# CIS565-Fall-2017/Project3-CUDA-Path-Tracer

Hardware: AMD Instinct MI355X
Metric: Mrays/sec (live paths x bounces) at 800x800 Cornell depth 8 (higher is better)
Workload: dtype f32

## Files before the change

project3-cuda-path-tracer_amd/csrc/pt_h_api.hpp:

```cpp
#pragma once

namespace one {

const char *pt_last_error(void) { return g_err; }
const char *pt_version(void) {
#ifdef PT_EXPERIMENTS
    return "ptmi355 0.1 (gfx950, fp32 no-contract, wave64) +experiments";
#else
    return "ptmi355 0.1 (gfx950, fp32 no-contract, wave64)";
#endif
}

void pt_free(void) {
    if (!R.live && !R.scratch) return;
    if (R.stream) (void)hipStreamSynchronize(R.stream);
    for (int k = 0; k < OV_MAX_LANES; ++k) {
        if (R.lane[k].stream) (void)hipStreamSynchronize(R.lane[k].stream);
        if (R.lane[k].la_stream) (void)hipStreamSynchronize(R.lane[k].la_stream);
    }
    if (R.la_gstream) (void)hipStreamSynchronize(R.la_gstream);
    for (int k = 0; k < 2; ++k) if (R.pool_mem[k]) (void)hipFree(R.pool_mem[k]);
    if (R.isect_mem) (void)hipFree(R.isect_mem);
    if (R.sort_table) (void)hipFree(R.sort_table);
    if (R.cache_mem) (void)hipFree(R.cache_mem);
    if (R.state_mem) (void)hipFree(R.state_mem);
    if (R.state_ended) (void)hipFree(R.state_ended);
    if (R.final_mem) (void)hipFree(R.final_mem);
    if (R.image && R.own_image) (void)hipFree(R.image);
    if (R.d_geoms) (void)hipFree(R.d_geoms);
    if (R.d_mats) (void)hipFree(R.d_mats);
    if (R.d_tris) (void)hipFree(R.d_tris);
    if (R.d_cull) (void)hipFree(R.d_cull);
    if (R.d_grec) (void)hipFree(R.d_grec);
    if (R.d_tri_bound) (void)hipFree(R.d_tri_bound);
    if (R.d_ginfo) (void)hipFree(R.d_ginfo);
    if (R.d_env) (void)hipFree(R.d_env);
    if (R.d_lights) (void)hipFree(R.d_lights);
    if (R.d_tex) (void)hipFree(R.d_tex);
    if (R.d_tex_tab) (void)hipFree(R.d_tex_tab);
    if (R.d_bump) (void)hipFree(R.d_bump);
    if (R.d_bump_tab) (void)hipFree(R.d_bump_tab);
    if (R.mesh_hit) (void)hipFree(R.mesh_hit);
    for (int k = 0; k < 2; ++k) if (R.mesh_flags[k]) (void)hipFree(R.mesh_flags[k]);
    if (R.d_bvh_nodes) (void)hipFree(R.d_bvh_nodes);
    if (R.d_bvh_meshes) (void)hipFree(R.d_bvh_meshes);
    if (R.d_bvh_tris) (void)hipFree(R.d_bvh_tris);
    if (R.d_bvh_top) (void)hipFree(R.d_bvh_top);
    if (R.d_cam_mask) (void)hipFree(R.d_cam_mask);
    R.d_cam_mask = nullptr; R.cam_mask_valid = false;
    if (R.d_cull0) (void)hipFree(R.d_cull0);
    R.d_cull0 = nullptr; R.cull0_tiles = 0;
    free_lanes();
    if (R.ctl) (void)hipFree(R.ctl);
    if (R.dir_mem) (void)hipFree(R.dir_mem);
    if (R.persist) (void)hipFree(R.persist);
    if (R.iter_counts) (void)hipFree(R.iter_counts);
    if (R.h_stats) (void)hipHostFree(R.h_stats);
    if (R.scratch) (void)hipFree(R.scratch);
    if (R.gb_mem) (void)hipFree(R.gb_mem);
    for (int k = 0; k < 2; ++k) if (R.dn_plane[k]) (void)hipFree(R.dn_plane[k]);
    if (R.dn_rgba) (void)hipFree(R.dn_rgba);
    if (R.gb_alt) (void)hipFree(R.gb_alt);
    if (R.alb_mem) (void)hipFree(R.alb_mem);
    for (int k = 0; k < 2; ++k) {
        if (R.tp_c[k]) (void)hipFree(R.tp_c[k]);
        if (R.tp_n[k]) (void)hipFree(R.tp_n[k]);
    }
    if (R.tp_hc) (void)hipFree(R.tp_hc);
    if (R.tp_hn) (void)hipFree(R.tp_hn);
    if (R.dbg_counts) (void)hipFree(R.dbg_counts);
    if (R.copy_stream) (void)hipStreamSynchronize(R.copy_stream);
    for (auto &h : R.host_regs) (void)hipHostUnregister(h.ptr);
    for (int j = 0; j < 2; ++j) {
        if (R.snap[j]) (void)hipFree(R.snap[j]);
        if (R.ev_snap[j]) (void)hipEventDestroy(R.ev_snap[j]);
        if (R.ev_copied[j]) (void)hipEventDestroy(R.ev_copied[j]);
    }
    if (R.copy_stream) (void)hipStreamDestroy(R.copy_stream);
    for (hipEvent_t e : R.ev) (void)hipEventDestroy(e);
    if (R.stream && R.own_stream) (void)hipStreamDestroy(R.stream);
    R = Renderer{};
}


static float glossy_alpha2(float exponent) {
    if (!(exponent > 0.0f)) return 0.0f;
    return (float)(2.0 / ((double)exponent + 2.0));
}

static void pack_materials(const pt_material *materials, int count, float *rec, bool glossy = false) {
    for (int i = 0; i < count; ++i) {
        const pt_material &m = materials[i];
        float *r = rec + (size_t)i * ptd::MAT_WORDS;
        r[0] = m.color.x; r[1] = m.color.y; r[2] = m.color.z;
        r[3] = m.specular.color.x; r[4] = m.specular.color.y; r[5] = m.specular.color.z;
        r[6] = m.hasReflective; r[7] = m.hasRefractive; r[8] = m.indexOfRefraction; r[9] = m.emittance;
        if (glossy) r[10] = glossy_alpha2(m.specular.exponent);
    }
}

static int init_impl(const pt_scene_desc *d);
int la_discard(int how);
enum { LA_STREAM = 0, LA_HOST = 1, LA_LATER = 2 };

}

#include "pt_h_scene.hpp"

namespace one {

int pt_init(const pt_scene_desc *d) {
    if (!d) return fail(PT_ERR_INVALID, "pt_init: null descriptor");
    if (R.live) pt_free();
    const int rc = init_impl(d);
    if (rc != PT_OK) {
        char keep[ERR_BYTES];
        memcpy(keep, t_err, sizeof keep);
        R.live = true;
        pt_free();
        memcpy(t_err, keep, sizeof keep);
    }
    return rc;
}

static int init_impl(const pt_scene_desc *d) {
    const int W = d->camera.resolution[0], H = d->camera.resolution[1];
    if (W <= 0 || H <= 0 || (int64_t)W * H > (1 << 28)) return fail(PT_ERR_INVALID, "pt_init: bad resolution %dx%d", W, H);
    if (d->num_geoms < 0 || d->num_materials <= 0 || (d->num_geoms > 0 && !d->geoms) || !d->materials)
        return fail(PT_ERR_INVALID, "pt_init: geoms/materials missing");
    if (d->trace_depth < 1 || d->trace_depth > MAX_DEPTH) return fail(PT_ERR_INVALID, "pt_init: trace_depth %d outside [1,%d]", d->trace_depth, MAX_DEPTH);
    const int tile_count = d->tile_count <= 0 ? 1 : d->tile_count;
    if (d->tile_index < 0 || d->tile_index >= tile_count) return fail(PT_ERR_INVALID, "pt_init: tile_index %d / tile_count %d", d->tile_index, tile_count);
    if (tile_count > 1 && d->strip_rows <= 0) return fail(PT_ERR_INVALID, "pt_init: strip_rows must be > 0 when tiling");
    for (int i = 0; i < d->num_geoms; ++i) {
        const pt_geom &g = d->geoms[i];
        if (g.type < PT_SPHERE || g.type > PT_TRIANGLE_MESH) return fail(PT_ERR_INVALID, "pt_init: geom %d has type %d", i, g.type);
        if (g.materialid < 0 || g.materialid >= d->num_materials) return fail(PT_ERR_INVALID, "pt_init: geom %d materialid %d out of range", i, g.materialid);
    }
    if (d->num_meshes < 0 || d->num_triangles < 0 || (d->num_meshes > 0 && !d->meshes) || (d->num_triangles > 0 && !d->triangles))
        return fail(PT_ERR_INVALID, "pt_init: meshes / triangles missing");
    for (int k = 0; k < d->num_meshes; ++k) {
        const pt_mesh &m = d->meshes[k];
        if (m.geom_index < 0 || m.geom_index >= d->num_geoms || d->geoms[m.geom_index].type != PT_TRIANGLE_MESH ||
            m.first_triangle < 0 || m.triangle_count < 0 ||
            (int64_t)m.first_triangle + (int64_t)m.triangle_count > (int64_t)d->num_triangles)
            return fail(PT_ERR_INVALID, "pt_init: mesh %d is inconsistent", k);
        for (int j = 0; j < k; ++j)
            if (d->meshes[j].geom_index == m.geom_index)
                return fail(PT_ERR_INVALID, "pt_init: geom %d owns more than one mesh", m.geom_index);
    }
    if ((d->flags & PT_CACHE_FIRST) && ((d->flags & PT_AA_JITTER) || d->lens_radius > 0.0f))
        return fail(PT_ERR_INVALID, "pt_init: PT_CACHE_FIRST needs identical camera rays every iteration; it cannot be "
                                    "combined with PT_AA_JITTER or a lens (INSTRUCTION.md:113)");
    if (d->lens_radius > 0.0f && !(d->focal_distance > 0.0f))
        return fail(PT_ERR_INVALID, "pt_init: a lens needs focal_distance > 0");
    std::vector<pt_light_element> light_el;
    if ((d->flags & PT_DIRECT_SKY) && !(d->flags & PT_DIRECT_LIGHT) && !(d->flags & PT_FAKE_SHADER))
        return fail(PT_ERR_INVALID, "pt_init: PT_DIRECT_SKY needs PT_DIRECT_LIGHT (the sky is one more light element of its sampler)");
    if ((d->flags & PT_DIRECT_LIGHT) && !(d->flags & PT_FAKE_SHADER)) {
        if (d->flags & PT_UNFUSED)
            return fail(PT_ERR_INVALID, "pt_init: PT_DIRECT_LIGHT cannot be combined with PT_UNFUSED (its intersection planes do not carry the winning primitive)");
        if (d->flags & PT_CACHE_FIRST)
            return fail(PT_ERR_INVALID, "pt_init: PT_DIRECT_LIGHT cannot be combined with PT_CACHE_FIRST (the table form of bounce 0 has no DIRECT variant)");
        if (d->trace_depth > MAX_DEPTH - 1)
            return fail(PT_ERR_INVALID, "pt_init: PT_DIRECT_LIGHT runs trace_depth + 1 bounces: trace_depth %d outside [1,%d]", d->trace_depth, MAX_DEPTH - 1);
        const int ne = ptlight::elements(d->geoms, d->num_geoms, d->materials, d->num_materials, light_el);
        if (ne < 0) return fail(PT_ERR_INTERNAL, "pt_init: light elements");
        if (ne > ptlight::MAX_ELEMENTS)
            return fail(PT_ERR_INVALID, "pt_init: PT_DIRECT_LIGHT: %d light elements (at most %d)", ne, ptlight::MAX_ELEMENTS);
    }
    if ((d->flags & PT_TEXTURES) && !(d->flags & PT_FAKE_SHADER)) {
        if (d->flags & PT_UNFUSED)
            return fail(PT_ERR_INVALID, "pt_init: PT_TEXTURES cannot be combined with PT_UNFUSED (its intersection planes do not carry the winning primitive)");
        if (d->flags & PT_CACHE_FIRST)
            return fail(PT_ERR_INVALID, "pt_init: PT_TEXTURES cannot be combined with PT_CACHE_FIRST (the table form of bounce 0 has no TEX variant)");
        if (d->flags & PT_DIRECT_LIGHT)
            return fail(PT_ERR_INVALID, "pt_init: PT_TEXTURES cannot be combined with PT_DIRECT_LIGHT (the direct kernels have no textured form yet)");
    }
    int ndev = 0;
    if (hipGetDeviceCount(&ndev) != hipSuccess || ndev <= 0)
        return fail(PT_ERR_DEVICE, "pt_init: no HIP device (this library has no CPU fallback)");
    if (d->device < 0 || d->device >= ndev) return fail(PT_ERR_INVALID, "pt_init: device %d of %d", d->device, ndev);
    HIPCHK(hipSetDevice(d->device));

    R = Renderer{};
    R.desc = *d; R.cam = d->camera; R.trace_depth = d->trace_depth; R.flags = d->flags; R.device = d->device;
    R.lens = Lens{(d->flags & PT_AA_JITTER) ? 1 : 0, d->lens_radius, d->focal_distance};
    R.whole_max_paths = 6000000;
    if (const char *wm = getenv("PTMI355_WHOLE_MAX")) R.whole_max_paths = strtoull(wm, nullptr, 10);
    R.whole_max_host_paths = 16000000;
    if (const char *wm = getenv("PTMI355_WHOLE_MAX_HOST")) R.whole_max_host_paths = strtoull(wm, nullptr, 10);
    if (getenv("PTMI355_WHOLE_MAX") && !getenv("PTMI355_WHOLE_MAX_HOST")) R.whole_max_host_paths = R.whole_max_paths;
    if (const char *e = getenv("PTMI355_OVERLAP")) {
        const int nl = atoi(e);
        R.ov_enabled = nl != 0;
        if (nl >= 2) { R.ov_lanes = std::min(nl, OV_MAX_LANES); R.ov_lanes_set = true; }
    }
    if (const char *e = getenv("PTMI355_OVERLAP_GB")) R.ov_budget_gb = atof(e);
    if (const char *e = pt_experiment("PTMI355_LANE_STREAMS")) R.ov_streams = std::max(1, atoi(e));
    R.epi_enabled = true;
    if (const char *e = pt_experiment("PTMI355_HOST_EPILOGUE")) R.epi_enabled = atoi(e) != 0;
    if (const char *e = pt_experiment("PTMI355_EPI_DIRECT")) R.epi_direct_enabled = atoi(e) != 0;
    R.defer_enabled = true;
    if (const char *e = pt_experiment("PTMI355_DEFER_DIR")) R.defer_enabled = atoi(e) != 0;
    R.own_enabled = true;
    if (const char *e = pt_experiment("PTMI355_OWN_SURFACE")) R.own_enabled = atoi(e) != 0;
    R.first_hit_enabled = true;
    if (const char *e = pt_experiment("PTMI355_FIRST_HIT")) R.first_hit_enabled = atoi(e) != 0;
    R.first_two_enabled = true;
    if (const char *e = pt_experiment("PTMI355_FIRST_TWO")) R.first_two_enabled = atoi(e) != 0;
    R.first_state_enabled = true;
    if (const char *e = pt_experiment("PTMI355_FIRST_STATE")) R.first_state_enabled = atoi(e) != 0;
    R.host_sparse_enabled = (d->flags & (PT_HOST_SPARSE | PT_SHARED_IMAGE)) != 0;
    if (const char *e = pt_experiment("PTMI355_ASYNC_DIRECT")) R.async_direct_enabled = atoi(e) != 0;
    R.pin_enabled = true;
    if (const char *e = pt_experiment("PTMI355_PIN")) R.pin_enabled = atoi(e) != 0;
    R.npix = W * H;
    R.map.W = W; R.map.H = H; R.map.tile_index = d->tile_index; R.map.tile_count = tile_count;
    R.map.strip_rows = tile_count > 1 ? d->strip_rows : H;
    R.map.tile_pixels = tile_rows(d->tile_index, tile_count, R.map.strip_rows, H) * W;
    if (R.map.tile_pixels <= 0) return fail(PT_ERR_INVALID, "pt_init: tile owns no rows");
    make_div_magic((uint32_t)R.map.tile_pixels, &R.map.div_magic, &R.map.div_shift);
    auto magic_holds = [](uint32_t d, uint32_t magic, uint32_t shift) {
        auto fast = [&](uint32_t n) {
            if (d == 1) return n;
            const uint32_t q = (uint32_t)(((uint64_t)magic * n) >> 32);
            return (((n - q) >> 1) + q) >> shift;
        };
        for (uint64_t k = 0; k <= 0xffffffffull / d && k < 4096; ++k)
            for (int e = -1; e <= 1; ++e) {
                const uint64_t n = k * d + (uint64_t)(int64_t)e;
                if (n <= 0xffffffffull && fast((uint32_t)n) != (uint32_t)n / d) return false;
            }
        const uint32_t probes[] = {0u, 1u, d - 1, d, d + 1, 0x7fffffffu, 0x80000000u, 0xfffffffeu, 0xffffffffu};
        for (uint32_t n : probes)
            if (fast(n) != n / d) return false;
        return true;
    };
    if (!magic_holds((uint32_t)R.map.tile_pixels, R.map.div_magic, R.map.div_shift))
        return fail(PT_ERR_INTERNAL, "pt_init: division magic failed for n / %d", R.map.tile_pixels);
    if (tile_count > 1) {
        const uint32_t span = (uint32_t)R.map.strip_rows * (uint32_t)W;
        make_div_magic(span, &R.la_tg.magic, &R.la_tg.shift);
        R.la_tg.skip = (uint32_t)(tile_count - 1) * span;
        R.la_tg.first = (uint32_t)d->tile_index * span;
        R.la_tiles_ok = span >= 2 && magic_holds(span, R.la_tg.magic, R.la_tg.shift);
    }
    R.max_batch = d->max_batch < 1 ? 1 : d->max_batch;
    if ((int64_t)R.max_batch * R.map.tile_pixels >= (int64_t)0x3ffffff0)
        return fail(PT_ERR_INVALID, "pt_init: max_batch * tile pixels must stay below 2^30 (32-bit byte offsets into the planes)");
    R.cap = (uint32_t)R.max_batch * (uint32_t)R.map.tile_pixels;
    if (d->stream) { R.stream = (hipStream_t)d->stream; R.own_stream = false; }
    else {
        int lo = 0, hi = 0;
        const char *pe = pt_experiment("PTMI355_MAIN_PRIO");
        if (hipDeviceGetStreamPriorityRange(&lo, &hi) != hipSuccess) { (void)hipGetLastError(); lo = hi = 0; }
        if ((pe && atoi(pe) == 0) || hipStreamCreateWithPriority(&R.stream, hipStreamNonBlocking, hi) != hipSuccess) {
            (void)hipGetLastError();
            HIPCHK(hipStreamCreateWithFlags(&R.stream, hipStreamNonBlocking));
        }
        R.own_stream = true;
    }
    R.live = true;

    std::vector<float> grec((size_t)std::max(1, d->num_geoms) * ptd::GEOM_WORDS, 0.0f);
    for (int i = 0; i < d->num_geoms; ++i) {
        const pt_geom &g = d->geoms[i];
        float *r = grec.data() + (size_t)i * ptd::GEOM_WORDS;
        int first = 0, count = 0, boff = 0;
        for (int k = 0, off = 0; k < d->num_meshes; ++k) {
            if (d->meshes[k].geom_index == i) { first = d->meshes[k].first_triangle; count = d->meshes[k].triangle_count; boff = off; break; }
            off += (d->meshes[k].triangle_count + 63) & ~63;
        }
        memcpy(&r[0], &g.type, 4); memcpy(&r[1], &g.materialid, 4); memcpy(&r[2], &first, 4); memcpy(&r[3], &count, 4);
        const pt_mat4 *ms[3] = {&g.inverseTransform, &g.transform, &g.invTranspose};
        const int offs[3] = {ptd::G_INV, ptd::G_FWD, ptd::G_INVT};
        for (int m = 0; m < 3; ++m)
            for (int c = 0; c < 4; ++c)
                for (int rr = 0; rr < 3; ++rr) r[offs[m] + c * 3 + rr] = ms[m]->m[c][rr];
        if (g.type == PT_TRIANGLE_MESH) memcpy(&r[ptd::G_INV + 6], &boff, 4);
    }
    std::vector<float> mrec((size_t)d->num_materials * ptd::MAT_WORDS, 0.0f);
    pack_materials(d->materials, d->num_materials, mrec.data(), (d->flags & PT_GLOSSY) != 0);
    std::vector<float> trec((size_t)std::max(1, d->num_triangles) * TRI_WORDS, 0.0f);
    for (int i = 0; i < d->num_triangles; ++i) {
        const pt_triangle &t = d->triangles[i];
        float *r = trec.data() + (size_t)i * TRI_WORDS;
        r[0] = t.v0.x; r[1] = t.v0.y; r[2] = t.v0.z;
        r[3] = t.v1.x - t.v0.x; r[4] = t.v1.y - t.v0.y; r[5] = t.v1.z - t.v0.z;
        r[6] = t.v2.x - t.v0.x; r[7] = t.v2.y - t.v0.y; r[8] = t.v2.z - t.v0.z;
    }
    for (int k = 0; k < d->num_meshes; ++k) {
        const pt_mesh &m = d->meshes[k];
        const float pad = ptbvh::spec_pad(reinterpret_cast<const float *>(d->triangles + m.first_triangle), m.triangle_count);
        for (int i = 0; i < m.triangle_count; ++i) trec[(size_t)(m.first_triangle + i) * TRI_WORDS + 10] = pad;
    }
    HIPCHK(hipMalloc(&R.d_geoms, grec.size() * 4));
    HIPCHK(hipMalloc(&R.d_mats, mrec.size() * 4));
    HIPCHK(hipMalloc(&R.d_tris, trec.size() * 4));
    HIPCHK(hipMemcpy(R.d_geoms, grec.data(), grec.size() * 4, hipMemcpyHostToDevice));
    HIPCHK(hipMemcpy(R.d_mats, mrec.data(), mrec.size() * 4, hipMemcpyHostToDevice));
    HIPCHK(hipMemcpy(R.d_tris, trec.data(), trec.size() * 4, hipMemcpyHostToDevice));
    R.scene.geoms = R.d_geoms; R.scene.ngeoms = d->num_geoms;
    R.scene.mats = R.d_mats; R.scene.nmats = d->num_materials;
    R.scene.tris = R.d_tris; R.scene.ntris = d->num_triangles;
    {
        std::vector<float> gath((size_t)std::max(1, d->num_geoms) * GREC_WORDS, 0.0f);
        std::vector<uint32_t> ginfo((size_t)std::max(1, d->num_geoms), 0u);
        for (int i = 0; i < d->num_geoms; ++i) {
            const pt_geom &g = d->geoms[i];
            float *r = gath.data() + (size_t)i * GREC_WORDS;
            const pt_mat4 *ms[3] = {&g.inverseTransform, &g.transform, &g.invTranspose};
            for (int m = 0; m < (g.type == PT_CUBE ? 2 : 3); ++m)
                for (int c = 0; c < 4; ++c)
                    for (int rr = 0; rr < 3; ++rr) r[m * 12 + c * 3 + rr] = ms[m]->m[c][rr];
            if (g.type == PT_CUBE && !pt_experiment("PTMI355_NO_AXIS_REJECT")) {
                const int ax = ptcull::reject_row(&g.inverseTransform.m[0][0], r + GREC_ROW);
                if (ax == 4 && pt_experiment("PTMI355_NO_ROW_REJECT")) r[GREC_ROW] = r[GREC_ROW + 1] = r[GREC_ROW + 2] = r[GREC_ROW + 3] = 0.0f;
            }
            ginfo[(size_t)i] = (uint32_t)g.materialid | ((uint32_t)g.type << 28);
        }
        if (d->num_materials >= (1 << 28)) return fail(PT_ERR_INVALID, "pt_init: at most 2^28 materials");
        HIPCHK(hipMalloc(&R.d_grec, gath.size() * 4));
        HIPCHK(hipMalloc((void **)&R.d_ginfo, ginfo.size() * 4));
        HIPCHK(hipMemcpy(R.d_grec, gath.data(), gath.size() * 4, hipMemcpyHostToDevice));
        HIPCHK(hipMemcpy(R.d_ginfo, ginfo.data(), ginfo.size() * 4, hipMemcpyHostToDevice));
        if (d->num_geoms > 0) {
            hipLaunchKernelGGL(k_face_normals, dim3((d->num_geoms * 8 + BLOCK - 1) / BLOCK), dim3(BLOCK), 0, R.stream,
                               R.d_grec, (const uint32_t *)R.d_ginfo, d->num_geoms);
            HIPCHK(hipGetLastError());
            HIPCHK(hipStreamSynchronize(R.stream));
        }
        R.scene.grec = R.d_grec; R.scene.ginfo = R.d_ginfo;
    }
    R.mesh_mode = MESH_NONE;
    for (int i = 0; i < d->num_geoms; ++i)
        if (d->geoms[i].type == PT_TRIANGLE_MESH) R.mesh_mode = (d->flags & PT_MESH_BVH) ? MESH_BVH : MESH_TILES;
    R.geoms_keep.assign(d->geoms, d->geoms + d->num_geoms);
    if (d->num_triangles > 0) R.tris_keep.assign(d->triangles, d->triangles + d->num_triangles);
    R.desc.geoms = R.geoms_keep.data();
    R.desc.triangles = R.tris_keep.empty() ? nullptr : R.tris_keep.data();
    if (d->num_meshes > 0) R.meshes_keep.assign(d->meshes, d->meshes + d->num_meshes);
    R.desc.meshes = R.meshes_keep.empty() ? nullptr : R.meshes_keep.data();
    R.grec_frames.assign((size_t)std::max(1, d->num_geoms) * 4, 0.0f);
    {
        const int rc = upload_cull(&R.desc, R.cam);
        if (rc != PT_OK) return rc;
    }
    if (R.mesh_mode == MESH_BVH) {
        const int rc = upload_bvh(&R.desc, grec);
        if (rc != PT_OK) return rc;
        HIPCHK(hipMemcpy(R.d_geoms, grec.data(), grec.size() * 4, hipMemcpyHostToDevice));
    }
    R.grec_keep = grec;
    {
        const size_t base = ((size_t)LDS_CTL_WORDS + (size_t)WAVES * PW_WORDS) * 4 +
                            (R.mesh_mode == MESH_TILES ? (size_t)WAVES * TRQ_WORDS * 4 : 0);
        const size_t scene = (size_t)scene_lds_words(d->num_materials, d->num_geoms) * 4;
        R.scene_lds = base + scene <= 32 * 1024;
        if (const char *e = getenv("PTMI355_SCENE_LDS")) R.scene_lds = atoi(e) != 0 && base + scene <= 64 * 1024;
        R.lds_bytes = base + (R.scene_lds ? scene : 0);
        R.lds_bytes = (R.lds_bytes + 15) & ~(size_t)15;
        if (const char *pad = pt_experiment("PTMI355_LDS_PAD")) R.lds_bytes += (size_t)atoi(pad);
    }

    R.sort_keys = 0;
    if ((R.flags & PT_SORT_MATERIAL) && (R.flags & PT_COMPACT) && !(R.flags & (PT_UNFUSED | PT_FAKE_SHADER | PT_CACHE_FIRST)) &&
        R.mesh_mode != MESH_BVH && d->num_materials <= 64) {
        bool on = true;
        if (const char *e = pt_experiment("PTMI355_SORT_FUSED")) on = atoi(e) != 0;
        double budget_gb = 96.0;
        if (const char *e = pt_experiment("PTMI355_SORT_FUSED_GB")) budget_gb = atof(e);
        R.sort_runs = 1;
        if (const char *e = pt_experiment("PTMI355_SORT_RUNS")) R.sort_runs = std::max(1, std::min(8, atoi(e)));
        const double tiles_k = (double)d->num_materials * ((double)((R.cap + 63) / 64) + 8192.0 * R.sort_runs);
        if (on && tiles_k * 2560.0 * 2.0 <= budget_gb * 1e9 && tiles_k * 64.0 < 2147483648.0) R.sort_keys = d->num_materials;
    }
    if ((R.flags & PT_DIRECT_LIGHT) && !(R.flags & PT_FAKE_SHADER) && (R.flags & PT_SORT_MATERIAL) && !R.sort_keys)
        return fail(PT_ERR_INVALID, "pt_init: PT_DIRECT_LIGHT cannot be combined with the two-kernel form of PT_SORT_MATERIAL, which this "
                                    "session would take (its intersection planes do not carry the winning primitive)");
    if ((R.flags & PT_TEXTURES) && !(R.flags & PT_FAKE_SHADER) && (R.flags & PT_SORT_MATERIAL) && !R.sort_keys)
        return fail(PT_ERR_INVALID, "pt_init: PT_TEXTURES cannot be combined with the two-kernel form of PT_SORT_MATERIAL, which this "
                                    "session would take (its intersection planes do not carry the winning primitive)");
    if (!light_el.empty()) {
        std::vector<float> lrec;
        ptlight::records(d->geoms, light_el, lrec);
        static_assert(ptlight::RECORD_WORDS == ptd::LIGHT_WORDS, "one record layout");
        HIPCHK(hipMalloc((void **)&R.d_lights, lrec.size() * 4));
        HIPCHK(hipMemcpy(R.d_lights, lrec.data(), lrec.size() * 4, hipMemcpyHostToDevice));
        R.nlights = (int)light_el.size();
        if (sky_session()) R.lamp_rec = lrec;
    }
    const size_t capz = R.cap;
    const size_t pool_mult = (size_t)std::max(1, R.sort_keys);
    const size_t run_mult = R.sort_keys > 0 ? (size_t)R.sort_runs : 1;
    for (int k = 0; k < 2; ++k) {
        R.pool_bytes = pool_mult * (((capz + 63) / 64) + 2 * 8192 * run_mult) * 64 * 10 * 4;
        HIPCHK(hipMalloc(&R.pool_mem[k], R.pool_bytes));
        R.pool[k] = carve_pool(R.pool_mem[k], R.cap);
    }
    if ((R.flags & (PT_UNFUSED | PT_FAKE_SHADER)) || ((R.flags & PT_SORT_MATERIAL) && !R.sort_keys)) {
        const int rc = ensure_isect();
        if (rc != PT_OK) return rc;
    }
    R.final_bytes = capz * 4 * 4;
    HIPCHK(hipMalloc(&R.final_mem, R.final_bytes));
    HIPCHK(hipMemsetAsync(R.final_mem, 0, capz * 4 * 4, R.stream));
    R.fin_serial = 0;
    if (const char *e = pt_experiment("PTMI355_FIN_SERIAL")) R.fin_serial = (uint32_t)strtoul(e, nullptr, 0);
    if (d->device_image) { R.image = d->device_image; R.own_image = false; }
    else {
        HIPCHK(hipMalloc(&R.image, (size_t)R.npix * 3 * 4));
        R.own_image = true;
        HIPCHK(hipMemsetAsync(R.image, 0, (size_t)R.npix * 3 * 4, R.stream));
    }
    R.max_tiles = (R.cap + TILE - 1) / TILE;
    R.ctl_bytes = offsetof(Control, bucket) - offsetof(Control, stamp) +
                  (size_t)session_bounces_max(R.trace_depth) * sizeof(((Control *)nullptr)->bucket[0]);
    HIPCHK(hipMalloc((void **)&R.ctl, sizeof(Control)));
    HIPCHK(hipMemsetAsync(R.ctl, 0, sizeof(Control), R.stream));
    HIPCHK(hipMalloc((void **)&R.persist, sizeof(Persist)));
    HIPCHK(hipMemsetAsync(R.persist, 0, sizeof(Persist), R.stream));
    hipDeviceProp_t prop;
    HIPCHK(hipGetDeviceProperties(&prop, d->device));
    const int cus = prop.multiProcessorCount > 0 ? prop.multiProcessorCount : 256;
    int per_cu = 8;
    {
        const bool sorted = R.sort_keys > 0;
        const bool own = R.mesh_mode == MESH_NONE && !sorted;
        auto size_for = [&](auto sh) -> int {
            constexpr int SH = decltype(sh)::value;
            const void *fns[2];
            if (R.mesh_mode == MESH_BVH) { fns[0] = bounce_fn<MESH_PRE, SH>(R.scene_lds, false, false); fns[1] = bounce_fn<MESH_PRE, SH>(R.scene_lds, true, false); }
            else if (R.mesh_mode == MESH_TILES) { fns[0] = bounce_fn<MESH_TILES, SH>(R.scene_lds, false, sorted); fns[1] = bounce_fn<MESH_TILES, SH>(R.scene_lds, true, sorted); }
            else { fns[0] = bounce_fn<MESH_NONE, SH>(R.scene_lds, false, sorted); fns[1] = bounce_fn<MESH_NONE, SH>(R.scene_lds, true, sorted); }
            const void *fns_own[2] = {own ? bounce_fn<MESH_NONE, SH>(R.scene_lds, false, false, true) : fns[0], own ? bounce_fn<MESH_NONE, SH>(R.scene_lds, true, false, true) : fns[1]};
            const void *fns_tab[4] = {own ? bounce_fn<MESH_NONE, SH>(R.scene_lds, false, false, false, true) : fns[0], own ? bounce_fn<MESH_NONE, SH>(R.scene_lds, true, false, false, true) : fns[1],
                                      own ? bounce_fn<MESH_NONE, SH>(R.scene_lds, false, false, true, true) : fns[0], own ? bounce_fn<MESH_NONE, SH>(R.scene_lds, true, false, true, true) : fns[1]};
            const void *fns_two[2] = {own ? bounce_fn<MESH_NONE, SH>(R.scene_lds, true, false, false, true, true) : fns[0],
                                      own ? bounce_fn<MESH_NONE, SH>(R.scene_lds, true, false, true, true, true) : fns[0]};
            const void *fns_state[2] = {own ? bounce_fn<MESH_NONE, SH>(R.scene_lds, true, false, false, true, true, true) : fns[0],
                                        own ? bounce_fn<MESH_NONE, SH>(R.scene_lds, true, false, true, true, true, true) : fns[0]};
            for (const void *f : {fns[0], fns[1], fns_own[0], fns_own[1], fns_tab[0], fns_tab[1], fns_tab[2], fns_tab[3], fns_two[0], fns_two[1],
                                  fns_state[0], fns_state[1]}) {
                int n = 0;
                HIPCHK(hipOccupancyMaxActiveBlocksPerMultiprocessor(&n, f, BLOCK, R.lds_bytes));
                per_cu = std::min(per_cu, n);
            }
            return PT_OK;
        };
        int rc = size_for(std::integral_constant<int, 0>{});
        if (rc == PT_OK && (R.nlights > 0 || sky_session())) rc = size_for(std::integral_constant<int, SH_DIRECT>{});
        if (rc == PT_OK && (R.flags & PT_TEXTURES) && !(R.flags & PT_FAKE_SHADER)) rc = size_for(std::integral_constant<int, SH_TEX>{});
        if (rc != PT_OK) return rc;
    }
    if (per_cu < 1) per_cu = 1;
    if (per_cu > 8) per_cu = 8;
    if (const char *e = pt_experiment("PTMI355_WGS_PER_CU")) per_cu = std::max(1, std::min(per_cu, atoi(e)));
    R.grid = (int)std::min<uint32_t>((R.max_tiles + WAVES - 1) / WAVES, (uint32_t)cus * (uint32_t)per_cu);
    R.per_cu = per_cu;
    if (const char *e = pt_experiment("PTMI355_LA_CUS")) R.la_cus = std::max(0, std::min(64, atoi(e) & ~7));
    if (R.grid < 1) R.grid = 1;
    if (R.grid * WAVES > 8192) R.grid = 8192 / WAVES;
    {
        int n = 0;
        HIPCHK(hipOccupancyMaxActiveBlocksPerMultiprocessor(
            &n, R.scene_lds ? (const void *)k_iteration<true> : (const void *)k_iteration<false>, BLOCK, R.lds_bytes));
        n = std::max(1, std::min(n, 8));
        if (const char *e = pt_experiment("PTMI355_WGS_PER_CU")) n = std::max(1, std::min(n, atoi(e)));
        R.grid_iter = (int)std::min<uint32_t>((R.max_tiles + WAVES - 1) / WAVES, (uint32_t)cus * (uint32_t)n);
        R.grid_iter = std::max(1, std::min(R.grid_iter, 8192 / WAVES));
        R.grid_iter_cur = R.grid_iter; R.cus = cus;
        if (const char *e = pt_experiment("PTMI355_ITER_TPW")) R.iter_tpw = std::max(0, atoi(e));
        if (const char *e = pt_experiment("PTMI355_ITER_WGS_ALL")) R.iter_wgs_per_cu_all = std::max(1, atoi(e));
        R.iter_counts_bytes = (size_t)MAX_DEPTH * (size_t)R.grid_iter * 4;
        HIPCHK(hipMalloc((void **)&R.iter_counts, R.iter_counts_bytes));
        void *hs = nullptr, *ds = nullptr;
        if (hipHostMalloc(&hs, sizeof(HostStats), hipHostMallocMapped) == hipSuccess && hipHostGetDevicePointer(&ds, hs, 0) == hipSuccess) {
            memset(hs, 0, sizeof(HostStats));
            R.h_stats = (HostStats *)hs; R.d_stats = (HostStats *)ds;
        } else {
            (void)hipGetLastError();
            if (hs) (void)hipHostFree(hs);
        }
    }
    if (R.mesh_mode == MESH_BVH) {
        R.mesh_hit_bytes = (size_t)(((capz + 63) / 64) * 64) * sizeof(float4);
        HIPCHK(hipMalloc((void **)&R.mesh_hit, R.mesh_hit_bytes));
        R.flag_words = (size_t)R.max_tiles + 2 * (size_t)R.grid * WAVES + 8;
        for (int k = 0; k < 2; ++k) {
            HIPCHK(hipMalloc((void **)&R.mesh_flags[k], R.flag_words * sizeof(unsigned long long)));
            HIPCHK(hipMemsetAsync(R.mesh_flags[k], 0, R.flag_words * sizeof(unsigned long long), R.stream));
        }
        HIPCHK(hipFuncSetAttribute((const void *)k_mesh<true>, hipFuncAttributeMaxDynamicSharedMemorySize, (int)MESH_LDS_BYTES));
        HIPCHK(hipFuncSetAttribute((const void *)k_mesh<false>, hipFuncAttributeMaxDynamicSharedMemorySize, (int)MESH_LDS_BYTES));
        R.grid_mesh = (int)std::min<uint32_t>((R.max_tiles + MESH_WG_WAVES - 1) / MESH_WG_WAVES, (uint32_t)cus);
        if (R.grid_mesh < 1) R.grid_mesh = 1;
    }
    if (R.flags & PT_CACHE_FIRST) {
        HIPCHK(hipMalloc(&R.cache_mem, (size_t)R.map.tile_pixels * Isect::FIRST_HIT_BYTES));
    } else if (R.first_hit_enabled && !(R.flags & (PT_UNFUSED | PT_SORT_MATERIAL | PT_FAKE_SHADER | PT_AA_JITTER)) && R.mesh_mode == MESH_NONE) {
        if (hipMalloc(&R.cache_mem, (size_t)R.map.tile_pixels * Isect::FIRST_HIT_BYTES) != hipSuccess) { (void)hipGetLastError(); R.cache_mem = nullptr; }
        bool fixed0 = R.cache_mem != nullptr && R.first_state_enabled && !(R.flags & PT_GLOSSY);
        for (int m = 0; m < d->num_materials; ++m) fixed0 = fixed0 && !(d->materials[m].hasRefractive > 0.0f);
        if (fixed0) {
            if (hipMalloc(&R.state_mem, first_state_bytes((size_t)R.map.tile_pixels)) != hipSuccess) { (void)hipGetLastError(); R.state_mem = nullptr; }
            if (R.state_mem && R.map.tile_pixels % TILE == 0 &&
                hipMalloc((void **)&R.state_ended, (size_t)(R.map.tile_pixels / TILE) * sizeof(uint32_t)) != hipSuccess) { (void)hipGetLastError(); R.state_ended = nullptr; }
        }
    }
    if ((R.flags & PT_SORT_MATERIAL) && !R.sort_keys) {
        if (d->num_materials + 1 > SORT_MAX_BINS)
            return fail(PT_ERR_INVALID, "pt_init: PT_SORT_MATERIAL keeps one bin per material in LDS: at most %d materials", SORT_MAX_BINS - 1);
        {
            int per_cu_sort = 8;
            if (const char *e = pt_experiment("PTMI355_SORT_WGS")) per_cu_sort = std::max(1, atoi(e));
            R.sort_wave = true;
            if (const char *e = pt_experiment("PTMI355_SORT_WAVE")) R.sort_wave = atoi(e) != 0;
            const uint32_t chunks = (R.cap + SORT_CHUNK - 1) / SORT_CHUNK;
            R.grid_sort = (int)std::max<uint32_t>(1u, std::min<uint32_t>(chunks, (uint32_t)cus * (uint32_t)per_cu_sort));
        }
        HIPCHK(hipMalloc((void **)&R.sort_table, ((size_t)(d->num_materials + 1) * R.grid_sort + 4) * sizeof(uint32_t)));
    }
    {
        const size_t Wp = ((size_t)R.grid * WAVES * pool_mult * run_mult + 3) & ~(size_t)3;
        R.dir_stride = range_dir_words(Wp);
        R.dir_bytes = (size_t)MAX_DEPTH * R.dir_stride * sizeof(uint32_t);
        HIPCHK(hipMalloc((void **)&R.dir_mem, R.dir_bytes));
    }
    {
        const int rc = update_cam_mask();
        if (rc != PT_OK) return rc;
    }
    {
        bool on = true;
        if (const char *e = getenv("PTMI355_CULL0")) on = atoi(e) != 0;
        if (on && R.scene.ngeoms >= 1 && R.scene.ngeoms <= 64 && R.map.tile_pixels % TILE == 0) {
            R.cull0_tiles = (uint32_t)(R.map.tile_pixels / TILE);
            HIPCHK(hipMalloc((void **)&R.d_cull0, (size_t)R.cull0_tiles * sizeof(unsigned long long)));
            const int rc = update_cull0();
            if (rc != PT_OK) return rc;
        }
    }
    if (const char *e = pt_experiment("PTMI355_DBG_COUNTS")) {
        R.dbg_words = (size_t)std::max(64, atoi(e));
        HIPCHK(hipMalloc((void **)&R.dbg_counts, R.dbg_words * 4));
        HIPCHK(hipMemsetAsync(R.dbg_counts, 0, R.dbg_words * 4, R.stream));
    }
    HIPCHK(hipStreamSynchronize(R.stream));
    t_err[0] = 0;
    return PT_OK;
}

int pt_set_camera(const pt_camera *camera, int trace_depth) {
    if (!R.live) return fail(PT_ERR_INVALID, "pt_set_camera: not initialised");
    if (!camera) return fail(PT_ERR_INVALID, "pt_set_camera: null camera");
    if (camera->resolution[0] != R.map.W || camera->resolution[1] != R.map.H)
        return fail(PT_ERR_INVALID, "pt_set_camera: resolution changed (%dx%d -> %dx%d); re-init instead",
                    R.map.W, R.map.H, camera->resolution[0], camera->resolution[1]);
    if (trace_depth < 1 || trace_depth > MAX_DEPTH)
        return fail(PT_ERR_INVALID, "pt_set_camera: trace_depth %d outside [1, %d]", trace_depth, MAX_DEPTH);
    if ((R.flags & PT_DIRECT_LIGHT) && !(R.flags & PT_FAKE_SHADER) && trace_depth > MAX_DEPTH - 1)
        return fail(PT_ERR_INVALID, "pt_set_camera: PT_DIRECT_LIGHT runs trace_depth + 1 bounces: trace_depth %d outside [1, %d]", trace_depth, MAX_DEPTH - 1);
    if (memcmp(&R.cam, camera, sizeof R.cam) != 0) {
        R.cache_valid = false;
        const int rc = la_discard(LA_HOST);
        if (rc) return rc;
    }
    bool recull = false;
    {
        const double reach = (double)std::fabs(camera->position.x) + std::fabs(camera->position.y) + std::fabs(camera->position.z);
        if (std::isfinite(reach) && reach > (double)R.scene.rmax && reach != R.cull_eye_reach) {
            const int rc = upload_cull(&R.desc, *camera);
            if (rc != PT_OK) return rc;
            recull = true;
        }
    }
    if (trace_depth != R.trace_depth) {
        R.ctl_bytes = offsetof(Control, bucket) - offsetof(Control, stamp) +
                      (size_t)session_bounces_max(trace_depth) * sizeof(((Control *)nullptr)->bucket[0]);
    }
    const bool moved = memcmp(&R.cam, camera, sizeof R.cam) != 0;
    R.cam = *camera;
    R.trace_depth = trace_depth;
    if (moved || recull) {
        R.ov_active = false;
        const int rc = update_cull0();
        if (rc != PT_OK) return rc;
    }
    if (recull && R.mesh_mode == MESH_BVH) {
        HIPCHK(hipStreamSynchronize(R.stream));
        float **old[] = {&R.d_bvh_nodes, &R.d_bvh_tris, &R.d_bvh_top};
        for (float **p : old) { if (*p) (void)hipFree(*p); *p = nullptr; }
        if (R.d_bvh_meshes) { (void)hipFree(R.d_bvh_meshes); R.d_bvh_meshes = nullptr; }
        const int rc = upload_bvh(&R.desc, R.grec_keep);
        if (rc != PT_OK) return rc;
        HIPCHK(hipMemcpy(R.d_geoms, R.grec_keep.data(), R.grec_keep.size() * 4, hipMemcpyHostToDevice));
    }
    if ((moved || recull) && R.mesh_mode == MESH_BVH) {
        HIPCHK(hipStreamSynchronize(R.stream));
        const int rc = update_cam_mask();
        if (rc != PT_OK) return rc;
    }
    return PT_OK;
}

int pt_set_lens(float lens_radius, float focal_distance) {
    if (!R.live) return fail(PT_ERR_INVALID, "pt_set_lens: not initialised");
    if (lens_radius > 0.0f && !(focal_distance > 0.0f)) return fail(PT_ERR_INVALID, "pt_set_lens: a lens needs focal_distance > 0");
    if (lens_radius > 0.0f && (R.flags & PT_CACHE_FIRST))
        return fail(PT_ERR_INVALID, "pt_set_lens: PT_CACHE_FIRST cannot be combined with a lens");
    R.lens.radius = lens_radius; R.lens.focal = focal_distance;
    return PT_OK;
}

static int upload_sky_lights(const float *texels, int n) {
    std::vector<float> rows, cols, rec;
    int count = (int)(R.lamp_rec.size() / (size_t)ptlight::RECORD_WORDS);
    const std::vector<float> *src = &R.lamp_rec;
    if (texels && n > 0 && ptlight::sky_table(texels, n, rows, cols)) {
        count = ptlight::sky_records(R.lamp_rec, n, rows, cols, rec);
        src = &rec;
    }
    if (R.d_lights) { (void)hipFree(R.d_lights); R.d_lights = nullptr; }
    R.nlights = 0;
    if (count == 0) return PT_OK;
    if (hipMalloc((void **)&R.d_lights, src->size() * 4) != hipSuccess) {
        (void)hipGetLastError(); R.d_lights = nullptr;
        return fail(PT_ERR_NOMEM, "pt_set_environment: %zu bytes of device memory for the light table", src->size() * 4);
    }
    HIPCHK(hipMemcpy(R.d_lights, src->data(), src->size() * 4, hipMemcpyHostToDevice));
    R.nlights = count;
    return PT_OK;
}

int pt_set_environment(const float *texels, int n) {
    if (!R.live) return fail(PT_ERR_INVALID, "pt_set_environment: not initialised");
    if (n < 0 || n > 1024) return fail(PT_ERR_INVALID, "pt_set_environment: n = %d outside [0, 1024]", n);
    if (n > 0 && !texels) return fail(PT_ERR_INVALID, "pt_set_environment: null texels with n = %d", n);
    if (!texels) n = 0;
    const int rc = la_discard(LA_HOST);
    if (rc) return rc;
    HIPCHK(hipStreamSynchronize(R.stream));
    for (int k = 0; k < OV_MAX_LANES; ++k) {
        if (R.lane[k].stream) HIPCHK(hipStreamSynchronize(R.lane[k].stream));
        if (R.lane[k].la_stream) HIPCHK(hipStreamSynchronize(R.lane[k].la_stream));
    }
    if (R.la_gstream) HIPCHK(hipStreamSynchronize(R.la_gstream));
    if (R.copy_stream) HIPCHK(hipStreamSynchronize(R.copy_stream));
    R.ov_active = false;
    R.env_n = 0;
    if (R.d_env) { (void)hipFree(R.d_env); R.d_env = nullptr; }
    R.env_keep.clear();
    if (sky_session()) {
        const int rc2 = upload_sky_lights(nullptr, 0);
        if (rc2) return rc2;
    }
    if (n == 0) return PT_OK;
    const size_t count = (size_t)6 * (size_t)n * (size_t)n;
    std::vector<float> quad(count * 4);
    for (size_t k = 0; k < count; ++k) {
        quad[4 * k] = texels[3 * k]; quad[4 * k + 1] = texels[3 * k + 1]; quad[4 * k + 2] = texels[3 * k + 2]; quad[4 * k + 3] = 0.0f;
    }
    if (hipMalloc((void **)&R.d_env, count * 16) != hipSuccess) {
        (void)hipGetLastError(); R.d_env = nullptr;
        return fail(PT_ERR_NOMEM, "pt_set_environment: %zu bytes of device memory for a %d x %d x 6 map", count * 16, n, n);
    }
    HIPCHK(hipMemcpy(R.d_env, quad.data(), count * 16, hipMemcpyHostToDevice));
    R.env_keep.assign(texels, texels + count * 3);
    R.env_n = n;
    if (sky_session()) return upload_sky_lights(texels, n);
    return PT_OK;
}

int pt_get_environment(float *texels, int capacity_texels, int *n) {
    if (!R.live) return fail(PT_ERR_INVALID, "pt_get_environment: not initialised");
    if (!n) return fail(PT_ERR_INVALID, "pt_get_environment: null n");
    const int en = R.env_n;
    *n = en;
    if (en == 0) return PT_OK;
    const size_t count = (size_t)6 * (size_t)en * (size_t)en;
    if (!texels || capacity_texels < 0 || (size_t)capacity_texels < count)
        return fail(PT_ERR_INVALID, "pt_get_environment: room for %d texels, the map has %zu", texels ? capacity_texels : 0, count);
    memcpy(texels, R.env_keep.data(), count * 12);
    return PT_OK;
}

int pt_set_texture(int material, const float *texels, int n) {
    if (!R.live) return fail(PT_ERR_INVALID, "pt_set_texture: not initialised");
    if (!(R.flags & PT_TEXTURES)) return fail(PT_ERR_INVALID, "pt_set_texture: the session was not initialised with PT_TEXTURES");
    if (material < 0 || material >= R.scene.nmats) return fail(PT_ERR_INVALID, "pt_set_texture: material %d outside [0, %d)", material, R.scene.nmats);
    if (n < 0 || n > 1024) return fail(PT_ERR_INVALID, "pt_set_texture: n = %d outside [0, 1024]", n);
    if (n > 0 && !texels) return fail(PT_ERR_INVALID, "pt_set_texture: null texels with n = %d", n);
    if (!texels) n = 0;
    const int rc = la_discard(LA_HOST);
    if (rc) return rc;
    HIPCHK(hipStreamSynchronize(R.stream));
    for (int k = 0; k < OV_MAX_LANES; ++k) {
        if (R.lane[k].stream) HIPCHK(hipStreamSynchronize(R.lane[k].stream));
        if (R.lane[k].la_stream) HIPCHK(hipStreamSynchronize(R.lane[k].la_stream));
    }
    if (R.la_gstream) HIPCHK(hipStreamSynchronize(R.la_gstream));
    if (R.copy_stream) HIPCHK(hipStreamSynchronize(R.copy_stream));
    R.ov_active = false;
    if (R.tex_n.empty()) { R.tex_n.assign((size_t)R.scene.nmats, 0); R.tex_keep.resize((size_t)R.scene.nmats); }
    std::vector<int> tn = R.tex_n;
    tn[(size_t)material] = n;
    std::vector<int2> tab((size_t)R.scene.nmats);
    size_t total = 0;
    int ntex = 0;
    for (int m = 0; m < R.scene.nmats; ++m) {
        tab[(size_t)m] = make_int2((int)total, tn[(size_t)m]);
        total += (size_t)6 * (size_t)tn[(size_t)m] * (size_t)tn[(size_t)m];
        if (tn[(size_t)m] > 0) ++ntex;
    }
    if (total > (size_t)0x7fffffff) return fail(PT_ERR_INVALID, "pt_set_texture: %zu texels in all (at most 2^31 - 1)", total);
    float4 *d_new = nullptr;
    if (ntex > 0) {
        std::vector<float> quad(total * 4);
        for (int m = 0; m < R.scene.nmats; ++m) {
            const size_t cnt = (size_t)6 * (size_t)tn[(size_t)m] * (size_t)tn[(size_t)m];
            const float *src = m == material ? texels : R.tex_keep[(size_t)m].data();
            float *dst = quad.data() + (size_t)tab[(size_t)m].x * 4;
            for (size_t k = 0; k < cnt; ++k) { dst[4 * k] = src[3 * k]; dst[4 * k + 1] = src[3 * k + 1]; dst[4 * k + 2] = src[3 * k + 2]; dst[4 * k + 3] = 0.0f; }
        }
        if (hipMalloc((void **)&d_new, total * 16) != hipSuccess) {
            (void)hipGetLastError();
            return fail(PT_ERR_NOMEM, "pt_set_texture: %zu bytes of device memory for the session's textures", total * 16);
        }
        HIPCHK(hipMemcpy(d_new, quad.data(), total * 16, hipMemcpyHostToDevice));
    }
    if (!R.d_tex_tab) HIPCHK(hipMalloc((void **)&R.d_tex_tab, tab.size() * sizeof(int2)));
    HIPCHK(hipMemcpy(R.d_tex_tab, tab.data(), tab.size() * sizeof(int2), hipMemcpyHostToDevice));
    const int old_n = R.tex_n[(size_t)material];
    if (old_n != n || (n > 0 && memcmp(R.tex_keep[(size_t)material].data(), texels, (size_t)6 * (size_t)n * (size_t)n * 12) != 0))
        R.alb_valid = false;
    if (R.d_tex) (void)hipFree(R.d_tex);
    R.d_tex = d_new;
    R.tex_n = tn;
    if (n > 0) R.tex_keep[(size_t)material].assign(texels, texels + (size_t)6 * (size_t)n * (size_t)n * 3);
    else std::vector<float>().swap(R.tex_keep[(size_t)material]);
    R.ntex = ntex;
    return PT_OK;
}

int pt_get_texture(int material, float *texels, int capacity_texels, int *n) {
    if (!R.live) return fail(PT_ERR_INVALID, "pt_get_texture: not initialised");
    if (!(R.flags & PT_TEXTURES)) return fail(PT_ERR_INVALID, "pt_get_texture: the session was not initialised with PT_TEXTURES");
    if (material < 0 || material >= R.scene.nmats) return fail(PT_ERR_INVALID, "pt_get_texture: material %d outside [0, %d)", material, R.scene.nmats);
    if (!n) return fail(PT_ERR_INVALID, "pt_get_texture: null n");
    const int tn = R.tex_n.empty() ? 0 : R.tex_n[(size_t)material];
// ... 634 lines not shown
```

project3-cuda-path-tracer_amd/csrc/pt_h_enqueue.hpp:

```cpp
#pragma once

namespace {

BounceArgs bounce_args(int depth) {
    BounceArgs a{};
    a.dbg_counts = R.dbg_counts;
    a.in = R.pool[R.cur];
    a.out = (R.flags & PT_COMPACT) ? R.pool[R.cur ^ 1] : R.pool[R.cur];
    a.isect = R.isect;
    a.scene = R.scene;
    a.map = R.map;
    a.ctl = R.ctl;
    a.dir_in = tile_dir((R.flags & PT_COMPACT) ? R.cur_dir : -1);
    a.dir_out = tile_dir(depth);
    a.fin = R.final_mem;
    a.fin_stamp = R.fin_serial;
    a.cam = R.cam;
    a.lens = R.lens;
    a.depth = depth; a.trace_depth = R.trace_depth; a.iter0 = R.step_iter0;
    a.pool_n = (uint32_t)R.map.tile_pixels * (uint32_t)R.step_count;
    a.gen_rays = (depth == 0 && R.gen_fused) ? 1 : 0;
    a.mesh_hit = R.mesh_hit;
    a.mesh_flags_in = R.mesh_flags[depth & 1]; a.mesh_flags_out = R.mesh_flags[(depth + 1) & 1];
    a.mesh_scan = R.mesh_marked ? 0 : 1;
    a.cam_mask = (R.cam_mask_valid && !(R.lens.radius > 0.0f)) ? R.d_cam_mask : nullptr;
    const bool same_rays = !R.lens.aa && !(R.lens.radius > 0.0f);
    a.cull0 = (R.cull0_tiles && same_rays) ? R.d_cull0 : nullptr;
    a.cull0_tiles = R.cull0_tiles;
    a.iter_counts = R.iter_counts;
    a.persist = R.persist;
    a.env = R.d_env; a.env_n = R.env_n;
    a.lights = R.d_lights; a.nlights = R.nlights;
    if (R.ntex + R.nbump > 0) { a.tex = R.d_tex; a.tex_tab = R.d_tex_tab; }
    if (R.nbump > 0) { a.bumps = R.d_bump; a.bump_tab = R.d_bump_tab; }
    return a;
}

int next_fin_stamp(void) {
    if (++R.fin_serial == 0) {
        HIPCHK(hipMemsetAsync(R.final_mem, 0, (size_t)R.cap * 16, R.stream));
        if (R.ov_ready)
            for (int j = 1; j < R.ov_lanes; ++j)
                HIPCHK(hipMemsetAsync(R.lane[j].b.final_mem, 0, R.final_bytes, R.stream));
        R.fin_serial = 1;
    }
    return PT_OK;
}

int enqueue_begin(int iter0, int count, bool stepping, bool clear = true) {
    if (count < 1 || count > R.max_batch)
        return fail(PT_ERR_INVALID, "batch count %d outside [1, max_batch=%d]", count, R.max_batch);
    if (iter0 < 0 || (int64_t)iter0 + count - 1 > 0x7fffffff)
        return fail(PT_ERR_INVALID, "iteration %d (+%d) outside [0, 2^31)", iter0, count);
    R.step_iter0 = iter0; R.step_count = count; R.step_depth = 0; R.cur = 0; R.cur_dir = -1;
    R.pool_own = false;
    R.ov_active = false;
    R.last_ctl = R.ctl;
    const int rc = next_fin_stamp();
    if (rc) return rc;
    R.sorted_isects = false;
    R.mesh_marked = false;
    R.self_gathered = false; R.host_stats_serial = 0;
    if (clear) HIPCHK(hipMemsetAsync(&R.ctl->stamp, 0, R.ctl_bytes, R.stream));
    if (R.mesh_mode == MESH_BVH)
        for (int k = 0; k < 2; ++k)
            HIPCHK(hipMemsetAsync(R.mesh_flags[k], 0, R.flag_words * sizeof(unsigned long long), R.stream));
    R.gen_fused = !stepping && (!(R.flags & (PT_UNFUSED | PT_SORT_MATERIAL | PT_FAKE_SHADER)) || R.sort_keys > 0);
    R.gen_sort = !stepping && (R.flags & PT_SORT_MATERIAL) && !R.sort_keys && !(R.flags & PT_FAKE_SHADER) && R.sort_wave &&
                 R.scene.nmats + 1 <= SORTW_MAX_BINS;
    if (R.gen_fused || R.gen_sort) return PT_OK;
    const uint32_t total = (uint32_t)R.map.tile_pixels * (uint32_t)count;
    StageTimer tm(PT_STAGE_RAYGEN);
    hipLaunchKernelGGL(k_raygen, dim3((total + BLOCK - 1) / BLOCK), dim3(BLOCK), 0, R.stream, R.pool[0], R.cam,
                       R.lens, R.map, count, iter0, R.trace_depth, R.ctl);
    HIPCHK(hipGetLastError());
    return PT_OK;
}

#define PT_MESH_DISPATCH(CALL)                                          \
    do {                                                                \
        if (R.scene_lds) {                                              \
            constexpr bool SLDS = true;                                 \
            if (R.mesh_mode == MESH_BVH) { constexpr int MESH = MESH_BVH; CALL; }            \
            else if (R.mesh_mode == MESH_TILES) { constexpr int MESH = MESH_TILES; CALL; }   \
            else { constexpr int MESH = MESH_NONE; CALL; }              \
        } else {                                                        \
            constexpr bool SLDS = false;                                \
            if (R.mesh_mode == MESH_BVH) { constexpr int MESH = MESH_BVH; CALL; }            \
            else if (R.mesh_mode == MESH_TILES) { constexpr int MESH = MESH_TILES; CALL; }   \
            else { constexpr int MESH = MESH_NONE; CALL; }              \
        }                                                               \
    } while (0)

void launch_intersect(const Pool &in, const uint32_t *n_ptr, uint32_t n_fixed, const RangeDir &dir,
                      const uint32_t *nprev, bool raygen_pool = false, bool generate = false) {
    const bool same_rays = !R.lens.aa && !(R.lens.radius > 0.0f);
    const unsigned long long *cull0 = (raygen_pool && R.cull0_tiles && same_rays) ? R.d_cull0 : nullptr;
    RayGen gen{};
    if (generate) {
        gen.cam = R.cam; gen.lens = R.lens; gen.map = R.map; gen.trace_depth = R.trace_depth;
        gen.iter0 = R.step_iter0;
        PT_MESH_DISPATCH(hipLaunchKernelGGL((k_intersect<MESH, SLDS, true>), dim3(R.grid), dim3(BLOCK), R.lds_bytes, R.stream, in,
                                            R.isect, R.scene, n_ptr, n_fixed, dir, nprev, R.ctl, cull0, R.cull0_tiles, gen));
        return;
    }
    PT_MESH_DISPATCH(hipLaunchKernelGGL((k_intersect<MESH, SLDS>), dim3(R.grid), dim3(BLOCK), R.lds_bytes, R.stream, in,
                                        R.isect, R.scene, n_ptr, n_fixed, dir, nprev, R.ctl, cull0, R.cull0_tiles, gen));
}

template <int MESH, int SH = 0>
const void *bounce_fn(bool slds, bool gen, bool sorted, bool own = false, bool table = false, bool first2 = false, bool state2 = false) {
    if constexpr (MESH == MESH_NONE) {
        if (table && !sorted) {
            constexpr int SH0 = SH & (SH_ENV | SH_GLOSSY);
            if (first2 && state2) {
                if (own) return slds ? (const void *)k_bounce<MODE_STATE2, true, MESH, true, true, false, true, 0> : (const void *)k_bounce<MODE_STATE2, true, MESH, false, true, false, true, 0>;
                return slds ? (const void *)k_bounce<MODE_STATE2, true, MESH, true, true, false, false, 0> : (const void *)k_bounce<MODE_STATE2, true, MESH, false, true, false, false, 0>;
            }
            if (first2) {
                if (own) return slds ? (const void *)k_bounce<MODE_FIRST2, true, MESH, true, true, false, true, SH0> : (const void *)k_bounce<MODE_FIRST2, true, MESH, false, true, false, true, SH0>;
                return slds ? (const void *)k_bounce<MODE_FIRST2, true, MESH, true, true, false, false, SH0> : (const void *)k_bounce<MODE_FIRST2, true, MESH, false, true, false, false, SH0>;
            }
            if (own) {
                if (slds) return gen ? (const void *)k_bounce<MODE_CACHE0, true, MESH, true, true, false, true, SH0> : (const void *)k_bounce<MODE_CACHE0, true, MESH, true, false, false, true, SH0>;
                return gen ? (const void *)k_bounce<MODE_CACHE0, true, MESH, false, true, false, true, SH0> : (const void *)k_bounce<MODE_CACHE0, true, MESH, false, false, false, true, SH0>;
            }
            if (slds) return gen ? (const void *)k_bounce<MODE_CACHE0, true, MESH, true, true, false, false, SH0> : (const void *)k_bounce<MODE_CACHE0, true, MESH, true, false, false, false, SH0>;
            return gen ? (const void *)k_bounce<MODE_CACHE0, true, MESH, false, true, false, false, SH0> : (const void *)k_bounce<MODE_CACHE0, true, MESH, false, false, false, false, SH0>;
        }
        if (own && !sorted) {
            if (slds) return gen ? (const void *)k_bounce<MODE_FUSED, true, MESH, true, true, false, true, SH> : (const void *)k_bounce<MODE_FUSED, true, MESH, true, false, false, true, SH>;
            return gen ? (const void *)k_bounce<MODE_FUSED, true, MESH, false, true, false, true, SH> : (const void *)k_bounce<MODE_FUSED, true, MESH, false, false, false, true, SH>;
        }
    }
    if constexpr (MESH != MESH_PRE) {
        if (sorted) {
            if (slds) return gen ? (const void *)k_bounce<MODE_FUSED, true, MESH, true, true, true, false, SH> : (const void *)k_bounce<MODE_FUSED, true, MESH, true, false, true, false, SH>;
            return gen ? (const void *)k_bounce<MODE_FUSED, true, MESH, false, true, true, false, SH> : (const void *)k_bounce<MODE_FUSED, true, MESH, false, false, true, false, SH>;
        }
    }
    if (slds) return gen ? (const void *)k_bounce<MODE_FUSED, true, MESH, true, true, false, false, SH> : (const void *)k_bounce<MODE_FUSED, true, MESH, true, false, false, false, SH>;
    return gen ? (const void *)k_bounce<MODE_FUSED, true, MESH, false, true, false, false, SH> : (const void *)k_bounce<MODE_FUSED, true, MESH, false, false, false, false, SH>;
}
#define PT_SHADE_DISPATCH_WITH(EXTRA, ...)                                                                  \
    do {                                                                                                    \
        switch ((a.env_n ? SH_ENV : 0) | ((R.flags & PT_GLOSSY) ? SH_GLOSSY : 0)) {                         \
        case SH_ENV | SH_GLOSSY: { constexpr int SH = SH_ENV | SH_GLOSSY | (EXTRA); __VA_ARGS__; } break;   \
        case SH_GLOSSY: { constexpr int SH = SH_GLOSSY | (EXTRA); __VA_ARGS__; } break;                     \
        case SH_ENV: { constexpr int SH = SH_ENV | (EXTRA); __VA_ARGS__; } break;                           \
        default: { constexpr int SH = (EXTRA); __VA_ARGS__; } break;                                        \
        }                                                                                                   \
    } while (0)
#define PT_SHADE_DISPATCH(...) PT_SHADE_DISPATCH_WITH(0, __VA_ARGS__)
template <int MODE, bool COMPACT, int MESH, bool SLDS, bool GEN, bool SORT = false, bool OWN = false>
void launch_k_bounce(const BounceArgs &a) {
    if constexpr (MODE == MODE_STATE2) {
        hipLaunchKernelGGL((k_bounce<MODE, COMPACT, MESH, SLDS, GEN, SORT, OWN, 0>), dim3(R.grid), dim3(BLOCK), R.lds_bytes, R.stream, a);
        return;
    } else {
        if constexpr (MODE == MODE_FUSED) {
            if (a.nlights > 0 && a.depth >= a.trace_depth - 1) {
                PT_SHADE_DISPATCH_WITH(SH_DIRECT, hipLaunchKernelGGL((k_bounce<MODE, COMPACT, MESH, SLDS, GEN, SORT, OWN, SH>), dim3(R.grid), dim3(BLOCK), R.lds_bytes, R.stream, a));
                return;
            }
            if (a.tex_tab != nullptr) {
                PT_SHADE_DISPATCH_WITH(SH_TEX, hipLaunchKernelGGL((k_bounce<MODE, COMPACT, MESH, SLDS, GEN, SORT, OWN, SH>), dim3(R.grid), dim3(BLOCK), R.lds_bytes, R.stream, a));
                return;
            }
        }
        PT_SHADE_DISPATCH(hipLaunchKernelGGL((k_bounce<MODE, COMPACT, MESH, SLDS, GEN, SORT, OWN, SH>), dim3(R.grid), dim3(BLOCK), R.lds_bytes, R.stream, a));
    }
}
template <int MODE, bool COMPACT, int MESH, bool GEN>
void launch_bounce_at(const BounceArgs &a) {
    if constexpr (MODE == MODE_FUSED && COMPACT && MESH != MESH_PRE) {
        if (R.sort_keys > 0) {
            if (R.scene_lds) launch_k_bounce<MODE, COMPACT, MESH, true, GEN, true>(a);
            else launch_k_bounce<MODE, COMPACT, MESH, false, GEN, true>(a);
            return;
        }
    }
    if constexpr ((MODE == MODE_FUSED || MODE == MODE_CACHE0 || mode_first2(MODE)) && COMPACT && MESH == MESH_NONE) {
        if (R.own_form) {
            if (R.scene_lds) launch_k_bounce<MODE, COMPACT, MESH, true, GEN, false, true>(a);
            else launch_k_bounce<MODE, COMPACT, MESH, false, GEN, false, true>(a);
            return;
        }
    }
    if (R.scene_lds) launch_k_bounce<MODE, COMPACT, MESH, true, GEN>(a);
    else launch_k_bounce<MODE, COMPACT, MESH, false, GEN>(a);
}
template <int MODE, bool COMPACT>
void launch_bounce(const BounceArgs &a) {
    if constexpr (MODE == MODE_ISECT) {
        launch_bounce_at<MODE, COMPACT, MESH_NONE, false>(a);
    } else if constexpr (MODE == MODE_CACHE0) {
        if (a.gen_rays) launch_bounce_at<MODE, COMPACT, MESH_NONE, true>(a); else launch_bounce_at<MODE, COMPACT, MESH_NONE, false>(a);
    } else if constexpr (mode_first2(MODE)) {
        static_assert(COMPACT, "MODE_FIRST2 / MODE_STATE2 compact");
        launch_bounce_at<MODE, COMPACT, MESH_NONE, true>(a);
    } else {
        const bool gen = a.gen_rays != 0;
        if (R.mesh_mode == MESH_BVH) { if (gen) launch_bounce_at<MODE, COMPACT, MESH_PRE, true>(a); else launch_bounce_at<MODE, COMPACT, MESH_PRE, false>(a); }
        else if (R.mesh_mode == MESH_TILES) { if (gen) launch_bounce_at<MODE, COMPACT, MESH_TILES, true>(a); else launch_bounce_at<MODE, COMPACT, MESH_TILES, false>(a); }
        else { if (gen) launch_bounce_at<MODE, COMPACT, MESH_NONE, true>(a); else launch_bounce_at<MODE, COMPACT, MESH_NONE, false>(a); }
    }
}

int enqueue_bounce(int depth, bool may_fuse = false) {
    BounceArgs a = bounce_args(depth);
    R.own_form = false;
    const bool compact = (R.flags & PT_COMPACT) != 0;
    const bool sort2 = (R.flags & PT_SORT_MATERIAL) && R.sort_keys == 0;
    const bool unfused = (R.flags & PT_UNFUSED) != 0 || sort2;
    if (unfused) {
        StageTimer tm(PT_STAGE_INTERSECT);
        const bool generate = depth == 0 && R.gen_sort;
        const uint32_t *n_ptr = (compact && !generate) ? &R.ctl->nlive[depth] : (const uint32_t *)nullptr;
        const uint32_t *nprev = (compact && depth > 0) ? &R.ctl->nlive[depth - 1] : (const uint32_t *)nullptr;
        launch_intersect(a.in, n_ptr, a.pool_n, a.dir_in, nprev, depth == 0, generate);
        HIPCHK(hipGetLastError());
    }
    if (sort2) {
        a.in = R.pool[R.cur]; a.out = R.pool[R.cur ^ 1];
        a.sort_table = R.sort_table; a.nbins = R.scene.nmats + 1;
        a.gen_rays = (depth == 0 && R.gen_sort) ? 1 : 0;
        {
            StageTimer tm(PT_STAGE_SORT);
            const size_t lds = ((size_t)LDS_CTL_WORDS + (size_t)((a.nbins + 3) & ~3)) * 4;
            if (compact) hipLaunchKernelGGL(k_sort_hist<true>, dim3(R.grid_sort), dim3(BLOCK), lds, R.stream, a);
            else hipLaunchKernelGGL(k_sort_hist<false>, dim3(R.grid_sort), dim3(BLOCK), lds, R.stream, a);
            HIPCHK(hipGetLastError());
        }
        StageTimer tm(PT_STAGE_BOUNCE);
        if (a.nbins <= SORTW_MAX_BINS && R.sort_wave) {
            const size_t lds = shade_sorted_w_lds_words(R.scene.nmats) * 4;
#define PT_SORTED_W(COMPACT, GEN) \
    PT_SHADE_DISPATCH(hipLaunchKernelGGL((k_shade_sorted_w<COMPACT, GEN, SH>), dim3(R.grid_sort), dim3(BLOCK), lds, R.stream, a))
            if (a.gen_rays) {
                if (compact) PT_SORTED_W(true, true); else PT_SORTED_W(false, true);
            } else {
                if (compact) PT_SORTED_W(true, false); else PT_SORTED_W(false, false);
            }
#undef PT_SORTED_W
        } else {
            const size_t nb = (size_t)((a.nbins + 3) & ~3);
            const size_t lds = ((size_t)LDS_CTL_WORDS + (3 + WAVES) * nb + 2 * SORT_CHUNK +
                                (a.nbins <= 64 ? (size_t)R.scene.nmats * ptd::MAT_WORDS : 0)) * 4;
            if (compact) PT_SHADE_DISPATCH(hipLaunchKernelGGL((k_shade_sorted<true, SH>), dim3(R.grid_sort), dim3(BLOCK), lds, R.stream, a));
            else PT_SHADE_DISPATCH(hipLaunchKernelGGL((k_shade_sorted<false, SH>), dim3(R.grid_sort), dim3(BLOCK), lds, R.stream, a));
        }
        HIPCHK(hipGetLastError());
        R.cur ^= 1; R.cur_dir = -1;
        R.sorted_isects = true;
        R.step_depth = depth + 1;
        return PT_OK;
    }
    const bool same_rays = !R.lens.aa && !(R.lens.radius > 0.0f);
    const bool auto0 = depth == 0 && !unfused && R.first_hit_enabled && R.cache_mem != nullptr && !(R.flags & PT_FAKE_SHADER) &&
                       R.mesh_mode == MESH_NONE && R.sort_keys == 0 && same_rays && a.tex_tab == nullptr &&
                       !(a.nlights > 0 && depth >= a.trace_depth - 1);
    const bool cached0 = depth == 0 && !unfused && ((R.flags & PT_CACHE_FIRST) || auto0);
    const bool first2 = may_fuse && auto0 && !(R.flags & PT_CACHE_FIRST) && compact && R.gen_fused && R.first_two_enabled &&
                        R.trace_depth >= 2 && !(a.nlights > 0 && 1 >= a.trace_depth - 1);
    const bool state2 = first2 && R.state_mem != nullptr && a.env_n == 0;
    if (first2) {
        depth = 1;
        a.depth = 1;
        a.dir_out = tile_dir(1);
        a.gen_rays = 1;
    }
    a.defer_dir = (compact && !unfused && R.mesh_mode == MESH_NONE && R.sort_keys == 0 && depth + 1 < R.trace_depth &&
                   R.defer_enabled) ? 1 : 0;
    R.own_form = own_surface_plan((uint64_t)a.pool_n, R.scene.ngeoms,
                                  compact && !unfused && R.mesh_mode == MESH_NONE && R.sort_keys == 0 &&
                                  R.own_enabled);
    if (cached0 && !R.cache_valid) {
        StageTimer tm(PT_STAGE_INTERSECT);
        const Isect cache{R.cache_mem, (uint32_t)R.map.tile_pixels};
        const int blocks = std::min(R.grid, (R.map.tile_pixels + BLOCK - 1) / BLOCK);
        const hipStream_t fs = R.lane_cur ? R.lane_main : R.stream;
        PT_MESH_DISPATCH(hipLaunchKernelGGL((k_cache_first<MESH, SLDS>), dim3(blocks), dim3(BLOCK), R.lds_bytes, fs,
                                            cache, R.scene, R.cam, R.map, R.state_mem, R.state_ended));
        HIPCHK(hipGetLastError());
        if (R.lane_cur) {
            HIPCHK(hipEventRecord(R.ov_enter, fs));
            HIPCHK(hipStreamWaitEvent(R.stream, R.ov_enter, 0));
            R.first_hit_refence = true;
        }
        R.cache_valid = true;
        R.first_hit_fills++;
    }
    if (!cached0 && !unfused && R.mesh_mode == MESH_BVH) {
        StageTimer tm(PT_STAGE_MESH);
        if (compact) hipLaunchKernelGGL((k_mesh<true>), dim3(R.grid_mesh), dim3(MESH_BLOCK), MESH_LDS_BYTES, R.stream, a);
        else hipLaunchKernelGGL((k_mesh<false>), dim3(R.grid_mesh), dim3(MESH_BLOCK), MESH_LDS_BYTES, R.stream, a);
        HIPCHK(hipGetLastError());
    }
    StageTimer tm(PT_STAGE_BOUNCE);
    if (cached0) {
        a.isect = Isect{R.cache_mem, (uint32_t)R.map.tile_pixels};
        R.first_hit_launches++;
        if (state2) {
            a.first_state = R.state_mem; a.first_ended = R.state_ended; a.first_ended_tiles = (uint32_t)(R.map.tile_pixels / TILE);
            R.first_two_launches++; R.first_state_launches++; tm.two_bounces(); launch_bounce<MODE_STATE2, true>(a);
        }
        else if (first2) { R.first_two_launches++; tm.two_bounces(); launch_bounce<MODE_FIRST2, true>(a); }
        else if (compact) launch_bounce<MODE_CACHE0, true>(a); else launch_bounce<MODE_CACHE0, false>(a);
    } else if (unfused) {
        if (compact) launch_bounce<MODE_ISECT, true>(a); else launch_bounce<MODE_ISECT, false>(a);
    } else {
        if (compact) launch_bounce<MODE_FUSED, true>(a); else launch_bounce<MODE_FUSED, false>(a);
    }
    HIPCHK(hipGetLastError());
    if (R.mesh_mode == MESH_BVH) {
        R.mesh_marked = !cached0 && !unfused;
    }
    if (compact) { R.cur ^= 1; R.cur_dir = depth; }
    R.pool_own = R.own_form;
    R.step_depth = depth + 1;
    return PT_OK;
}

int enqueue_fake(void) {
    const uint32_t total = (uint32_t)R.map.tile_pixels * (uint32_t)R.step_count;
    launch_intersect(R.pool[R.cur], nullptr, total, tile_dir(-1), nullptr);
    HIPCHK(hipGetLastError());
    hipLaunchKernelGGL(k_shade_fake, dim3((total + BLOCK - 1) / BLOCK), dim3(BLOCK), 0, R.stream, R.pool[R.cur],
                       R.isect, R.scene.mats, R.map, R.step_iter0, total, R.final_mem, R.fin_serial);
    HIPCHK(hipGetLastError());
    R.step_depth = 1;
    return PT_OK;
}

int enqueue_end(void) {
    if (R.self_gathered) { R.whole = false; return PT_OK; }
    if (R.la_tracing) {
        hipLaunchKernelGGL(k_gather, dim3(1), dim3(BLOCK), 0, R.stream, R.image, R.final_mem, R.cap, R.map, R.step_count, R.ctl,
                           R.persist, session_bounces(), 0u, R.whole ? 1 : 0, 1, R.fin_serial, R.iter_counts, (uint32_t)R.grid_iter_cur,
                           (HostStats *)nullptr);
        R.whole = false;
        HIPCHK(hipGetLastError());
        HIPCHK(hipEventRecord(R.lane_cur->traced, R.stream));
        R.lane_cur->gathered_valid = false;
        return PT_OK;
    }
    StageTimer tm(PT_STAGE_GATHER);
    hipStream_t gs = R.stream;
    if (R.lane_cur) {
        HIPCHK(hipEventRecord(R.lane_cur->traced, R.stream));
        HIPCHK(hipStreamWaitEvent(R.lane_main, R.lane_cur->traced, 0));
        gs = R.lane_main;
    }
    hipLaunchKernelGGL(k_gather, dim3((R.map.tile_pixels + BLOCK - 1) / BLOCK), dim3(BLOCK), 0, gs, R.image,
                       R.final_mem, R.cap, R.map,
                       R.step_count, R.ctl, R.persist, (R.flags & PT_FAKE_SHADER) ? 0 : session_bounces(),
                       (R.flags & PT_FAKE_SHADER) ? (uint32_t)R.map.tile_pixels * (uint32_t)R.step_count : 0u,
                       R.whole ? 1 : 0, R.epi_done ? 1 : 0, R.fin_serial, R.iter_counts, (uint32_t)R.grid_iter_cur,
                       (R.whole && R.host_stats_serial) ? R.d_stats : (HostStats *)nullptr);
    R.whole = false;
    R.image_epoch++;
    HIPCHK(hipGetLastError());
    if (R.lane_cur) {
        HIPCHK(hipEventRecord(R.lane_cur->gathered, gs));
        R.lane_cur->gathered_valid = true;
    }
    return PT_OK;
}

Renderer::Bufs take_bufs(void) {
    Renderer::Bufs b{};
    for (int k = 0; k < 2; ++k) { b.pool_mem[k] = R.pool_mem[k]; b.pool[k] = R.pool[k]; b.mesh_flags[k] = R.mesh_flags[k]; }
    b.final_mem = R.final_mem; b.ctl = R.ctl; b.dir_mem = R.dir_mem; b.mesh_hit = R.mesh_hit; b.iter_counts = R.iter_counts;
    return b;
}
void put_bufs(const Renderer::Bufs &b) {
    for (int k = 0; k < 2; ++k) { R.pool_mem[k] = b.pool_mem[k]; R.pool[k] = b.pool[k]; R.mesh_flags[k] = b.mesh_flags[k]; }
    R.final_mem = b.final_mem; R.ctl = b.ctl; R.dir_mem = b.dir_mem; R.mesh_hit = b.mesh_hit; R.iter_counts = b.iter_counts;
}

void free_lanes(void) {
    for (int k = 0; k < OV_MAX_LANES; ++k) {
        Renderer::Lane &l = R.lane[k];
        if (l.stream && k < R.ov_streams) { (void)hipStreamSynchronize(l.stream); (void)hipStreamDestroy(l.stream); }
        if (l.la_stream && k < R.ov_streams) { (void)hipStreamSynchronize(l.la_stream); (void)hipStreamDestroy(l.la_stream); }
        if (l.traced) (void)hipEventDestroy(l.traced);
        if (l.gathered) (void)hipEventDestroy(l.gathered);
        if (k > 0) {
            for (int j = 0; j < 2; ++j) { if (l.b.pool_mem[j]) (void)hipFree(l.b.pool_mem[j]); if (l.b.mesh_flags[j]) (void)hipFree(l.b.mesh_flags[j]); }
            if (l.b.final_mem) (void)hipFree(l.b.final_mem);
            if (l.b.ctl) (void)hipFree(l.b.ctl);
            if (l.b.dir_mem) (void)hipFree(l.b.dir_mem);
            if (l.b.iter_counts) (void)hipFree(l.b.iter_counts);
            if (l.b.mesh_hit) (void)hipFree(l.b.mesh_hit);
        }
        l = Renderer::Lane{};
    }
    if (R.la_gstream) { (void)hipStreamSynchronize(R.la_gstream); (void)hipStreamDestroy(R.la_gstream); R.la_gstream = nullptr; }
    if (R.la_rs_event) { (void)hipEventDestroy(R.la_rs_event); R.la_rs_event = nullptr; }
    R.la_masks_ready = false; R.la_masked_last = false;
    if (R.ov_enter) (void)hipEventDestroy(R.ov_enter);
    R.ov_enter = nullptr;
    R.ov_ready = false;
}

static int alloc_lanes(void) {
    R.lane[0].b = take_bufs();
    for (int j = 1; j < R.ov_lanes; ++j) {
        Renderer::Bufs &b = R.lane[j].b;
        for (int k = 0; k < 2; ++k) {
            HIPCHK(hipMalloc((void **)&b.pool_mem[k], R.pool_bytes));
            b.pool[k] = carve_pool(b.pool_mem[k], R.cap);
        }
        HIPCHK(hipMalloc((void **)&b.final_mem, R.final_bytes));
        HIPCHK(hipMemsetAsync(b.final_mem, 0, R.final_bytes, R.stream));
        HIPCHK(hipMalloc((void **)&b.ctl, sizeof(Control)));
        HIPCHK(hipMemsetAsync(b.ctl, 0, sizeof(Control), R.stream));
        HIPCHK(hipMalloc((void **)&b.dir_mem, R.dir_bytes));
        HIPCHK(hipMalloc((void **)&b.iter_counts, R.iter_counts_bytes));
        if (R.mesh_mode == MESH_BVH) {
            HIPCHK(hipMalloc((void **)&b.mesh_hit, R.mesh_hit_bytes));
            for (int k = 0; k < 2; ++k) {
                HIPCHK(hipMalloc((void **)&b.mesh_flags[k], R.flag_words * sizeof(unsigned long long)));
                HIPCHK(hipMemsetAsync(b.mesh_flags[k], 0, R.flag_words * sizeof(unsigned long long), R.stream));
            }
        }
    }
    R.ov_streams = std::max(1, std::min(R.ov_streams, R.ov_lanes));
    for (int k = 0; k < R.ov_lanes; ++k) {
        if (k < R.ov_streams) HIPCHK(hipStreamCreateWithFlags(&R.lane[k].stream, hipStreamNonBlocking));
        else R.lane[k].stream = R.lane[k % R.ov_streams].stream;
        HIPCHK(hipEventCreateWithFlags(&R.lane[k].traced, hipEventDisableTiming));
        HIPCHK(hipEventCreateWithFlags(&R.lane[k].gathered, hipEventDisableTiming));
    }
    HIPCHK(hipEventCreateWithFlags(&R.ov_enter, hipEventDisableTiming));
    return PT_OK;
}

int ensure_lanes(void) {
    if (R.ov_ready || !R.ov_enabled) return PT_OK;
    const double per_lane = 2.0 * (double)R.pool_bytes + (double)R.final_bytes + (double)R.dir_bytes + (double)R.mesh_hit_bytes +
                            2.0 * (double)R.flag_words * 8.0 + (double)sizeof(Control);
    double budget = R.ov_budget_gb * 1e9;
    size_t free_b = 0, total_b = 0;
    if (hipMemGetInfo(&free_b, &total_b) == hipSuccess) budget = std::min(budget, 0.5 * (double)free_b);
    const int fit = 1 + (int)std::min(16.0, std::floor(budget / std::max(1.0, per_lane)));
    R.ov_lanes = std::min(R.ov_lanes, fit);
    if (R.ov_lanes == 3) R.ov_lanes = 2;
    if (R.ov_lanes < 2) { R.ov_enabled = false; return PT_OK; }
    if (alloc_lanes() != PT_OK) {
        (void)hipGetLastError();
        free_lanes();
        R.ov_enabled = false;
        return PT_OK;
    }
    R.ov_ready = true;
    return PT_OK;
}

bool ensure_la_masks(void) {
    if (R.la_masks_ready) return true;
    if (R.la_masks_failed || R.la_shared_device || !R.ov_ready || R.la_cus < 8 || R.cus != 256 || R.mesh_mode == MESH_BVH) return false;
    uint32_t trace_mask[8], gather_mask[8];
    for (int b = 0; b < 8; ++b) { trace_mask[b] = 0xffffffffu; gather_mask[b] = 0; }
    for (int b = 0; b < R.la_cus; ++b) { trace_mask[b / 32] &= ~(1u << (b % 32)); gather_mask[b / 32] |= 1u << (b % 32); }
    bool ok = hipExtStreamCreateWithCUMask(&R.la_gstream, 8, gather_mask) == hipSuccess &&
              hipEventCreateWithFlags(&R.la_rs_event, hipEventDisableTiming) == hipSuccess;
    for (int k = 0; ok && k < R.ov_streams; ++k) ok = hipExtStreamCreateWithCUMask(&R.lane[k].la_stream, 8, trace_mask) == hipSuccess;
    if (!ok) {
        (void)hipGetLastError();
        for (int k = 0; k < R.ov_streams; ++k) if (R.lane[k].la_stream) { (void)hipStreamDestroy(R.lane[k].la_stream); R.lane[k].la_stream = nullptr; }
        if (R.la_gstream) { (void)hipStreamDestroy(R.la_gstream); R.la_gstream = nullptr; }
        if (R.la_rs_event) { (void)hipEventDestroy(R.la_rs_event); R.la_rs_event = nullptr; }
        R.la_masks_failed = true;
        return false;
    }
    for (int k = R.ov_streams; k < R.ov_lanes; ++k) R.lane[k].la_stream = R.lane[k % R.ov_streams].la_stream;
    R.grid_la = (int)std::min<uint32_t>((uint32_t)R.grid, (uint32_t)(R.cus - R.la_cus) * (uint32_t)std::max(1, R.per_cu));
    R.la_masks_ready = true;
    return true;
}

bool overlap_eligible(int count) {
    return R.ov_ok && R.ov_enabled && !R.profiling && !R.epi_host && !R.dbg_counts &&
           !(R.flags & (PT_UNFUSED | PT_FAKE_SHADER)) && (!(R.flags & PT_SORT_MATERIAL) || R.sort_keys > 0) &&
           count >= 1 && count <= R.max_batch;
}

int enqueue_batch_serial(int iter0, int count);

int enter_lanes(void) {
    if (R.fin_serial == 0xffffffffu) {
        HIPCHK(hipStreamSynchronize(R.stream));
        for (int j = 0; j < R.ov_lanes; ++j) HIPCHK(hipStreamSynchronize(R.lane[j].stream));
        for (int j = 0; j < R.ov_lanes; ++j) if (R.lane[j].la_stream) HIPCHK(hipStreamSynchronize(R.lane[j].la_stream));
        for (int j = 0; j < R.ov_lanes; ++j) HIPCHK(hipMemsetAsync(R.lane[j].b.final_mem, 0, R.final_bytes, R.stream));
        HIPCHK(hipStreamSynchronize(R.stream));
        R.fin_serial = 0;
        R.ov_active = false;
        for (auto &w : R.la) { w.valid = false; w.inflight = false; }
    }
    if (!R.ov_active) {
        HIPCHK(hipEventRecord(R.ov_enter, R.stream));
        for (int k = 0; k < R.ov_lanes; ++k) {
            HIPCHK(hipStreamWaitEvent(R.lane[k].stream, R.ov_enter, 0));
            if (R.lane[k].la_stream && k < R.ov_streams) HIPCHK(hipStreamWaitEvent(R.lane[k].la_stream, R.ov_enter, 0));
            R.lane[k].gathered_valid = false;
        }
    }
    return PT_OK;
}

int enqueue_on_lane(Renderer::Lane &l, int iter0, int count) {
    if (l.gathered_valid) HIPCHK(hipStreamWaitEvent(l.stream, l.gathered, 0));
    const Renderer::Bufs home = take_bufs();
    R.lane_main = R.stream; R.lane_cur = &l;
    put_bufs(l.b); R.stream = l.stream;
    const int rc = enqueue_batch_serial(iter0, count);
    R.stream = R.lane_main; put_bufs(home);
    R.lane_cur = nullptr; R.lane_main = nullptr;
    R.ov_active = rc == PT_OK && !R.first_hit_refence;
    R.first_hit_refence = false;
    return rc;
}

int enqueue_batch(int iter0, int count) {
    if (!overlap_eligible(count)) return enqueue_batch_serial(iter0, count);
    int rc = ensure_lanes();
    if (rc) return rc;
    if (!R.ov_enabled) return enqueue_batch_serial(iter0, count);
    if (R.la_masked_last) { R.ov_active = false; R.la_masked_last = false; }
    rc = enter_lanes();
    if (rc) return rc;
    Renderer::Lane &l = R.lane[R.ov_next];
    R.ov_next = (R.ov_next + 1) % R.ov_lanes;
    return enqueue_on_lane(l, iter0, count);
}

int enqueue_window(int slot, int iter0, int count, bool masked) {
    if (masked != R.la_masked_last) R.ov_active = false;
    int rc = enter_lanes();
    if (rc) return rc;
    Renderer::Lane &l = R.lane[slot];
    const hipStream_t plain = l.stream;
    const int grid = R.grid;
    if (masked) { l.stream = l.la_stream; R.grid = R.grid_la; }
    R.la_tracing = true;
    rc = enqueue_on_lane(l, iter0, count);
    R.la_tracing = false;
    l.stream = plain; R.grid = grid;
    R.la_masked_last = masked;
    return rc;
}

int iter_grid_for(uint64_t paths, bool shared) {
    if (!shared || R.iter_tpw <= 0) return R.grid_iter;
    const uint64_t tiles = (paths + TILE - 1) / TILE;
    const uint64_t by_tiles = (tiles + (uint64_t)(WAVES * R.iter_tpw) - 1) / (uint64_t)(WAVES * R.iter_tpw);
    const uint64_t floor_g = ((uint64_t)R.iter_wgs_per_cu_all * (uint64_t)R.cus + (uint64_t)R.ov_lanes - 1) / (uint64_t)std::max(1, R.ov_lanes);
    return (int)std::min<uint64_t>(std::max(by_tiles, floor_g), (uint64_t)R.grid_iter);
}

int enqueue_batch_serial(int iter0, int count) {
    const uint64_t whole_limit = (count == 1 && R.epi_host) ? std::max(R.whole_max_paths, R.whole_max_host_paths) : R.whole_max_paths;
    const bool whole = !(R.flags & (PT_UNFUSED | PT_SORT_MATERIAL | PT_FAKE_SHADER | PT_CACHE_FIRST)) && (R.flags & PT_COMPACT) &&
                       R.mesh_mode == MESH_NONE && R.sort_keys == 0 && R.nlights == 0 && R.ntex + R.nbump == 0 && count >= 1 &&
                       (uint64_t)R.map.tile_pixels * (uint64_t)count <= whole_limit;
    int rc = enqueue_begin(iter0, count, false, !whole);
    if (rc) return rc;
    if (R.flags & PT_FAKE_SHADER) {
        rc = enqueue_fake();
        if (rc) return rc;
    } else if (whole) {
        StageTimer tm(PT_STAGE_BOUNCE);
        BounceArgs a = bounce_args(0);
        if (count == 1 && !R.lane_cur && R.epi_enabled) {
// ... 25 lines not shown
```

project3-cuda-path-tracer_amd/csrc/pt_h_scene.hpp:

```cpp
#pragma once

namespace {

int upload_tri_bounds(const pt_scene_desc *d, double Rorigin);

int upload_cull(const pt_scene_desc *d, const pt_camera &cam) {
    const int n = d->num_geoms;
    std::vector<const float *> inv((size_t)std::max(1, n));
    std::vector<char> sph((size_t)std::max(1, n)), skip((size_t)std::max(1, n));
    for (int i = 0; i < n; ++i) {
        inv[(size_t)i] = &d->geoms[i].inverseTransform.m[0][0];
        sph[(size_t)i] = d->geoms[i].type == PT_SPHERE;
        skip[(size_t)i] = d->geoms[i].type == PT_TRIANGLE_MESH;
    }
    const double eye[3] = {(double)cam.position.x, (double)cam.position.y, (double)cam.position.z};
    std::vector<ptcull::Box> boxes;
    std::vector<double> pts(eye, eye + 3);
    for (int t = 0; t < d->num_triangles; ++t) {
        const pt_vec3 *v = &d->triangles[t].v0;
        double m = 0.0;
        for (int k = 0; k < 3; ++k) m = std::max(m, (double)std::fabs(v[k].x) + std::fabs(v[k].y) + std::fabs(v[k].z));
        if (t == 0 || m > pts[3]) { if (pts.size() < 6) pts.resize(6, 0.0); pts[3] = m; pts[4] = 0.0; pts[5] = 0.0; }
    }
    R.scene.rmax = ptcull::make_boxes(inv.data(), reinterpret_cast<const bool *>(sph.data()),
                                      reinterpret_cast<const bool *>(skip.data()), n, pts.data(), (int)(pts.size() / 3), boxes);
    std::vector<float> rec((size_t)std::max(1, n) * CULL_WORDS, 0.0f);
    for (int i = 0; i < n; ++i) {
        float *r = rec.data() + (size_t)i * CULL_WORDS;
        for (int k = 0; k < 3; ++k) ptcull::centre_half(boxes[(size_t)i].lo[k], boxes[(size_t)i].hi[k], r[2 * k], r[2 * k + 1]);
        int ax = 3;
        if (d->geoms[i].type == PT_CUBE && !pt_experiment("PTMI355_NO_AXIS_REJECT"))
            ax = ptcull::reject_row(&d->geoms[i].inverseTransform.m[0][0], &r[7]);
        if (ax == 4 && pt_experiment("PTMI355_NO_ROW_REJECT")) ax = 3;
        const int tw = d->geoms[i].type | (ax << 8);
        memcpy(&r[6], &tw, 4);
        const uint32_t ent = ((uint32_t)d->geoms[i].type << 7) | ((uint32_t)i << 9);
        memcpy(&r[11], &ent, 4);
    }
    if (!R.d_cull) HIPCHK(hipMalloc(&R.d_cull, rec.size() * 4));
    HIPCHK(hipMemcpyAsync(R.d_cull, rec.data(), rec.size() * 4, hipMemcpyHostToDevice, R.stream));
    HIPCHK(hipStreamSynchronize(R.stream));
    R.scene.cull = R.d_cull;
    R.cull_eye_reach = std::fabs(eye[0]) + std::fabs(eye[1]) + std::fabs(eye[2]);
    return upload_tri_bounds(d, (double)R.scene.rmax);
}

void make_tri_bounds(const pt_triangle *tris, int count, double Rorigin, float *out) {
    const double u = 0x1p-24;
    const float pad = ptbvh::spec_pad(reinterpret_cast<const float *>(tris), count);
    const int n4 = (count + 3) & ~3;
    for (int i = 0; i < n4; ++i) {
        float *o = out + (size_t)i * 4;
        if (i >= count) { o[0] = o[1] = o[2] = 0.0f; o[3] = -1.0f; continue; }
        const pt_triangle &t = tris[i];
        const float v0[3] = {t.v0.x, t.v0.y, t.v0.z};
        const float e1[3] = {t.v1.x - t.v0.x, t.v1.y - t.v0.y, t.v1.z - t.v0.z};
        const float e2[3] = {t.v2.x - t.v0.x, t.v2.y - t.v0.y, t.v2.z - t.v0.z};
        double c[3], h2 = 0.0, cinf = 0.0;
        bool fin = true;
        for (int a = 0; a < 3; ++a) {
            const float x1 = v0[a] + e1[a], x2 = v0[a] + e2[a];
            const float lo = std::fmin(v0[a], std::fmin(x1, x2)) - pad, hi = std::fmax(v0[a], std::fmax(x1, x2)) + pad;
            if (!std::isfinite(lo) || !std::isfinite(hi)) fin = false;
            c[a] = 0.5 * ((double)lo + (double)hi);
            const double h = 0.5 * ((double)hi - (double)lo);
            h2 += h * h;
            cinf = std::fmax(cinf, std::fabs(c[a]));
        }
        if (!fin || !std::isfinite(Rorigin)) { o[0] = o[1] = o[2] = 0.0f; o[3] = INFINITY; continue; }
        const double R0 = std::sqrt(h2);
        const double reach = Rorigin + cinf + R0;
        const double delta = 2.0 * 1.7320508075688772 * u * reach;
        const double Rs = (R0 + 4.0 * (delta + 0x1p-19 * reach)) * (1.0 + 0x1p-10);
        for (int a = 0; a < 3; ++a) o[a] = (float)c[a];
        o[3] = ptcull::round_up(Rs * Rs);
        if (!std::isfinite(o[3])) o[3] = INFINITY;
    }
}

void make_tri_records(const float *spheres, int n, _Float16 *records, float frame[4]) {
    double lo[3] = {INFINITY, INFINITY, INFINITY}, hi[3] = {-INFINITY, -INFINITY, -INFINITY};
    for (int i = 0; i < n; ++i) {
        const float *sp = spheres + (size_t)i * 4;
        if (!(sp[3] >= 0.0f) || !std::isfinite(sp[3])) continue;
        for (int a = 0; a < 3; ++a) { lo[a] = std::fmin(lo[a], (double)sp[a]); hi[a] = std::fmax(hi[a], (double)sp[a]); }
    }
    double g[3] = {0.0, 0.0, 0.0}, Rm = 0.0;
    if (lo[0] <= hi[0]) for (int a = 0; a < 3; ++a) g[a] = (double)(float)(0.5 * (lo[a] + hi[a]));
    for (int i = 0; i < n; ++i) {
        const float *sp = spheres + (size_t)i * 4;
        if (!(sp[3] >= 0.0f) || !std::isfinite(sp[3])) continue;
        const double dx = sp[0] - g[0], dy = sp[1] - g[1], dz = sp[2] - g[2];
        Rm = std::fmax(Rm, std::sqrt(dx * dx + dy * dy + dz * dz) + std::sqrt((double)sp[3]));
    }
    Rm = Rm > 0.0 ? Rm * (1.0 + 0x1p-20) : 1.0;
    float ir = (float)(1.0 / Rm);
    if (!(ir > 0.0f) || !std::isfinite(ir)) ir = 1.0f;
    frame[0] = (float)g[0]; frame[1] = (float)g[1]; frame[2] = (float)g[2]; frame[3] = ir;
    auto pair = [](double v, _Float16 &h, _Float16 &l) { h = (_Float16)(float)v; l = (_Float16)(float)(v - (double)(float)h); };
    for (int i = 0; i < n; ++i) {
        const float *sp = spheres + (size_t)i * 4;
        _Float16 *a = records + (size_t)i * 32;
        for (int k = 0; k < 32; ++k) a[k] = (_Float16)0.0f;
        a[29] = (_Float16)1.0f; a[30] = (_Float16)1.0f;
        if (!(sp[3] >= 0.0f)) { a[27] = (_Float16)30000.0f; continue; }
        if (!std::isfinite(sp[3])) { a[27] = (_Float16)-30000.0f; continue; }
        const double c[3] = {(sp[0] - g[0]) * (double)ir, (sp[1] - g[1]) * (double)ir, (sp[2] - g[2]) * (double)ir};
        const double v[9] = {-c[0] * c[0], -c[1] * c[1], -c[2] * c[2], -2.0 * c[0] * c[1], -2.0 * c[0] * c[2], -2.0 * c[1] * c[2], c[0], c[1], c[2]};
        for (int t = 0; t < 9; ++t) { _Float16 h, l; pair(v[t], h, l); a[3 * t] = h; a[3 * t + 1] = h; a[3 * t + 2] = l; }
        _Float16 h, l;
        pair((c[0] * c[0] + c[1] * c[1] + c[2] * c[2]) - (double)sp[3] * (double)ir * (double)ir, h, l);
        a[27] = h; a[28] = l;
    }
}

int upload_tri_bounds(const pt_scene_desc *d, double Rorigin) {
    if (R.mesh_mode != MESH_TILES || d->num_meshes <= 0) return PT_OK;
    size_t recs = 0;
    for (int k = 0; k < d->num_meshes; ++k) recs += (size_t)((d->meshes[k].triangle_count + 63) & ~63);
    std::vector<_Float16> tr(std::max<size_t>(recs, 64) * 32, (_Float16)0.0f);
    std::vector<float> sph;
    size_t off = 0;
    for (int k = 0; k < d->num_meshes; ++k) {
        const pt_mesh &m = d->meshes[k];
        const size_t n64 = (size_t)((m.triangle_count + 63) & ~63);
        sph.assign(n64 * 4, 0.0f);
        make_tri_bounds(d->triangles + m.first_triangle, m.triangle_count, Rorigin, sph.data());
        for (size_t i = (size_t)((m.triangle_count + 3) & ~3); i < n64; ++i) sph[i * 4 + 3] = -1.0f;
        float frame[4];
        make_tri_records(sph.data(), (int)n64, tr.data() + off * 32, frame);
        float *r = R.grec_frames.data() + (size_t)m.geom_index * 4;
        for (int a = 0; a < 4; ++a) r[a] = frame[a];
        off += n64;
    }
    if (!R.d_tri_bound || R.tri_bound_words < tr.size() / 2) {
        if (R.d_tri_bound) { HIPCHK(hipStreamSynchronize(R.stream)); (void)hipFree(R.d_tri_bound); R.d_tri_bound = nullptr; }
        HIPCHK(hipMalloc(&R.d_tri_bound, tr.size() * 2));
        R.tri_bound_words = tr.size() / 2;
    }
    HIPCHK(hipMemcpyAsync(R.d_tri_bound, tr.data(), tr.size() * 2, hipMemcpyHostToDevice, R.stream));
    for (int k = 0; k < d->num_meshes; ++k) {
        const int gi = d->meshes[k].geom_index;
        HIPCHK(hipMemcpyAsync(R.d_geoms + (size_t)gi * ptd::GEOM_WORDS + ptd::G_INV + 7, R.grec_frames.data() + (size_t)gi * 4, 16, hipMemcpyHostToDevice, R.stream));
    }
    HIPCHK(hipStreamSynchronize(R.stream));
    R.scene.tri_rec = R.d_tri_bound;
    return PT_OK;
}

}

namespace one {

static int upload_bvh(const pt_scene_desc *d, std::vector<float> &grec) {
    std::vector<float> nodes, btris, tops;
    std::vector<int32_t> mesh_list;
    float prune = 0.0f;
    int guard = 1;
    R.bvh_info = pt_bvh_info{};
    R.mesh_grids.clear();
    std::vector<int> by_geom((size_t)d->num_meshes);
    for (int k = 0; k < d->num_meshes; ++k) by_geom[(size_t)k] = k;
    std::sort(by_geom.begin(), by_geom.end(), [&](int x, int y) { return d->meshes[x].geom_index < d->meshes[y].geom_index; });
    for (int kk = 0; kk < d->num_meshes; ++kk) {
        const int k = by_geom[(size_t)kk];
        const pt_mesh &m = d->meshes[k];
        if (kk > 0 && d->meshes[by_geom[(size_t)kk - 1]].geom_index == m.geom_index)
            return fail(PT_ERR_INVALID, "pt_init: geom %d owns more than one mesh", m.geom_index);
        ptbvh::Tree tree;
        ptbvh::build(reinterpret_cast<const float *>(d->triangles + m.first_triangle), m.triangle_count, tree, (double)R.scene.rmax);
        const int root = (int)(nodes.size() / BVH_NODE_WORDS);
        const int slot0 = (int)(btris.size() / TRI_WORDS);
        if ((int64_t)slot0 + m.triangle_count >= (1 << ptbvh::LINK_BITS) || tree.num_nodes() >= (1 << ptbvh::LINK_BITS))
            return fail(PT_ERR_INVALID, "pt_init: PT_MESH_BVH holds at most 2^24 triangles (record links are 24 bits)");
        for (int n = 0; n < tree.num_nodes(); ++n) {
            float *w = &tree.nodes[(size_t)n * BVH_NODE_WORDS];
            for (int c = 0; c < 2; ++c) {
                uint32_t link;
                memcpy(&link, &w[6 + c], 4);
                if ((link >> ptbvh::LINK_BITS) & ptbvh::INFO_LEAF) { link += (uint32_t)slot0; memcpy(&w[6 + c], &link, 4); }
            }
        }
        nodes.insert(nodes.end(), tree.nodes.begin(), tree.nodes.end());
        for (int s = 0; s < m.triangle_count; ++s) {
            const int32_t orig = m.first_triangle + tree.order[(size_t)s];
            const pt_triangle &t = d->triangles[orig];
            float r[TRI_WORDS] = {t.v0.x, t.v0.y, t.v0.z,
                                  t.v1.x - t.v0.x, t.v1.y - t.v0.y, t.v1.z - t.v0.z,
                                  t.v2.x - t.v0.x, t.v2.y - t.v0.y, t.v2.z - t.v0.z, 0.0f, 0.0f, 0.0f};
            memcpy(&r[9], &orig, 4);
            r[10] = tree.spec_pad;
            btris.insert(btris.end(), r, r + TRI_WORDS);
        }
        float *g = grec.data() + (size_t)m.geom_index * ptd::GEOM_WORDS;
        memcpy(&g[2], &root, 4); memcpy(&g[3], &m.triangle_count, 4);
        for (int a = 0; a < 3; ++a) { g[ptd::G_INV + a] = tree.origin[a]; g[ptd::G_INV + 3 + a] = tree.step[a]; }
        for (int a = 0; a < 3; ++a) R.mesh_grids.push_back(tree.origin[a] - tree.step[a]);
        for (int a = 0; a < 3; ++a) R.mesh_grids.push_back(tree.origin[a] + (float)(ptbvh::GRID_MAX + 1) * tree.step[a]);
        const int share = d->num_meshes <= BVH_TOP ? BVH_TOP / d->num_meshes : 0;
        const int top_cnt = std::min(share, tree.num_nodes()), top_off = (int)(tops.size() / BVH_NODE_WORDS);
        tops.insert(tops.end(), tree.nodes.begin(), tree.nodes.begin() + (size_t)top_cnt * BVH_NODE_WORDS);
        const int32_t entry[4] = {m.geom_index, root, m.triangle_count, top_off | (top_cnt << 16)};
        mesh_list.insert(mesh_list.end(), entry, entry + 4);
        prune = std::max(prune, tree.prune);
        guard = std::max(guard, tree.num_nodes() + 1);
        R.bvh_info.nodes += tree.num_nodes();
        R.bvh_info.triangles += m.triangle_count;
        R.bvh_info.depth = std::max(R.bvh_info.depth, tree.depth);
        R.bvh_info.pad = std::max(R.bvh_info.pad, tree.pad);
    }
    R.bvh_info.prune = prune;
    if (nodes.size() * 4 >= ((size_t)1 << 32))
        return fail(PT_ERR_INVALID, "pt_init: PT_MESH_BVH holds at most 4 GiB of hierarchy records (k_mesh addresses them with 32-bit offsets)");
    if (nodes.empty()) nodes.assign(BVH_NODE_WORDS, 0.0f);
    if (btris.empty()) btris.assign(TRI_WORDS, 0.0f);
    HIPCHK(hipMalloc(&R.d_bvh_nodes, nodes.size() * 4));
    HIPCHK(hipMalloc(&R.d_bvh_tris, btris.size() * 4));
    HIPCHK(hipMemcpy(R.d_bvh_nodes, nodes.data(), nodes.size() * 4, hipMemcpyHostToDevice));
    HIPCHK(hipMemcpy(R.d_bvh_tris, btris.data(), btris.size() * 4, hipMemcpyHostToDevice));
    if (mesh_list.empty()) mesh_list.assign(4, 0);
    HIPCHK(hipMalloc((void **)&R.d_bvh_meshes, mesh_list.size() * 4));
    HIPCHK(hipMemcpy(R.d_bvh_meshes, mesh_list.data(), mesh_list.size() * 4, hipMemcpyHostToDevice));
    R.scene.bvh_meshes = R.d_bvh_meshes; R.scene.bvh_nmesh = d->num_meshes;
    R.scene.bvh_nodes = R.d_bvh_nodes; R.scene.bvh_tris = R.d_bvh_tris;
    R.scene.bvh_top_n = (int)(tops.size() / BVH_NODE_WORDS);
    if (tops.empty()) tops.assign(BVH_NODE_WORDS, 0.0f);
    HIPCHK(hipMalloc(&R.d_bvh_top, tops.size() * 4));
    HIPCHK(hipMemcpy(R.d_bvh_top, tops.data(), tops.size() * 4, hipMemcpyHostToDevice));
    R.scene.bvh_top = R.d_bvh_top;
    R.scene.bvh_prune = prune; R.scene.bvh_guard = guard;
    return PT_OK;
}

static int update_cull0() {
    if (!R.cull0_tiles) return PT_OK;
    hipLaunchKernelGGL(k_cull0_mask, dim3((R.cull0_tiles + WAVES - 1) / WAVES), dim3(BLOCK), 0, R.stream, R.scene, R.cam,
                       R.map, R.trace_depth, R.d_cull0, R.cull0_tiles);
    HIPCHK(hipGetLastError());
    return PT_OK;
}

static int update_cam_mask() {
    R.cam_mask_valid = false;
    if (R.mesh_mode != MESH_BVH || R.map.tile_pixels % TILE != 0 || R.mesh_grids.empty()) return PT_OK;
    const pt_camera &c = R.cam;
    const double M[3][3] = {{c.view.x, -c.right.x, -c.up.x}, {c.view.y, -c.right.y, -c.up.y}, {c.view.z, -c.right.z, -c.up.z}};
    const double det = M[0][0] * (M[1][1] * M[2][2] - M[1][2] * M[2][1]) - M[0][1] * (M[1][0] * M[2][2] - M[1][2] * M[2][0]) +
                       M[0][2] * (M[1][0] * M[2][1] - M[1][1] * M[2][0]);
    if (!(std::fabs(det) > 1e-9) || !(c.pixelLength[0] != 0.0f) || !(c.pixelLength[1] != 0.0f)) return PT_OK;
    double x0 = INFINITY, x1 = -INFINITY, y0 = INFINITY, y1 = -INFINITY;
    for (size_t m = 0; m + 6 <= R.mesh_grids.size(); m += 6) {
        for (int corner = 0; corner < 8; ++corner) {
            const double v[3] = {(double)R.mesh_grids[m + ((corner & 1) ? 3 : 0)] - c.position.x,
                                 (double)R.mesh_grids[m + 1 + ((corner & 2) ? 3 : 0)] - c.position.y,
                                 (double)R.mesh_grids[m + 2 + ((corner & 4) ? 3 : 0)] - c.position.z};
            auto det3 = [](const double A[3][3]) {
                return A[0][0] * (A[1][1] * A[2][2] - A[1][2] * A[2][1]) - A[0][1] * (A[1][0] * A[2][2] - A[1][2] * A[2][0]) +
                       A[0][2] * (A[1][0] * A[2][1] - A[1][1] * A[2][0]);
            };
            double sol[3];
            for (int k = 0; k < 3; ++k) {
                double A[3][3];
                for (int i = 0; i < 3; ++i) for (int j = 0; j < 3; ++j) A[i][j] = (j == k) ? v[i] : M[i][j];
                sol[k] = det3(A) / det;
            }
            const double reach = std::fabs(v[0]) + std::fabs(v[1]) + std::fabs(v[2]);
            if (!(sol[0] > 1e-6 * (reach + 1.0))) return PT_OK;
            const double fx = 0.5 * c.resolution[0] + sol[1] / sol[0] / (double)c.pixelLength[0];
            const double fy = 0.5 * c.resolution[1] + sol[2] / sol[0] / (double)c.pixelLength[1];
            if (!std::isfinite(fx) || !std::isfinite(fy)) return PT_OK;
            x0 = std::min(x0, fx); x1 = std::max(x1, fx); y0 = std::min(y0, fy); y1 = std::max(y1, fy);
        }
    }
    x0 -= 2.0; x1 += 2.0; y0 -= 2.0; y1 += 2.0;
    const uint32_t tps = (uint32_t)R.map.tile_pixels / TILE;
    std::vector<unsigned long long> mask((tps + 63) / 64, 0ull);
    for (uint32_t t = 0; t < tps; ++t) {
        bool any = false;
        for (int k = 0; k < TILE && !any; ++k) {
            const int j = (int)t * TILE + k;
            int pix = j;
            if (R.map.tile_count != 1) {
                const int ly = j / R.map.W, x = j - ly * R.map.W, ls = ly / R.map.strip_rows;
                pix = x + ((ls * R.map.tile_count + R.map.tile_index) * R.map.strip_rows + (ly - ls * R.map.strip_rows)) * R.map.W;
            }
            const int y = pix / R.map.W, x = pix - y * R.map.W;
            any = x >= x0 && x <= x1 && y >= y0 && y <= y1;
        }
        if (any) mask[t >> 6] |= 1ull << (t & 63u);
    }
    if (!R.d_cam_mask) HIPCHK(hipMalloc((void **)&R.d_cam_mask, mask.size() * sizeof(unsigned long long)));
    HIPCHK(hipMemcpy(R.d_cam_mask, mask.data(), mask.size() * sizeof(unsigned long long), hipMemcpyHostToDevice));
    R.cam_mask_valid = true;
    return PT_OK;
}

}
```

project3-cuda-path-tracer_amd/csrc/pt_h_session.hpp:

```cpp
#pragma once

namespace {

constexpr size_t ERR_BYTES = 512;
char g_err[ERR_BYTES] = "";
thread_local char *t_err = g_err;

int fail(int code, const char *fmt, ...) {
    va_list ap;
    va_start(ap, fmt);
    vsnprintf(t_err, ERR_BYTES, fmt, ap);
    va_end(ap);
    return code;
}

#define HIPCHK(expr)                                                                            \
    do {                                                                                        \
        hipError_t e_ = (expr);                                                                 \
        if (e_ != hipSuccess)                                                                   \
            return fail(PT_ERR_DEVICE, "HIP error (%s:%d): %s: %s", __builtin_strrchr(__FILE__, '/') ? __builtin_strrchr(__FILE__, '/') + 1 : __FILE__, __LINE__, #expr, \
                        hipGetErrorString(e_));                                                 \
    } while (0)

constexpr int OV_MAX_LANES = 8;
struct Renderer {
    bool live = false;
    pt_scene_desc desc{};
    pt_camera cam{};
    int trace_depth = 0;
    uint32_t flags = 0;
    int device = 0;
    hipStream_t stream = nullptr;
    bool own_stream = false;
    TileMap map{};
    int npix = 0;
    uint32_t cap = 0;
    int max_batch = 1;
    float *pool_mem[2] = {nullptr, nullptr};
    Pool pool[2]{};
    int cur = 0;
    float *isect_mem = nullptr;
    uint32_t *sort_table = nullptr;
    float *cache_mem = nullptr;
    bool cache_valid = false;
    bool first_hit_enabled = true;
    bool first_hit_refence = false;
    bool first_two_enabled = true;
    uint64_t first_two_launches = 0;
    float *state_mem = nullptr;
    uint32_t *state_ended = nullptr;
    bool first_state_enabled = true;
    uint64_t first_state_launches = 0;
    uint64_t first_hit_fills = 0, first_hit_launches = 0;
    Isect isect{};
    float *final_mem = nullptr;
    uint32_t fin_serial = 0;
    float *image = nullptr;
    bool own_image = false;
    float *d_geoms = nullptr, *d_mats = nullptr, *d_tris = nullptr;
    float *d_cull = nullptr, *d_grec = nullptr;
    float *d_tri_bound = nullptr;
    size_t tri_bound_words = 0;
    std::vector<float> grec_frames;
    uint32_t *d_ginfo = nullptr;
    double cull_eye_reach = 0.0;
    std::vector<pt_geom> geoms_keep;
    std::vector<pt_triangle> tris_keep;
    std::vector<pt_mesh> meshes_keep;
    std::vector<float> grec_keep;
    bool scene_lds = true;
    SceneDev scene{};
    float4 *d_env = nullptr;
    int env_n = 0;
    std::vector<float> env_keep;
    float *d_lights = nullptr;
    int nlights = 0;
    std::vector<float> lamp_rec;
    std::vector<std::vector<float>> tex_keep;
    std::vector<int> tex_n;
    float4 *d_tex = nullptr;
    int2 *d_tex_tab = nullptr;
    int ntex = 0;
    std::vector<std::vector<float>> bump_keep;
    std::vector<int> bump_n;
    ptd::bump_texel *d_bump = nullptr;
    int2 *d_bump_tab = nullptr;
    int nbump = 0;
    size_t lds_bytes = 0;
    Control *ctl = nullptr;
    Persist *persist = nullptr;
    uint32_t *iter_counts = nullptr;
    size_t iter_counts_bytes = 0;
    HostStats *h_stats = nullptr, *d_stats = nullptr;
    bool want_host_stats = false;
    uint32_t host_stats_serial = 0;
    bool self_gathered = false;
    uint32_t *dir_mem = nullptr;
    size_t dir_stride = 0;
    int cur_dir = -1;
    uint32_t max_tiles = 0;
    size_t flag_words = 0;
    size_t ctl_bytes = 0;
    int grid = 0;
    int grid_iter = 0;
    int grid_iter_cur = 0;
    int iter_tpw = 4;
    int iter_wgs_per_cu_all = 15;
    bool ov_lanes_set = false;
    int ov_streams = 2;
    int cus = 0;
    int grid_sort = 0;
    bool sort_wave = true;
    int sort_runs = 1;
    int sort_keys = 0;
    bool sorted_isects = false;
    bool gen_fused = false;
    bool gen_sort = false;
    Lens lens{0, 0.0f, 0.0f};
    uint64_t whole_max_paths = 6000000;
    uint64_t whole_max_host_paths = 16000000;
    bool whole = false;
    struct Bufs {
        float *pool_mem[2]; Pool pool[2]; float *final_mem; Control *ctl; uint32_t *dir_mem;
        float4 *mesh_hit; unsigned long long *mesh_flags[2]; uint32_t *iter_counts;
    };
    struct Lane {
        hipStream_t stream = nullptr;
        Bufs b{};
        hipEvent_t traced = nullptr, gathered = nullptr;
        bool gathered_valid = false;
        hipStream_t la_stream = nullptr;
    } lane[OV_MAX_LANES];
    Lane *lane_cur = nullptr;
    hipStream_t lane_main = nullptr;
    size_t pool_bytes = 0, final_bytes = 0, dir_bytes = 0, mesh_hit_bytes = 0;
    int ov_lanes = 4;
    double ov_budget_gb = 64.0;
    hipEvent_t ov_enter = nullptr;
    bool ov_ready = false;
    bool ov_enabled = true;
    bool ov_ok = false;
    bool ov_active = false;
    int ov_next = 0;
    static constexpr int LA_SLOTS = 4, LA_AHEAD = 3;
    struct LaWindow {
        bool valid = false;
        bool inflight = false;
        int iter0 = 0, count = 0, next = 0;
        uint32_t stamp = 0;
        pt_camera cam{}; int depth = 0; Lens lens{0, 0.0f, 0.0f};
        Control *ctl = nullptr;
        bool masked = false;
    } la[LA_SLOTS];
    int la_cur = 0;
    int la_cus = 24, grid_la = 0, per_cu = 0;
    bool la_masks_ready = false, la_masks_failed = false;
    uint64_t la_masked_windows = 0, la_masked_calls = 0;
    bool la_masked_last = false;
    hipStream_t la_gstream = nullptr;
    hipEvent_t la_rs_event = nullptr;
    bool la_tracing = false;
    uint64_t la_misses = 0, la_windows = 0, la_discards = 0;
    TileGather la_tg{};
    bool la_tiles_ok = false, la_shared_device = false;
    Control *last_ctl = nullptr;
    float *epi_host = nullptr;
    bool epi_done = false;
    bool epi_direct_enabled = true;
    bool defer_enabled = true;
    bool own_enabled = true;
    bool own_form = false;
    bool pool_own = false;
    bool host_sparse_enabled = false;
    uint64_t image_epoch = 0;
    float *host_synced = nullptr;
    uint64_t host_epoch = 0;
    bool epi_enabled = true;
    bool pin_enabled = true;
    int mesh_mode = MESH_NONE;
    float *d_bvh_nodes = nullptr, *d_bvh_tris = nullptr, *d_bvh_top = nullptr;
    std::vector<float> mesh_grids;
    unsigned long long *d_cam_mask = nullptr;
    bool cam_mask_valid = false;
    unsigned long long *d_cull0 = nullptr;
    uint32_t cull0_tiles = 0;
    int4 *d_bvh_meshes = nullptr;
    float4 *mesh_hit = nullptr;
    unsigned long long *mesh_flags[2] = {nullptr, nullptr};
    bool mesh_marked = false;
    int grid_mesh = 0;
    pt_bvh_info bvh_info{};
    struct HostReg { void *ptr; size_t bytes; void *dev; };
    std::vector<HostReg> host_regs;
    float *snap[2] = {nullptr, nullptr};
    hipStream_t copy_stream = nullptr;
    hipEvent_t ev_snap[2] = {nullptr, nullptr}, ev_copied[2] = {nullptr, nullptr};
    uint64_t async_calls = 0;
    hipEvent_t ev_direct[2] = {nullptr, nullptr};
    int direct_k = 0;
    hipEvent_t async_prev = nullptr, dma_last = nullptr;
    bool async_direct_enabled = true;
    unsigned int *dbg_counts = nullptr;
    size_t dbg_words = 0;
    float4 *gb_mem = nullptr;
    bool gb_valid = false;
    pt_camera gb_cam{};
    float *dn_plane[2] = {nullptr, nullptr};
    uint8_t *dn_rgba = nullptr;
    float *dn_result = nullptr;
    uint64_t dn_launches[3] = {0, 0, 0};
    bool alb_on = false, alb_valid = false;
    float *alb_mem = nullptr;
    pt_camera alb_cam{};
    float4 *gb_alt = nullptr, *tp_gb = nullptr;
    bool tp_ready = false, tp_cur = false;
    pt_camera tp_cam{};
    float *tp_c[2] = {nullptr, nullptr}, *tp_n[2] = {nullptr, nullptr};
    int tp_k = 0;
    float *tp_hc = nullptr, *tp_hn = nullptr;
    uint64_t tp_launches[2] = {0, 0};
    void *scratch = nullptr;
    size_t scratch_bytes = 0;
    int step_iter0 = 0, step_count = 0, step_depth = 0;
    bool in_step = false;
    pt_stats stats{};
    bool profiling = false;
    std::vector<hipEvent_t> ev;
    std::vector<int> ev_stage;
    size_t ev_used = 0;
    pt_profile prof{};
};

Renderer g_single;
thread_local Renderer *t_ctx = &g_single;
#define R (*t_ctx)

constexpr size_t EV_PAIRS = 2048;

int drain_events(void) {
    if (R.ev_used == 0) return PT_OK;
    HIPCHK(hipStreamSynchronize(R.stream));
    for (size_t k = 0; k < R.ev_used; ++k) {
        float ms = 0.0f;
        HIPCHK(hipEventElapsedTime(&ms, R.ev[2 * k], R.ev[2 * k + 1]));
        R.prof.ms[R.ev_stage[k] & 0xff] += (double)ms;
        R.prof.launches[R.ev_stage[k] & 0xff] += 1 + (R.ev_stage[k] >> 8);
    }
    R.ev_used = 0;
    return PT_OK;
}

struct StageTimer {
    bool on;
    size_t k;
    StageTimer(int stage) : on(false), k(0) {
        if (!R.profiling) return;
        if (R.ev_used >= EV_PAIRS && drain_events() != PT_OK) return;
        k = R.ev_used++;
        R.ev_stage[k] = stage;
        on = hipEventRecord(R.ev[2 * k], R.stream) == hipSuccess;
    }
    ~StageTimer() { if (on) (void)hipEventRecord(R.ev[2 * k + 1], R.stream); }
    void two_bounces() { if (on) R.ev_stage[k] |= 0x100; }
};

Pool carve_pool(float *mem, uint32_t cap) { return Pool{mem, cap}; }

void make_div_magic(uint32_t d, uint32_t *magic, uint32_t *shift) {
    if (d == 1) { *magic = 0; *shift = 0; return; }
    uint32_t L = 31;
    while (!((d >> L) & 1u)) --L;
    if ((d & (d - 1)) == 0) { *magic = 0; *shift = L - 1; return; }
    const uint64_t num = 1ull << (32 + L);
    uint64_t m = num / d, rem = num % d;
    m += m;
    const uint64_t twice = rem + rem;
    if (twice >= d) m += 1;
    *magic = (uint32_t)(m + 1);
    *shift = L;
}

int tile_rows(int tile_index, int tile_count, int strip_rows, int H) {
    if (tile_count <= 1) return H;
    int rows = 0;
    for (int y = 0; y < H; ++y)
        if ((y / strip_rows) % tile_count == tile_index) rows++;
    return rows;
}

int ensure_isect(void) {
    if (R.isect_mem) return PT_OK;
    HIPCHK(hipMalloc(&R.isect_mem, (size_t)R.cap * 5 * 4));
    R.isect = Isect{R.isect_mem, R.cap};
    return PT_OK;
}

int ensure_scratch(size_t bytes) {
    if (bytes <= R.scratch_bytes) return PT_OK;
    if (R.scratch) (void)hipFree(R.scratch);
    R.scratch = nullptr; R.scratch_bytes = 0;
    HIPCHK(hipMalloc(&R.scratch, bytes));
    R.scratch_bytes = bytes;
    return PT_OK;
}

int session_bounces(void) { return R.trace_depth + (R.nlights > 0 ? 1 : 0); }
bool sky_session(void) { return (R.flags & PT_DIRECT_SKY) && (R.flags & PT_DIRECT_LIGHT) && !(R.flags & PT_FAKE_SHADER); }
int session_bounces_max(int trace_depth) { return trace_depth + ((R.nlights > 0 || sky_session()) ? 1 : 0); }

RangeDir tile_dir(int depth) {
    const uint32_t W = (uint32_t)R.grid * WAVES * (uint32_t)(R.sort_keys > 0 ? R.sort_runs : 1);
    const uint32_t nr = W * (uint32_t)std::max(1, R.sort_keys);
    if (depth < 0) return RangeDir{nullptr, W, nr};
    return RangeDir{R.dir_mem + (size_t)depth * R.dir_stride, W, nr};
}


}
```

project3-cuda-path-tracer_amd/csrc/pt_k_bounce.hpp:

```cpp
#pragma once

namespace {

enum { MODE_FUSED = 0, MODE_ISECT = 1, MODE_CACHE0 = 2, MODE_FIRST2 = 3, MODE_STATE2 = 4 };
constexpr bool mode_first2(int mode) { return mode == MODE_FIRST2 || mode == MODE_STATE2; }

template <typename T>
__device__ __forceinline__ T karg_field(size_t offset) {
    const __attribute__((address_space(4))) char *kp = (const __attribute__((address_space(4))) char *)__builtin_amdgcn_kernarg_segment_ptr();
    asm volatile("" : "+s"(kp));
    return *(const __attribute__((address_space(4))) T *)(kp + offset);
}
template <typename T>
__device__ __forceinline__ T karg_struct(size_t offset) {
    static_assert(sizeof(T) % 4 == 0, "whole dwords");
    const __attribute__((address_space(4))) char *kp = (const __attribute__((address_space(4))) char *)__builtin_amdgcn_kernarg_segment_ptr();
    asm volatile("" : "+s"(kp));
    uint32_t w[sizeof(T) / 4];
#pragma unroll
    for (size_t k = 0; k < sizeof(T) / 4; ++k) w[k] = *(const __attribute__((address_space(4))) uint32_t *)(kp + offset + 4 * k);
    T t;
    __builtin_memcpy(&t, w, sizeof(T));
    return t;
}
__device__ __forceinline__ Pool karg_pool(size_t offset) {
    return Pool{karg_field<float *>(offset + offsetof(Pool, base)), karg_field<uint32_t>(offset + offsetof(Pool, cap))};
}

struct TileCtx {
    bool kargs = false;
    bool kmisc = false;
    bool epi_direct = false;
    SceneAcc acc;
    float *tri_lds;
    int lane, iter0;
    uint32_t stamp;
};

struct TileRegs {
    bool have, active;
    bool miss0;
    uint32_t i, src, tile, pid, smp;
    int pixel;
    f3 col;
    MeshBest mb;
};

template <bool GEN, bool RESOLVE = false, bool OWN = false>
__device__ __forceinline__ void tile_load(const BounceArgs &a, const TileCtx &c, const Pool &in, int depth,
                                          uint32_t tile, uint32_t i, uint32_t src, bool have, bool active,
                                          TileRegs &tr, f3 &ro, f3 &rd, uint32_t &own) {
    own = 0u;
    constexpr bool gen_rays = GEN;
    tr.have = have; tr.i = i; tr.src = src; tr.tile = tile;
    tr.miss0 = false;
    tr.pid = DEAD_PID; tr.smp = 0; tr.pixel = 0;
    tr.col = ptd::mk(1.0f, 1.0f, 1.0f);
    tr.mb.t = FLT_MAX; tr.mb.geom = -1; tr.mb.tri = -1;
    ro = ptd::mk(0, 0, 0); rd = ptd::mk(0, 0, 1);
    if (active) {
        if (gen_rays) {
            tr.pid = i;
        } else {
            const SlotPtr p = (c.kargs ? karg_pool(offsetof(BounceArgs, in)) : in).slot(src);
            tr.pid = ppid(p);
            ro = ptd::mk(pf(p, 0), pf(p, 1), pf(p, 2));
            rd = ptd::mk(pf(p, 3), pf(p, 4), pf(p, 5));
            tr.col = ptd::mk(pf(p, 6), pf(p, 7), pf(p, 8));
            if (tr.pid == DEAD_PID) active = false;
        }
    }
    bool pending = false;
    if (RESOLVE && active) { pending = (tr.pid & PENDING_DIR) != 0u; tr.pid &= ~PENDING_DIR; }
    if (OWN && !GEN && active) { own = (tr.pid & OWN_MASK) >> OWN_SHIFT; tr.pid &= ~OWN_MASK; }
    if (active) {
        if (c.kmisc) {
            const TileMap map = karg_struct<TileMap>(offsetof(BounceArgs, map));
            tr.smp = sample_of(map, tr.pid);
            tr.pixel = local_to_pixel(map, (int)(tr.pid - tr.smp * (uint32_t)map.tile_pixels));
            if (gen_rays) camera_ray(karg_struct<pt_camera>(offsetof(BounceArgs, cam)), karg_struct<Lens>(offsetof(BounceArgs, lens)),
                                     karg_field<int>(offsetof(BounceArgs, trace_depth)), c.iter0 + (int)tr.smp, tr.pixel, map.W, ro, rd);
        } else {
            tr.smp = sample_of(a.map, tr.pid);
            tr.pixel = local_to_pixel(a.map, (int)(tr.pid - tr.smp * (uint32_t)a.map.tile_pixels));
            if (gen_rays) camera_ray(a.cam, a.lens, a.trace_depth, c.iter0 + (int)tr.smp, tr.pixel, a.map.W, ro, rd);
        }
    }
    if (RESOLVE && pending) {
        uint32_t rng = ptd::seeded_engine(c.iter0 + (int)tr.smp, tr.pixel, depth - 1);
        rd = ptd::hemisphere(rd, rng);
    }
    tr.active = active;
}

template <bool OWN, int SH>
__device__ __forceinline__ void tile_first(const BounceArgs &a, const TileCtx &c, TileRegs &tr, f3 &ro, f3 &rd, uint32_t &own) {
    constexpr bool ENV = (SH & SH_ENV) != 0, GLOSSY = (SH & SH_GLOSSY) != 0;
    bool alive = false;
    if (tr.active) {
        const Isect tab = c.kargs ? karg_struct<Isect>(offsetof(BounceArgs, isect)) : a.isect;
        const uint32_t tile_pixels = (uint32_t)(c.kargs ? karg_field<int>(offsetof(BounceArgs, map) + offsetof(TileMap, tile_pixels)) : a.map.tile_pixels);
        const size_t k = tr.pid - tr.smp * tile_pixels;
        const float4 h = *tab.first_hit(k);
        const int2 id = *tab.first_id(k);
        bool deferred = false, missed = false;
        ptd::PathState ps;
        ps.o = ro; ps.d = rd; ps.c = tr.col;
        alive = ptd::shade_scatter<GLOSSY>(ps, h.x, ptd::mk(h.y, h.z, h.w), id.x & 0x7fffffff, (id.x < 0) ? 0 : 1, c.acc.mats,
                                           c.iter0 + (int)tr.smp, tr.pixel, 0, false, false, &deferred, ENV ? &missed : nullptr);
        if (alive) {
            ro = ps.o; rd = ps.d; tr.col = ps.c;
            if (OWN) own = (uint32_t)(id.y + 1);
        } else if (ENV && missed) {
            tr.miss0 = true;
        } else {
            put_final(c.kargs ? karg_field<float *>(offsetof(BounceArgs, fin)) : a.fin, tr.pid, ps.c, c.stamp);
        }
    }
    tr.active = alive;
}

template <bool OWN>
__device__ __forceinline__ void tile_state(const BounceArgs &a, const TileCtx &c, uint32_t tile, uint32_t i, bool have, bool active,
                                           TileRegs &tr, f3 &ro, f3 &rd, uint32_t &own) {
    own = 0u;
    tr.have = have; tr.i = i; tr.src = i; tr.tile = tile;
    tr.miss0 = false;
    tr.pid = DEAD_PID; tr.smp = 0; tr.pixel = 0;
    tr.col = ptd::mk(1.0f, 1.0f, 1.0f);
    tr.mb.t = FLT_MAX; tr.mb.geom = -1; tr.mb.tri = -1;
    ro = ptd::mk(0, 0, 0); rd = ptd::mk(0, 0, 1);
    bool alive = false;
    if (active) {
        tr.pid = i;
        tr.smp = sample_of(a.map, tr.pid);
        const uint32_t k = tr.pid - tr.smp * (uint32_t)a.map.tile_pixels;
        tr.pixel = local_to_pixel(a.map, (int)k);
        const SlotPtr p = Pool{karg_field<float *>(offsetof(BounceArgs, first_state)), 0u}.slot(k);
        const uint32_t word = ppid(p);
        const f3 so = ptd::mk(pf(p, 0), pf(p, 1), pf(p, 2));
        const f3 sd = ptd::mk(pf(p, 3), pf(p, 4), pf(p, 5));
        const f3 sc = ptd::mk(pf(p, 6), pf(p, 7), pf(p, 8));
        const uint32_t kind = word & FS_KIND_MASK;
        if (kind == FS_DIFFUSE || kind == FS_FIXED) {
            alive = true;
            ro = so; rd = sd; tr.col = sc;
            if (OWN) own = (word & OWN_MASK) >> OWN_SHIFT;
            if (kind == FS_DIFFUSE) {
                uint32_t rng = ptd::seeded_engine(c.iter0 + (int)tr.smp, tr.pixel, 0);
                rd = ptd::hemisphere(sd, rng);
            }
        } else if (kind == FS_CONST) {
            put_final(karg_field<float *>(offsetof(BounceArgs, fin)), tr.pid, sc, c.stamp);
        }
    }
    tr.active = alive;
}

__device__ __forceinline__ bool mesh_root_candidate(const int4 *bvh_meshes, int bvh_nmesh, const float *geoms, const float *bvh_nodes, f3 ro, f3 rd) {
    bool cand = false;
#pragma unroll 1
    for (int k = 0; k < bvh_nmesh; ++k) {
        const __attribute__((address_space(4))) int *mrec =
            (const __attribute__((address_space(4))) int *)(unsigned long long)(bvh_meshes + k);
        cfloat *grid = as_const(geoms) + (size_t)mrec[0] * ptd::GEOM_WORDS + ptd::G_INV;
        const __attribute__((address_space(4))) uint32_t *b =
            (const __attribute__((address_space(4))) uint32_t *)(unsigned long long)(bvh_nodes + (size_t)mrec[1] * BVH_NODE_WORDS);
        const BvhRay br = bvh_ray(ro, rd, ptd::mk(grid[0], grid[1], grid[2]), ptd::mk(grid[3], grid[4], grid[5]));
        float tn, tf;
        bvh_slab(br, b[0], b[1], b[2], tn, tf);
        cand |= tn <= tf;
        bvh_slab(br, b[3], b[4], b[5], tn, tf);
        cand |= tn <= tf;
    }
    return cand;
}
__device__ __forceinline__ bool mesh_root_candidate(const SceneDev &sc, f3 ro, f3 rd) {
    return mesh_root_candidate(sc.bvh_meshes, sc.bvh_nmesh, sc.geoms, sc.bvh_nodes, ro, rd);
}

template <bool COMPACT, int MESH = MESH_NONE, bool SORT = false, bool DEFER = false, int SH = 0>
__device__ __forceinline__ void tile_shade(const BounceArgs &a, const TileCtx &c, const Pool &in, const Pool &out, int depth,
                                           const TileRegs &tr, f3 ro, f3 rd, float t, f3 nrm, int mat, int outside,
                                           uint32_t n, uint32_t dst_base, uint32_t &packed, uint32_t &traced,
                                           uint32_t key_stride = 0, uint32_t own_bits = 0, int geom = -1) {
    constexpr bool ENV = (SH & SH_ENV) != 0, GLOSSY = (SH & SH_GLOSSY) != 0, DIRECT = (SH & SH_DIRECT) != 0, TEX = (SH & SH_TEX) != 0;
    static_assert(!(DIRECT && TEX), "pt_init refuses PT_TEXTURES with PT_DIRECT_LIGHT");
    const int lane = c.lane;
    bool alive = false, deferred = false, missed = false;
    ptd::PathState ps;
    ps.o = ro; ps.d = rd; ps.c = tr.col;
    auto end_path = [&]() {
        {
            if (ENV && missed) {
                if (c.kargs || c.kmisc)
                    ps.c = ptd::miss_colour(ps.c, ps.d, karg_field<const float4 *>(offsetof(BounceArgs, env)), karg_field<int>(offsetof(BounceArgs, env_n)));
                else
                    ps.c = ptd::miss_colour(ps.c, ps.d, a.env, a.env_n);
            }
            if (c.epi_direct) {
                if (!(ps.c.x == 0.0f && ps.c.y == 0.0f && ps.c.z == 0.0f)) {
                    float *img = karg_field<float *>(offsetof(BounceArgs, epi_image)) + 3 * (size_t)tr.pixel;
                    const float r = img[0] + ps.c.x, g = img[1] + ps.c.y, b = img[2] + ps.c.z;
                    img[0] = r; img[1] = g; img[2] = b;
                    float *host = karg_field<float *>(offsetof(BounceArgs, epi_host));
                    if (host) { host += 3 * (size_t)tr.pixel; host[0] = r; host[1] = g; host[2] = b; }
                }
            } else {
                put_final((c.kargs || c.kmisc) ? karg_field<float *>(offsetof(BounceArgs, fin)) : a.fin, tr.pid, ps.c, c.stamp);
            }
        }
    };
    if (tr.active) {
        const bool defer = DEFER && (c.kargs ? karg_field<int>(offsetof(BounceArgs, defer_dir)) : a.defer_dir) != 0;
        if constexpr (DIRECT) {
            const float *lights = c.kargs ? karg_field<const float *>(offsetof(BounceArgs, lights)) : a.lights;
            const int nlights = c.kargs ? karg_field<int>(offsetof(BounceArgs, nlights)) : a.nlights;
            if (depth == a.trace_depth) {
                const int target = ptd::direct_target(lights, nlights, c.iter0 + (int)tr.smp, tr.pixel, depth - 1);
                if (ENV && target < 0) {
                    if (!(t > 0.0f)) missed = true;
                    else ps.c = ptd::mk(0.0f, 0.0f, 0.0f);
                } else if (t > 0.0f && geom == target) {
                    const float *m = c.acc.mats + mat * ptd::MAT_WORDS;
                    ps.c = ptd::mul(ps.c, ptd::scale(ptd::mk(m[0], m[1], m[2]), m[9]));
                } else {
                    ps.c = ptd::mk(0.0f, 0.0f, 0.0f);
                }
            } else {
                alive = ptd::shade_scatter<GLOSSY, true>(ps, t, nrm, mat, outside, c.acc.mats, c.iter0 + (int)tr.smp, tr.pixel, depth,
                                                         depth == a.trace_depth - 1, defer, &deferred, ENV ? &missed : nullptr, lights, nlights);
            }
        } else if constexpr (TEX) {
            const int2 *btab = c.kargs ? karg_field<const int2 *>(offsetof(BounceArgs, bump_tab)) : a.bump_tab;
            alive = ptd::shade_scatter_tex<GLOSSY>(ps, t, nrm, mat, outside, c.acc.mats, c.iter0 + (int)tr.smp, tr.pixel, depth,
                                   depth == a.trace_depth - 1, defer, &deferred, ENV ? &missed : nullptr,
                                   geom >= 0 ? c.acc.ginfo[geom] >> 28 : (uint32_t)PT_TRIANGLE_MESH,
                                   c.acc.grec + (size_t)(geom >= 0 ? geom : 0) * GREC_WORDS,
                                   c.kargs ? karg_field<const int2 *>(offsetof(BounceArgs, tex_tab)) : a.tex_tab,
                                   c.kargs ? karg_field<const float4 *>(offsetof(BounceArgs, tex)) : a.tex, btab,
                                   c.kargs ? karg_field<const ptd::bump_texel *>(offsetof(BounceArgs, bumps)) : a.bumps);
        } else {
            alive = ptd::shade_scatter<GLOSSY>(ps, t, nrm, mat, outside, c.acc.mats, c.iter0 + (int)tr.smp, tr.pixel, depth,
                                   depth == a.trace_depth - 1, defer, &deferred, ENV ? &missed : nullptr);
        }
        if (!ENV && !alive) end_path();
    }
    const uint64_t bal = ballot64(alive);
    const uint64_t act = ballot64(tr.active);
    traced += (uint32_t)__popcll((unsigned long long)act);
    uint32_t dst = tr.i;
    if (COMPACT && SORT) {
        for_each_key(alive, (uint32_t)mat, [&](uint32_t k, uint64_t m) {
            const uint32_t have = (uint32_t)__builtin_amdgcn_readlane((int)packed, (int)k);
            if (alive && (uint32_t)mat == k) dst = k * key_stride + dst_base + have + rank_below(m);
            if ((uint32_t)lane == k) packed += (uint32_t)__popcll((unsigned long long)m);
        });
    } else if (COMPACT) {
        dst = dst_base + packed + rank_below(bal);
        packed += (uint32_t)__popcll((unsigned long long)bal);
    }
    if (alive) {
        const SlotPtr p = (c.kargs ? karg_pool(offsetof(BounceArgs, out)) : out).slot(dst);
        pf(p, 0) = ps.o.x; pf(p, 1) = ps.o.y; pf(p, 2) = ps.o.z;
        pf(p, 3) = ps.d.x; pf(p, 4) = ps.d.y; pf(p, 5) = ps.d.z;
        pf(p, 6) = ps.c.x; pf(p, 7) = ps.c.y; pf(p, 8) = ps.c.z;
        ppid(p) = (deferred ? (tr.pid | PENDING_DIR) : tr.pid) | own_bits;
        if (MESH == MESH_PRE) {
            constexpr size_t SC = offsetof(BounceArgs, scene);
            const bool reach = c.kargs
                ? mesh_root_candidate(karg_field<const int4 *>(SC + offsetof(SceneDev, bvh_meshes)), karg_field<int>(SC + offsetof(SceneDev, bvh_nmesh)),
                                      karg_field<const float *>(SC + offsetof(SceneDev, geoms)), karg_field<const float *>(SC + offsetof(SceneDev, bvh_nodes)), ps.o, ps.d)
                : mesh_root_candidate(a.scene, ps.o, ps.d);
            if (reach)
                atomicOr(&(c.kargs ? karg_field<unsigned long long *>(offsetof(BounceArgs, mesh_flags_out)) : a.mesh_flags_out)[dst >> 6], 1ull << (dst & 63u));
        }
    } else if (!COMPACT && tr.have && tr.i < n) {
        out.pid(dst) = DEAD_PID;
    }
    if (ENV && tr.active && !alive) end_path();
}

template <bool COMPACT, int MESH, bool SORT = false, bool DEFER = false, bool OWN = false, int SH = 0, bool FIRST = false>
__device__ __forceinline__ void tile_finish(const BounceArgs &a, const TileCtx &c, const WaveQ &q, int par, const Pool &in,
                                            const Pool &out, int depth, const TileRegs &tr, uint32_t n, uint32_t dst_base,
                                            uint32_t &packed, uint32_t &traced, uint32_t key_stride = 0) {
    const float *ry = q.rays(par) + c.lane;
    const f3 ro = ptd::mk(ry[0], ry[64], ry[128]);
    const f3 rd = ptd::mk(ry[192], ry[256], ry[320]);
    float t = -1.0f; f3 nrm = ptd::mk(0, 0, 0); int mat = 0, outside = 1;
    int geom = -1;
    if (tr.active) tile_result(q, par, c.acc, a.scene.tris, tr.mb, t, nrm, mat, outside, geom);
    tile_shade<COMPACT, MESH, SORT, DEFER, SH>(a, c, in, out, depth, tr, ro, rd, t, nrm, mat, outside, n, dst_base, packed, traced, key_stride,
                                           OWN ? (uint32_t)(geom + 1) << OWN_SHIFT : 0u, geom);
    if constexpr (FIRST && (SH & SH_ENV) != 0) {
        if (tr.miss0)
            put_final(karg_field<float *>(offsetof(BounceArgs, fin)), tr.pid,
                      ptd::miss_colour(tr.col, rd, karg_field<const float4 *>(offsetof(BounceArgs, env)), karg_field<int>(offsetof(BounceArgs, env_n))), c.stamp);
    }
}

struct WgSpans {
    uint32_t p1, p2, p3, total;
    uint32_t b0, b1, b2, b3;
};

template <int MODE, bool COMPACT, int MESH, bool GEN, bool SORT = false, bool DEFER = false, bool RESOLVE = false, bool OWN = false, int SH = 0>
__device__ __forceinline__ void run_tiles(const BounceArgs &a, const TileCtx &c, WaveQ &q, const Pool &in, const Pool &out,
                                          int depth, uint32_t first_tile, uint32_t count, uint32_t tiles,
                                          uint32_t n, bool packed_in, uint32_t span_in, uint32_t &cur, uint32_t dst_base,
                                          bool own_span, const WgSpans &ws, uint32_t &packed, uint32_t &traced,
                                          uint32_t key_stride = 0, bool aligned = false) {
    const int lane = c.lane;
    bool pending = false;
    TileRegs prev{};
    uint32_t prev_ticket = 0;
    int par = 0;
    const bool masked = MODE == MODE_FUSED && GEN && a.cull0 != nullptr;
    uint32_t mtile = masked ? first_tile % a.cull0_tiles : 0u;
    const uint32_t *ended = MODE == MODE_STATE2 ? a.first_ended : nullptr;
    uint32_t etile = ended ? first_tile % a.first_ended_tiles : 0u;
    for (uint32_t r = 0; r < count; ++r) {
        const uint32_t tile = first_tile + r;
        if (!own_span && tile >= tiles) break;
        if (MODE == MODE_STATE2 && ended) {
            const uint32_t whole = ((const __attribute__((address_space(4))) uint32_t *)(unsigned long long)ended)[etile];
            if (++etile == a.first_ended_tiles) etile = 0;
            if (whole) continue;
        }
        rotate_priority(r + (uint32_t)depth, PT_MIN_WAVES + 1);
        unsigned long long gmask = 0;
        if (masked) {
            gmask = ((const __attribute__((address_space(4))) unsigned long long *)(unsigned long long)a.cull0)[mtile];
            if (++mtile == a.cull0_tiles) mtile = 0;
        }
        bool have, active;
        uint32_t i, src;
        if (own_span) {
            const uint32_t L = tile * TILE + lane;
            have = true; active = L < ws.total;
            uint32_t off = L, b = ws.b0;
            if (L >= ws.p1) { off = L - ws.p1; b = ws.b1; }
            if (L >= ws.p2) { off = L - ws.p2; b = ws.b2; }
            if (L >= ws.p3) { off = L - ws.p3; b = ws.b3; }
            src = b + off; i = src;
        } else if (aligned) {
            have = tile < tiles;
            active = false; i = 0; src = 0;
            if (have) {
                const uint32_t *tb = a.dir_in.tbase();
                while (tile >= tb[cur + 1]) ++cur;
                const uint32_t t64 = (tile - tb[cur]) * TILE + (uint32_t)lane;
                active = t64 < a.dir_in.count()[cur];
                src = cur * span_in + t64;
                i = a.dir_in.base()[cur] + t64;
            }
        } else {
            have = tile < tiles;
            i = tile * TILE + lane;
            active = have && i < n;
            src = i;
            if (packed_in && have) src = resolve_src(a.dir_in, span_in, cur, i, active, a.ctl);
        }
        TileRegs tr;
        f3 ro, rd;
        uint32_t own;
        if constexpr (MODE == MODE_STATE2) {
            tile_state<OWN>(a, c, tile, i, have, active, tr, ro, rd, own);
            if (ballot64(tr.active) == 0) continue;
        } else {
            tile_load<GEN, RESOLVE, OWN>(a, c, in, depth, tile, i, src, have, active, tr, ro, rd, own);
        }
        if (MODE == MODE_FIRST2) tile_first<OWN, SH>(a, c, tr, ro, rd, own);
        if (MODE == MODE_FUSED || mode_first2(MODE)) {
            const float4 *pre_hit = nullptr;
            if (MESH == MESH_PRE && tr.active) {
                unsigned long long *fl = c.kargs ? karg_field<unsigned long long *>(offsetof(BounceArgs, mesh_flags_in)) : a.mesh_flags_in;
                const unsigned long long word = fl[src >> 6];
                if ((word >> (src & 63u)) & 1ull) pre_hit = (c.kargs ? karg_field<float4 *>(offsetof(BounceArgs, mesh_hit)) : a.mesh_hit) + src;
                if (word != 0ull && (uint32_t)lane == (uint32_t)__builtin_ctzll((unsigned long long)ballot64(tr.active))) fl[src >> 6] = 0ull;
            }
            cull_scene<MESH, OWN>(a.scene, c.acc, q, par, c.tri_lds, tr.active, ro, rd, tr.mb, pre_hit, masked, gmask,
                                  (OWN && (!GEN || mode_first2(MODE))) ? own_surface_miss(c.acc, own, ro, rd) : 0xffffffffu);
            const uint32_t ticket = q.total;
            if (pending) {
                drain_to(q, c.acc, prev_ticket);
                tile_finish<COMPACT, MESH, SORT, DEFER, OWN, SH, MODE == MODE_FIRST2>(a, c, q, par ^ 1, in, out, depth, prev, n, dst_base, packed, traced, key_stride);
            }
            prev = tr; prev_ticket = ticket; pending = true; par ^= 1;
        } else if (MODE == MODE_CACHE0) {
            float t = -1.0f; f3 nrm = ptd::mk(0, 0, 0); int mat = 0, outside = 1, geom = -1;
            if (tr.active) {
                const size_t k = tr.pid - tr.smp * (uint32_t)a.map.tile_pixels;
                const float4 h = *a.isect.first_hit(k);
                const int2 id = *a.isect.first_id(k);
                t = h.x; nrm = ptd::mk(h.y, h.z, h.w);
                mat = id.x & 0x7fffffff; outside = (id.x < 0) ? 0 : 1; geom = id.y;
            }
            tile_shade<COMPACT, MESH_NONE, false, DEFER, SH>(a, c, in, out, depth, tr, ro, rd, t, nrm, mat, outside, n, dst_base, packed, traced, 0,
                                                             OWN ? (uint32_t)(geom + 1) << OWN_SHIFT : 0u, geom);
        } else {
            float t = -1.0f; f3 nrm = ptd::mk(0, 0, 0); int mat = 0, outside = 1;
            if (tr.active) {
                const uint32_t k = i;
                t = at(a.isect.plane(0), k);
                nrm = ptd::mk(at(a.isect.plane(1), k), at(a.isect.plane(2), k), at(a.isect.plane(3), k));
                const int m = at(a.isect.mat(), k);
                mat = m & 0x7fffffff; outside = (m < 0) ? 0 : 1;
            }
            tile_shade<COMPACT, MESH_NONE, false, DEFER, SH>(a, c, in, out, depth, tr, ro, rd, t, nrm, mat, outside, n, dst_base, packed, traced);
        }
    }
    if (pending) {
        drain_to(q, c.acc, prev_ticket);
        tile_finish<COMPACT, MESH, SORT, DEFER, OWN, SH, MODE == MODE_FIRST2>(a, c, q, par ^ 1, in, out, depth, prev, n, dst_base, packed, traced, key_stride);
    }
}

#ifdef PT_WAVE_TIMES
__device__ unsigned long long g_wave_times[8][8192][2];
__device__ uint32_t g_wave_hw[8][8192];
#endif

template <int MODE, bool COMPACT, int MESH, bool SLDS, bool GEN = false, bool SORT = false, bool OWN = false, int SH = 0>
__global__ __launch_bounds__(BLOCK, MESH == MESH_TILES ? PT_LOOP_WAVES : (MESH == MESH_PRE && PT_PRE_WAVES > PT_MIN_WAVES) ? PT_PRE_WAVES : (SORT && MODE == MODE_FUSED && MESH == MESH_NONE) ? PT_SORT_WAVES : ((MODE == MODE_FUSED || MODE == MODE_CACHE0 || mode_first2(MODE)) && COMPACT && MESH == MESH_NONE && !SORT && PT_FUSED_WAVES > PT_MIN_WAVES) ? PT_FUSED_WAVES : PT_MIN_WAVES) void k_bounce(BounceArgs a) {
    static_assert(!OWN || ((MODE == MODE_FUSED || MODE == MODE_CACHE0 || mode_first2(MODE)) && COMPACT && MESH == MESH_NONE && !SORT),
                  "own-surface form: the plain fused compacting kernel, or the table form of its bounce 0");
    static_assert(!mode_first2(MODE) || (COMPACT && MESH == MESH_NONE && GEN && !SORT), "MODE_FIRST2 / MODE_STATE2: the plain compacting pipeline's first launch");
    static_assert(MODE != MODE_STATE2 || SH == 0, "MODE_STATE2: sessions without environment map or lobes");
#ifdef PT_WAVE_TIMES
    const unsigned long long wt0 = __builtin_amdgcn_s_memrealtime();
#endif
    extern __shared__ __attribute__((aligned(16))) float lds_raw[];
    uint32_t *sctl = reinterpret_cast<uint32_t *>(lds_raw);
    const LdsCarve lc = carve_lds(lds_raw, a.scene, SLDS);
    TileCtx c;
#ifndef PT_NO_KARG_RELOAD
    c.kargs = MESH != MESH_TILES;
#endif
    c.tri_lds = lc.tri;
#ifdef PT_STAMPS
#define STAMP(k) do { if (blockIdx.x == 0 && threadIdx.x == 0 && a.depth == PT_STAMPS) a.ctl->stamp[k] = __builtin_amdgcn_s_memrealtime(); } while (0)
#else
#define STAMP(k) do {} while (0)
#endif
    STAMP(0);
    c.acc = stage_scene<SLDS>(lc.scene, a.scene);
    STAMP(1);
    WaveQ q{lc.pw, 0, 0};
    const int lane = threadIdx.x & 63;
    c.lane = lane;
    const uint32_t Wp = gridDim.x * WAVES;
    constexpr bool DEFER = COMPACT && MESH == MESH_NONE && !SORT && MODE != MODE_ISECT;
    constexpr bool RESOLVE = MODE == MODE_FUSED && COMPACT && MESH == MESH_NONE && !SORT && !GEN;
    const uint32_t W = (SORT && COMPACT) ? a.dir_out.W : Wp;
    const uint32_t runs_per_wave = (SORT && COMPACT) ? W / Wp : 1u;
    const uint32_t wid0 = run_id();
    c.iter0 = a.iter0;
    c.stamp = a.fin_stamp;
    const uint32_t n = (COMPACT && !GEN) ? a.ctl->nlive[a.depth] : a.pool_n;
    const bool packed_in = COMPACT && !GEN && a.dir_in.mem != nullptr;
    constexpr bool ALIGNED = PT_ALIGNED_TILES && MODE == MODE_FUSED && COMPACT && !GEN && !SORT;
    const bool aligned = ALIGNED && packed_in;
    const uint32_t tiles = aligned ? a.dir_in.tbase()[a.dir_in.nr] : (n + TILE - 1) / TILE;
    const uint32_t R = (tiles + W - 1) / W;
    const uint32_t span_in = packed_in ? *a.dir_in.span() : 0;
    uint32_t traced = 0;
    if (GEN && blockIdx.x == 0 && threadIdx.x == 0) a.ctl->nlive[0] = a.pool_n;
    for (uint32_t j = 0; j < runs_per_wave; ++j) {
        const uint32_t wid = j * Wp + wid0;
        uint32_t packed = 0;
        uint32_t cur = 0;
        if (packed_in && wid * R < tiles)
            cur = aligned ? find_range(a.dir_in.tbase(), a.dir_in.nr, wid * R) : find_range(a.dir_in.base(), a.dir_in.nr, wid * R * TILE);
        STAMP(2);
        run_tiles<MODE, COMPACT, MESH, GEN, SORT, DEFER, RESOLVE, OWN, SH>(a, c, q, a.in, a.out, a.depth, wid * R, R, tiles, n, packed_in, span_in,
                                                  cur, wid * R * TILE, false, WgSpans{}, packed, traced, W * R * TILE, aligned);
        if (COMPACT) {
            if (SORT) {
                if ((uint32_t)lane * W < a.dir_out.nr)
                    __hip_atomic_store(&a.dir_out.count()[(uint32_t)lane * W + wid], packed, __ATOMIC_RELAXED, __HIP_MEMORY_SCOPE_AGENT);
            } else if (lane == 0)
                __hip_atomic_store(&a.dir_out.count()[wid], packed, __ATOMIC_RELAXED, __HIP_MEMORY_SCOPE_AGENT);
        }
    }
    const uint32_t wid = wid0;
    STAMP(6);
#ifdef PT_WAVE_TIMES
    if (lane == 0 && a.depth < 8 && wid < 8192) {
        g_wave_times[a.depth][wid][0] = wt0; g_wave_times[a.depth][wid][1] = __builtin_amdgcn_s_memrealtime();
        uint32_t xcc, hwid;
        asm volatile("s_getreg_b32 %0, hwreg(HW_REG_XCC_ID)" : "=s"(xcc));
        asm volatile("s_getreg_b32 %0, hwreg(HW_REG_HW_ID)" : "=s"(hwid));
        g_wave_hw[a.depth][wid] = (xcc & 0xf) | (hwid << 4);
    }
#endif
    if (mode_first2(MODE)) {
        if (blockIdx.x == 0 && threadIdx.x == 0) a.ctl->alive[0] = n;
        if (lane == 0) sctl[8 + (threadIdx.x >> 6)] = traced;
        __syncthreads();
        if (threadIdx.x == 0) {
            const uint32_t tb = sctl[8] + sctl[9] + sctl[10] + sctl[11];
            if (tb) { atomicAdd(&a.ctl->nlive[1], tb); atomicAdd(&a.ctl->alive[1], tb); }
        }
    } else if (COMPACT) {
        if (blockIdx.x == 0 && threadIdx.x == 0) a.ctl->alive[a.depth] = n;
    } else {
        if (lane == 0) sctl[8 + (threadIdx.x >> 6)] = traced;
        __syncthreads();
        if (threadIdx.x == 0) {
            const uint32_t tb = sctl[8] + sctl[9] + sctl[10] + sctl[11];
            if (tb) atomicAdd(&a.ctl->alive[a.depth], tb);
        }
    }

    if (COMPACT) {
        asm volatile("s_waitcnt vmcnt(0)" ::: "memory");
        __syncthreads();
        if (threadIdx.x == 0) {
            const bool last = elect_last(a.ctl->bucket[a.depth][0], &a.ctl->done[a.depth]);
            if (last) {
                __builtin_amdgcn_fence(__ATOMIC_ACQUIRE, "agent");
                asm volatile("s_waitcnt vmcnt(0)" ::: "memory");
            }
            sctl[0] = last ? 1u : 0u;
        }
        __syncthreads();
        STAMP(7);
        if (sctl[0]) {
            const unsigned long long t0 = __builtin_amdgcn_s_memrealtime();
            scan_range_counts(a.dir_out, &a.ctl->nlive[a.depth + 1], sctl + 16, R * TILE, PT_ALIGNED_TILES && !SORT);
            if (threadIdx.x == 0) a.ctl->scan_ticks[a.depth] = (uint32_t)(__builtin_amdgcn_s_memrealtime() - t0);
#ifdef PT_STAMPS
            if (threadIdx.x == 0 && a.depth == PT_STAMPS) { a.ctl->stamp[8] = t0; a.ctl->stamp[9] = __builtin_amdgcn_s_memrealtime(); }
#endif
        }
    }
}

__device__ __forceinline__ void fold_iter_counts(const uint32_t *counts, uint32_t G, int depth, Control *ctl, Persist *per, HostStats *hs,
                                                 uint32_t iterations, uint32_t serial, uint32_t *lds ) {
    constexpr int PER_PASS = BLOCK / 32;
    unsigned long long rays = 0;
    uint32_t first = 0;
    for (int d0 = 0; d0 < depth; d0 += PER_PASS) {
        const int d = d0 + (int)(threadIdx.x >> 5);
        uint32_t sum = 0;
        if (d < depth)
            for (uint32_t b = threadIdx.x & 31u; b < G; b += 32u)
                sum += __hip_atomic_load(&counts[(uint32_t)d * G + b], __ATOMIC_RELAXED, __HIP_MEMORY_SCOPE_AGENT);
        for (int off = 16; off > 0; off >>= 1) sum += __shfl_down(sum, off, 32);
        if ((threadIdx.x & 31u) == 0) lds[threadIdx.x >> 5] = sum;
        __syncthreads();
        if (threadIdx.x == 0)
            for (int k = 0; k < PER_PASS && d0 + k < depth; ++k) {
                const uint32_t tot = lds[k];
                ctl->alive[d0 + k] = tot;
                if (hs) hs->alive[d0 + k] = tot;
                rays += tot;
                if (d0 + k == 0) first = tot;
            }
        __syncthreads();
    }
    if (threadIdx.x == 0) {
        atomicAdd(&per->rays, rays);
        atomicAdd(&per->iterations, (unsigned long long)iterations);
        atomicAdd(&per->first_rays, (unsigned long long)first);
        if (hs) {
            for (int d = depth; d <= MAX_DEPTH; ++d) hs->alive[d] = 0;
            hs->error = 0;
            __hip_atomic_store(&hs->serial, serial, __ATOMIC_RELEASE, __HIP_MEMORY_SCOPE_SYSTEM);
        }
    }
}

template <bool SLDS, int SH = 0>
__global__ __launch_bounds__(BLOCK, PT_ITER_WAVES) void k_iteration(BounceArgs a) {
    extern __shared__ __attribute__((aligned(16))) float lds_raw[];
    const LdsCarve lc = carve_lds(lds_raw, a.scene, SLDS);
    TileCtx c;
#ifndef PT_NO_KARG_RELOAD
    c.kmisc = true;
#endif
    c.tri_lds = nullptr;
    c.epi_direct = a.epi_direct != 0;
    c.acc = stage_scene<SLDS>(lc.scene, a.scene);
    WaveQ q{lc.pw, 0, 0};
    const int lane = threadIdx.x & 63;
    c.lane = lane;
    const uint32_t W = gridDim.x * WAVES;
    const uint32_t wid = run_id();
    c.iter0 = a.iter0;
    c.stamp = a.fin_stamp;
    const uint32_t n = a.pool_n;
    const uint32_t tiles = (n + TILE - 1) / TILE;
    const uint32_t R = range_tiles(n, W);
    const uint32_t base = wid * R * TILE;
    if (blockIdx.x == 0 && threadIdx.x == 0) a.ctl->nlive[0] = n;
    Pool in = a.in, out = a.out;
    uint32_t cur = 0;
    uint32_t *xcnt = reinterpret_cast<uint32_t *>(lds_raw);
    const int wave = threadIdx.x >> 6;
    WgSpans ws{};
    ws.b0 = (0u * gridDim.x + blockIdx.x) * R * TILE; ws.b1 = (1u * gridDim.x + blockIdx.x) * R * TILE;
    ws.b2 = (2u * gridDim.x + blockIdx.x) * R * TILE; ws.b3 = (3u * gridDim.x + blockIdx.x) * R * TILE;
    static_assert(WAVES == 4, "four spans per workgroup");
    for (int d = 0; d < a.trace_depth; ++d) {
        uint32_t traced = 0, packed = 0;
        if (d == 0) {
            run_tiles<MODE_FUSED, true, MESH_NONE, true, false, false, false, false, SH>(a, c, q, in, out, 0, wid * R, R, tiles, n, false, 0, cur, base, false, ws,
                                                         packed, traced);
        } else {
            const uint32_t wg_tiles = (ws.total + TILE - 1) / TILE;
            const uint32_t per = (wg_tiles + WAVES - 1) / WAVES;
            const uint32_t first = (uint32_t)wave * per;
            const uint32_t mine = first < wg_tiles ? min(per, wg_tiles - first) : 0u;
            run_tiles<MODE_FUSED, true, MESH_NONE, false, false, false, false, false, SH>(a, c, q, in, out, d, first, mine, tiles, n, false, 0, cur, base, true, ws,
                                                          packed, traced);
        }
        uint32_t *slot = xcnt + (d & 1) * (2 * WAVES);
        if (lane == 0) { slot[wave] = packed; slot[WAVES + wave] = traced; }
        __builtin_amdgcn_fence(__ATOMIC_ACQ_REL, "workgroup");
        asm volatile("s_waitcnt vmcnt(0) lgkmcnt(0)" ::: "memory");
        __syncthreads();
        const uint32_t c0 = slot[0], c1 = slot[1], c2 = slot[2], c3 = slot[3];
        ws.p1 = c0; ws.p2 = c0 + c1; ws.p3 = c0 + c1 + c2; ws.total = c0 + c1 + c2 + c3;
        if (threadIdx.x == 0)
            __hip_atomic_store(&karg_field<uint32_t *>(offsetof(BounceArgs, iter_counts))[(uint32_t)d * gridDim.x + blockIdx.x],
                               slot[WAVES] + slot[WAVES + 1] + slot[WAVES + 2] + slot[WAVES + 3], __ATOMIC_RELAXED, __HIP_MEMORY_SCOPE_AGENT);
        if (ws.total == 0) {
            if ((int)threadIdx.x > d && (int)threadIdx.x < karg_field<int>(offsetof(BounceArgs, trace_depth)))
                __hip_atomic_store(&karg_field<uint32_t *>(offsetof(BounceArgs, iter_counts))[threadIdx.x * gridDim.x + blockIdx.x], 0u,
                                   __ATOMIC_RELAXED, __HIP_MEMORY_SCOPE_AGENT);
            break;
        }
        const Pool tmp = in; in = out; out = tmp;
    }
    float *const epi_image = karg_field<float *>(offsetof(BounceArgs, epi_image));
    if (epi_image && !c.epi_direct) {
        asm volatile("s_waitcnt vmcnt(0)" ::: "memory");
        float *const epi_host = karg_field<float *>(offsetof(BounceArgs, epi_host));
        const float *const fin = karg_field<float *>(offsetof(BounceArgs, fin));
        const TileMap map = karg_struct<TileMap>(offsetof(BounceArgs, map));
        float *tr = lc.pw;
        for (uint32_t r = 0; r < R; ++r) {
            const uint32_t tile = wid * R + r;
            if (tile >= tiles) break;
            const uint32_t j = tile * TILE + lane;
            float cx = 0.0f, cy = 0.0f, cz = 0.0f;
            if (j < n) {
                const float *f = fin + (size_t)j * 4;
                if (__float_as_uint(__hip_atomic_load(f + 3, __ATOMIC_RELAXED, __HIP_MEMORY_SCOPE_AGENT)) == c.stamp) {
                    cx = __hip_atomic_load(f, __ATOMIC_RELAXED, __HIP_MEMORY_SCOPE_AGENT);
                    cy = __hip_atomic_load(f + 1, __ATOMIC_RELAXED, __HIP_MEMORY_SCOPE_AGENT);
                    cz = __hip_atomic_load(f + 2, __ATOMIC_RELAXED, __HIP_MEMORY_SCOPE_AGENT);
                }
            }
            tr[3 * lane] = cx; tr[3 * lane + 1] = cy; tr[3 * lane + 2] = cz;
            __builtin_amdgcn_fence(__ATOMIC_ACQ_REL, "wavefront");
#pragma unroll
            for (int k = 0; k < 3; ++k) {
                const uint32_t w = (uint32_t)k * TILE + lane;
                const uint32_t jl = w / 3u;
                const uint32_t jj = tile * TILE + jl;
                if (jj < n) {
                    const size_t idx = (size_t)local_to_pixel(map, (int)jj) * 3 + (w - jl * 3u);
                    const float v = epi_image[idx] + tr[w];
                    epi_image[idx] = v;
                    if (epi_host) epi_host[idx] = v;
                }
            }
            __builtin_amdgcn_fence(__ATOMIC_ACQ_REL, "wavefront");
        }
    }
    if (epi_image) {
        asm volatile("s_waitcnt vmcnt(0)" ::: "memory");
        __syncthreads();
        if (threadIdx.x == 0) {
            const bool last = elect_last_self_clearing(karg_field<Control *>(offsetof(BounceArgs, ctl))->ticket);
            if (last) {
                __builtin_amdgcn_fence(__ATOMIC_ACQUIRE, "agent");
                asm volatile("s_waitcnt vmcnt(0)" ::: "memory");
            }
            xcnt[0] = last ? 1u : 0u;
        }
        __syncthreads();
        if (xcnt[0])
            fold_iter_counts(karg_field<uint32_t *>(offsetof(BounceArgs, iter_counts)), gridDim.x, karg_field<int>(offsetof(BounceArgs, trace_depth)),
                             karg_field<Control *>(offsetof(BounceArgs, ctl)), karg_field<Persist *>(offsetof(BounceArgs, persist)),
                             karg_field<HostStats *>(offsetof(BounceArgs, host_stats)),
                             n / (uint32_t)karg_field<int>(offsetof(BounceArgs, map) + offsetof(TileMap, tile_pixels)), c.stamp, xcnt + 4);
    }
}

}
```

project3-cuda-path-tracer_amd/csrc/pt_types.hpp:

```cpp
#pragma once

namespace {


#ifndef PT_MIN_WAVES
#define PT_MIN_WAVES 4
#endif
#ifndef PT_FUSED_WAVES
#define PT_FUSED_WAVES 6
#endif
#ifndef PT_ISECT_WAVES
#define PT_ISECT_WAVES 4
#endif
#ifndef PT_PRE_WAVES
#define PT_PRE_WAVES 6
#endif
#ifndef PT_ITER_WAVES
#define PT_ITER_WAVES PT_MIN_WAVES
#endif
#ifndef PT_SORT_WAVES
#define PT_SORT_WAVES 6
#endif
#ifndef PT_LOOP_WAVES
#define PT_LOOP_WAVES 3
#endif
constexpr int BLOCK = 256;
constexpr int WAVES = BLOCK / 64;
constexpr int TILE = 64;
constexpr int TRI_WORDS = 12;
constexpr int BVH_NODE_WORDS = 16;
enum { MESH_NONE = 0, MESH_TILES = 1, MESH_BVH = 2, MESH_PRE = 3 };
constexpr int MAX_DEPTH = 64;
constexpr uint32_t DEAD_PID = 0xffffffffu;
constexpr uint32_t PENDING_DIR = 0x80000000u;
constexpr int OWN_SHIFT = 26;
constexpr uint32_t OWN_MASK = 0xfu << OWN_SHIFT;
constexpr int OWN_MAX_GEOMS = 15;
constexpr uint64_t OWN_MAX_PATHS = 1ull << OWN_SHIFT;
inline bool own_surface_plan(uint64_t paths, int ngeoms, bool plain_fused) {
    return plain_fused && ngeoms >= 1 && ngeoms <= OWN_MAX_GEOMS && paths <= OWN_MAX_PATHS;
}

template <typename T>
__device__ __forceinline__ T &at(T *plane, uint32_t i) {
    return *reinterpret_cast<T *>(reinterpret_cast<char *>(plane) + (i << 2));
}

#ifndef PT_POOL_QUADS
#define PT_POOL_QUADS 1
#endif
#if PT_POOL_QUADS
struct SlotPtr { char *q, *c; };
struct Pool {
    float *base;
    uint32_t cap;
    __device__ __forceinline__ SlotPtr slot(uint32_t s) const {
        char *t = reinterpret_cast<char *>(base) + (size_t)(s >> 6) * 2560u;
        return SlotPtr{t + ((s & 63u) << 4), t + 2048u + ((s & 63u) << 3)};
    }
    __device__ __forceinline__ float &f(uint32_t s, int k) const {
        const SlotPtr p = slot(s);
        return *reinterpret_cast<float *>(k < 8 ? p.q + (k >> 2) * 1024 + (k & 3) * 4 : p.c);
    }
    __device__ __forceinline__ uint32_t &pid(uint32_t s) const { return *reinterpret_cast<uint32_t *>(slot(s).c + 4); }
};
__device__ __forceinline__ float &pf(const SlotPtr &p, int k) { return *reinterpret_cast<float *>(k < 8 ? p.q + (k >> 2) * 1024 + (k & 3) * 4 : p.c); }
__device__ __forceinline__ uint32_t &ppid(const SlotPtr &p) { return *reinterpret_cast<uint32_t *>(p.c + 4); }
#else
typedef char *SlotPtr;
struct Pool {
    float *base;
    uint32_t cap;
    __device__ __forceinline__ char *slot(uint32_t s) const {
        return reinterpret_cast<char *>(base) + (size_t)(s >> 6) * 2560u + ((s & 63u) << 3);
    }
    __device__ __forceinline__ float &f(uint32_t s, int k) const { return *reinterpret_cast<float *>(slot(s) + (k >> 1) * 512 + (k & 1) * 4); }
    __device__ __forceinline__ uint32_t &pid(uint32_t s) const { return *reinterpret_cast<uint32_t *>(slot(s) + 4 * 512 + 4); }
};
__device__ __forceinline__ float &pf(char *slot, int k) { return *reinterpret_cast<float *>(slot + (k >> 1) * 512 + (k & 1) * 4); }
__device__ __forceinline__ uint32_t &ppid(char *slot) { return *reinterpret_cast<uint32_t *>(slot + 4 * 512 + 4); }
#endif

struct Isect {
    float *base;
    uint32_t cap;
    __device__ __forceinline__ float *plane(int k) const { return base + (size_t)k * cap; }
    __device__ __forceinline__ int *mat() const { return reinterpret_cast<int *>(base + (size_t)4 * cap); }
    __device__ __forceinline__ float4 *first_hit(size_t k) const { return reinterpret_cast<float4 *>(base) + k; }
    __device__ __forceinline__ int2 *first_id(size_t k) const { return reinterpret_cast<int2 *>(base + (size_t)4 * cap) + k; }
    static constexpr size_t FIRST_HIT_BYTES = 24;
};

struct TileMap {
    int W, H;
    int tile_index, tile_count, strip_rows;
    int tile_pixels;
    uint32_t div_magic;
    uint32_t div_shift;
};

__device__ __forceinline__ uint32_t sample_of(const TileMap &m, uint32_t pid) {
    if (m.tile_pixels == 1) return pid;
    const uint32_t q = __umulhi(m.div_magic, pid);
    return (((pid - q) >> 1) + q) >> m.div_shift;
}

struct TileGather {
    uint32_t magic, shift, skip, first;
};

struct Control {
    uint32_t keep[16];
    unsigned long long stamp[16];
    uint32_t nlive[MAX_DEPTH + 1];
    uint32_t alive[MAX_DEPTH + 1];
    uint32_t done[MAX_DEPTH];
    uint32_t done_sort[MAX_DEPTH];
    uint32_t error;
    uint32_t scan_ticks[MAX_DEPTH];
    uint32_t pad[512 - 16 - 32 - 2 * (MAX_DEPTH + 1) - 3 * MAX_DEPTH - 1];
    uint32_t bucket[MAX_DEPTH][2][32 * 16];
    uint32_t ticket[33 * 16];
};
constexpr int ELECT_BUCKETS = 32;
static_assert(offsetof(Control, ticket) == 2048 + 2 * MAX_DEPTH * 32 * 16 * 4, "Control up to `ticket` is one memset block");
static_assert(sizeof(Control) % 16 == 0, "memset block is a multiple of 16 B");

__device__ __forceinline__ bool elect_last(uint32_t *buckets , uint32_t *top) {
    const uint32_t G = gridDim.x;
    const uint32_t k = blockIdx.x % ELECT_BUCKETS;
    const uint32_t members = (G - k + ELECT_BUCKETS - 1) / ELECT_BUCKETS;
    const uint32_t used = G < ELECT_BUCKETS ? G : ELECT_BUCKETS;
    const uint32_t old = __hip_atomic_fetch_add(&buckets[k * 16], 1u, __ATOMIC_RELAXED, __HIP_MEMORY_SCOPE_AGENT);
    if (old != members - 1) return false;
    const uint32_t t = __hip_atomic_fetch_add(top, 1u, __ATOMIC_RELAXED, __HIP_MEMORY_SCOPE_AGENT);
    return t == used - 1;
}

__device__ __forceinline__ bool elect_last_self_clearing(uint32_t *ticket ) {
    const uint32_t G = gridDim.x;
    const uint32_t k = blockIdx.x % ELECT_BUCKETS;
    const uint32_t members = (G - k + ELECT_BUCKETS - 1) / ELECT_BUCKETS;
    const uint32_t used = G < ELECT_BUCKETS ? G : ELECT_BUCKETS;
    const uint32_t old = __hip_atomic_fetch_add(&ticket[k * 16], 1u, __ATOMIC_RELAXED, __HIP_MEMORY_SCOPE_AGENT);
    if (old != members - 1) return false;
    __hip_atomic_store(&ticket[k * 16], 0u, __ATOMIC_RELAXED, __HIP_MEMORY_SCOPE_AGENT);
    const uint32_t t = __hip_atomic_fetch_add(&ticket[32 * 16], 1u, __ATOMIC_RELAXED, __HIP_MEMORY_SCOPE_AGENT);
    if (t != used - 1) return false;
    __hip_atomic_store(&ticket[32 * 16], 0u, __ATOMIC_RELAXED, __HIP_MEMORY_SCOPE_AGENT);
    return true;
}

#ifndef PT_ALIGNED_TILES
#define PT_ALIGNED_TILES 1
#endif
struct RangeDir {
    uint32_t *mem;
    uint32_t W;
    uint32_t nr;
    __device__ __forceinline__ uint32_t *count() const { return mem; }
    __device__ __forceinline__ uint32_t *base() const { return mem + ((nr + 3u) & ~3u); }
    __device__ __forceinline__ uint32_t *tbase() const { return mem + 2u * ((nr + 3u) & ~3u) + 4u; }
    __device__ __forceinline__ uint32_t *span() const { return mem + 3u * ((nr + 3u) & ~3u) + 8u; }
};
__host__ __device__ constexpr size_t range_dir_words(size_t nr) { return 3u * ((nr + 3u) & ~(size_t)3u) + 12u; }

__device__ __forceinline__ uint32_t run_id() {
    return __builtin_amdgcn_readfirstlane((threadIdx.x >> 6) * gridDim.x + blockIdx.x);
}

__host__ __device__ __forceinline__ uint32_t range_tiles(uint32_t n, uint32_t W) {
    const uint32_t tiles = (n + 63u) / 64u;
    return (tiles + W - 1) / W;
}

struct Persist {
    unsigned long long rays;
    unsigned long long iterations;
    unsigned long long first_rays;
};

struct HostStats {
    uint32_t alive[MAX_DEPTH + 1];
    uint32_t error;
    uint32_t serial;
};

struct Lens {
    int aa;
    float radius, focal;
};

struct SceneDev {
    const float *geoms;  int ngeoms;
    const float *cull;
    const float *grec;
    const uint32_t *ginfo;
    float rmax;
    const float *mats;   int nmats;
    const float *tris;   int ntris;
    const void *tri_rec;
    const float *bvh_nodes;
    const float *bvh_tris;
    float bvh_prune;  int bvh_guard;
    const int4 *bvh_meshes; int bvh_nmesh;
    const float *bvh_top;  int bvh_top_n;
};

struct BounceArgs {
    unsigned int *dbg_counts;
    Pool in, out;
    Lens lens;
    Isect isect;
    SceneDev scene;
    TileMap map;
    Control *ctl;
    RangeDir dir_in;
    RangeDir dir_out;
    float *fin;
    uint32_t fin_stamp;
    pt_camera cam;
    int depth, trace_depth, iter0;
    uint32_t pool_n;
    int gen_rays;
    float4 *mesh_hit;
    unsigned long long *mesh_flags_in, *mesh_flags_out;
    int mesh_scan;
    const unsigned long long *cam_mask;
    const unsigned long long *cull0;
    uint32_t cull0_tiles;
    float *epi_image, *epi_host;
    int epi_direct;
    uint32_t *iter_counts;
    Persist *persist;
    HostStats *host_stats;
    uint32_t *sort_table;
    int nbins;
    int defer_dir;
    const float4 *env;
    int env_n;
    const float *lights;
    int nlights;
    const float4 *tex;
    const int2 *tex_tab;
    const ptd::bump_texel *bumps;
    const int2 *bump_tab;
    float *first_state;
    const uint32_t *first_ended;
    uint32_t first_ended_tiles;
};

enum : uint32_t { FS_ZERO = 0, FS_CONST = 1, FS_DIFFUSE = 2, FS_FIXED = 3, FS_KIND_MASK = 3 };
__host__ __device__ constexpr size_t first_state_bytes(size_t tile_pixels) { return ((tile_pixels + 63) / 64) * 2560; }

enum : int {
    SH_ENV = 1,
    SH_GLOSSY = 2,
    SH_DIRECT = 4,
    SH_TEX = 8
};

struct RayGen {
    pt_camera cam;
    Lens lens;
    TileMap map;
    int trace_depth, iter0;
};

__device__ __forceinline__ int local_to_pixel(const TileMap &m, int j) {
    if (m.tile_count == 1) return j;
    int ly = j / m.W;
    int x = j - ly * m.W;
    int ls = ly / m.strip_rows;
    int y = (ls * m.tile_count + m.tile_index) * m.strip_rows + (ly - ls * m.strip_rows);
    return x + y * m.W;
}

__device__ __forceinline__ void camera_ray(const pt_camera &cam, const Lens &lens, int trace_depth, int iter,
                                           int pix, int W, f3 &ro, f3 &rd) {
    const int y = pix / W;
    const int x = pix - y * W;
    f3 view = ptd::mk(cam.view.x, cam.view.y, cam.view.z);
    f3 right = ptd::mk(cam.right.x, cam.right.y, cam.right.z);
    f3 up = ptd::mk(cam.up.x, cam.up.y, cam.up.z);
    f3 pos = ptd::mk(cam.position.x, cam.position.y, cam.position.z);
    float fx = (float)x, fy = (float)y;
    uint32_t rng = 0;
    if (lens.aa || lens.radius > 0.0f) rng = ptd::seeded_engine(iter, pix, trace_depth);
    if (lens.aa) {
        fx = fx + (ptd::u01(rng) - 0.5f);
        fy = fy + (ptd::u01(rng) - 0.5f);
    }
    f3 a = ptd::scale(ptd::scale(right, cam.pixelLength[0]), (fx - (float)cam.resolution[0] * 0.5f));
    f3 b = ptd::scale(ptd::scale(up, cam.pixelLength[1]), (fy - (float)cam.resolution[1] * 0.5f));
    ro = pos;
    rd = ptd::normalize(ptd::sub(ptd::sub(view, a), b));
    if (lens.radius > 0.0f) {
        const float ft = lens.focal / ptd::dot(rd, view);
        const f3 focus = ptd::add(pos, ptd::scale(rd, ft));
        const float r = lens.radius * __builtin_sqrtf(ptd::u01(rng));
        const float theta = ptd::u01(rng) * 6.2831853071795864769252867665590057683943f;
        float sa, ca;
        ptd::sincos_shared(theta, sa, ca);
        ro = ptd::add(ptd::add(pos, ptd::scale(right, r * ca)), ptd::scale(up, r * sa));
        rd = ptd::normalize(ptd::sub(focus, ro));
    }
}

}
```

project3-cuda-path-tracer_amd/csrc/ptmi355.hip:

```cpp
#include <hip/hip_runtime.h>

#include <algorithm>
#include <atomic>
#include <cfloat>
#include <cmath>
#include <cstdarg>
#include <cstdio>
#include <cstdlib>
#include <cstring>
#include <type_traits>
#include <vector>

#include "../../include/ptmi355.h"
#include "pt_device.hpp"

static_assert(sizeof(pt_vec3) == 12 && sizeof(pt_mat4) == 64 && sizeof(pt_ray) == 24, "ABI");
static_assert(sizeof(pt_geom) == 236 && offsetof(pt_geom, transform) == 44 &&
              offsetof(pt_geom, inverseTransform) == 108 && offsetof(pt_geom, invTranspose) == 172, "Geom ABI");
static_assert(sizeof(pt_material) == 44 && offsetof(pt_material, hasReflective) == 28 &&
              offsetof(pt_material, emittance) == 40, "Material ABI");
static_assert(sizeof(pt_camera) == 84 && offsetof(pt_camera, view) == 32 &&
              offsetof(pt_camera, pixelLength) == 76, "Camera ABI");
static_assert(sizeof(pt_path_segment) == 44 && offsetof(pt_path_segment, pixelIndex) == 36, "PathSegment ABI");
static_assert(sizeof(pt_shadeable_intersection) == 20 && offsetof(pt_shadeable_intersection, materialId) == 16,
              "ShadeableIntersection ABI");
static_assert(sizeof(pt_triangle) == 36, "triangle ABI");

using ptd::f3;

static inline const char *pt_experiment(const char *name) {
#ifdef PT_EXPERIMENTS
    return getenv(name);
#else
    (void)name;
    return nullptr;
#endif
}

#include "pt_types.hpp"
#include "pt_bvh.hpp"
#include "pt_cull.hpp"
#include "pt_lights.hpp"
#include "pt_kernels.hpp"

#include "pt_h_session.hpp"
#include "pt_h_enqueue.hpp"
#include "pt_h_image.hpp"
#include "pt_h_api.hpp"
#include "pt_h_denoise.hpp"


#include "pt_probe.hpp"
#include "pt_multi.hpp"

extern "C" int ptdbg_counts(unsigned int *out, int words) {
    if (!g_single.live || !g_single.dbg_counts || words < 0 || (size_t)words > g_single.dbg_words) return -1;
    if (hipStreamSynchronize(g_single.stream) != hipSuccess) return -1;
    if (hipMemcpy(out, g_single.dbg_counts, (size_t)words * 4, hipMemcpyDeviceToHost) != hipSuccess) return -1;
    if (hipMemset(g_single.dbg_counts, 0, g_single.dbg_words * 4) != hipSuccess) return -1;
    return words;
}

extern "C" int ptdbg_lookahead(unsigned long long out[4]) {
    if (G.live) {
        for (int k = 0; k < 4; ++k) out[k] = 0;
        for (auto &wp : G.w) {
            const Renderer &c = wp->ctx;
            out[0] += c.la_windows; out[1] += c.la_misses; out[2] += c.la_discards;
        }
        const Renderer &c0 = G.w[0]->ctx;
        out[3] = c0.la[c0.la_cur].valid ? (unsigned long long)c0.la[c0.la_cur].count : 0ull;
        return 0;
    }
    if (!g_single.live) return -1;
    out[0] = g_single.la_windows; out[1] = g_single.la_misses; out[2] = g_single.la_discards;
    out[3] = g_single.la[g_single.la_cur].valid ? (unsigned long long)g_single.la[g_single.la_cur].count : 0ull;
    return 0;
}

extern "C" int ptdbg_lookahead_masked(unsigned long long out[2]) {
    if (G.live) {
        out[0] = 0; out[1] = 0;
        for (auto &wp : G.w) { out[0] += wp->ctx.la_masked_windows; out[1] += wp->ctx.la_masked_calls; }
        return 0;
    }
    if (!g_single.live) return -1;
    out[0] = g_single.la_masked_windows; out[1] = g_single.la_masked_calls;
    return 0;
}

extern "C" int ptdbg_first_hit(unsigned long long out[2]) {
    if (G.live) {
        out[0] = 0; out[1] = 0;
        for (auto &wp : G.w) { out[0] += wp->ctx.first_hit_fills; out[1] += wp->ctx.first_hit_launches; }
        return 0;
    }
    if (!g_single.live) return -1;
    out[0] = g_single.first_hit_fills; out[1] = g_single.first_hit_launches;
    return 0;
}

extern "C" int ptdbg_first_two(unsigned long long out[1]) {
    if (G.live) {
        out[0] = 0;
        for (auto &wp : G.w) out[0] += wp->ctx.first_two_launches;
        return 0;
    }
    if (!g_single.live) return -1;
    out[0] = g_single.first_two_launches;
    return 0;
}

extern "C" int ptdbg_first_state(unsigned long long out[1]) {
    if (G.live) {
        out[0] = 0;
        for (auto &wp : G.w) out[0] += wp->ctx.first_state_launches;
        return 0;
    }
    if (!g_single.live) return -1;
    out[0] = g_single.first_state_launches;
    return 0;
}

extern "C" int ptdbg_denoise(unsigned long long out[3]) {
    if (!g_single.live) return -1;
    for (int k = 0; k < 3; ++k) out[k] = g_single.dn_launches[k];
    return 0;
}

extern "C" int ptdbg_denoise_times(const pt_denoise_params *params, int iter, int reps, float *ms) {
    if (G.live) return fail(PT_ERR_INVALID, "ptdbg_denoise_times: single-device sessions");
    return one::denoise_times(params, iter, reps, ms);
}

extern "C" int ptdbg_temporal(unsigned long long out[2]) {
    if (!g_single.live) return -1;
    for (int k = 0; k < 2; ++k) out[k] = g_single.tp_launches[k];
    return 0;
}

extern "C" int ptdbg_temporal_times(const pt_denoise_params *params, const pt_temporal_params *temporal, int iter, int reps, float *ms) {
    if (G.live) return fail(PT_ERR_INVALID, "ptdbg_temporal_times: single-device sessions");
    return one::temporal_times(params, temporal, iter, reps, ms);
}

#ifdef PT_WAVE_TIMES
extern "C" int ptdbg_wave_times(unsigned long long *times , uint32_t *hw ) {
    if (hipMemcpyFromSymbol(times, HIP_SYMBOL(g_wave_times), sizeof(unsigned long long) * 8 * 8192 * 2) != hipSuccess) return -1;
    if (hipMemcpyFromSymbol(hw, HIP_SYMBOL(g_wave_hw), sizeof(uint32_t) * 8 * 8192) != hipSuccess) return -1;
    return 0;
}
#endif
```

Baseline: 65740.

## Drop paths that cannot reach an emitter before the final bounce

```diff
diff --git a/profiles/aimed_last/count_aimed.py b/profiles/aimed_last/count_aimed.py
--- /dev/null
+++ b/profiles/aimed_last/count_aimed.py
@@ -0,0 +1,37 @@
+import json
+import os
+import sys
+
+ROOT = os.path.dirname(os.path.dirname(os.path.dirname(os.path.abspath(__file__))))
+sys.path.insert(0, ROOT)
+sys.path.insert(0, os.path.join(ROOT, "tests"))
+import __graft_entry__ as ge
+import aimed_model as am
+from oracle import pyoracle as po
+
+
+def main(paths, iterations):
+    pt = ge.load_package()
+    for path in paths:
+        scn = pt.load_scene(path)
+        w, h = scn.resolution
+        for it in iterations:
+            s = am.survey(pt, po, scn.geoms, scn.materials, scn.camera, scn.traceDepth, it)
+            n = max(s.n, 1)
+            out = {"scene": os.path.relpath(path, ROOT), "frame": [w, h], "depth": scn.traceDepth, "iteration": it,
+                   "emitters": s.emitters, "survivors_of_bounce_D-2": s.n, "aimed": int(s.aimed.sum()),
+                   "aimed_share": float(s.aimed.sum()) / n, "wild": int(s.wild.sum()), "score_at_last_bounce": int(s.score.sum()),
+                   "score_share": float(s.score.sum()) / n, "scoring_but_not_aimed": int(s.unsafe.sum()),
+                   "tiles_of_64": s.tiles, "tiles_without_aimed_lane": s.tiles_unaimed,
+                   "tiles_without_aimed_lane_share": float(s.tiles_unaimed) / max(s.tiles, 1)}
+            print(json.dumps(out), flush=True)
+
+
+if __name__ == "__main__":
+    args = sys.argv[1:]
+    its = (1, 2)
+    if "--iterations" in args:
+        k = args.index("--iterations")
+        its = tuple(int(x) for x in args[k + 1].split(","))
+        del args[k:k + 2]
+    main(args or [os.path.join(ROOT, "scenes", n) for n in ("cornell.txt", "cornell_glass.txt", "cornell_4k.txt")], its)
diff --git a/profiles/aimed_last/regs_diff.py b/profiles/aimed_last/regs_diff.py
--- /dev/null
+++ b/profiles/aimed_last/regs_diff.py
@@ -0,0 +1,61 @@
+#!/usr/bin/env python3
+import re
+import sys
+
+KEYS = ("vgpr_count", "sgpr_count", "vgpr_spill_count", "sgpr_spill_count", "private_segment_fixed_size", "group_segment_fixed_size")
+
+
+def metadata(path):
+    out, cur = {}, None
+    with open(path, errors="replace") as f:
+        for line in f:
+            if line.startswith("  - .agpr_count") or line.startswith("  - .args"):
+                cur = {}
+            elif cur is not None:
+                m = re.match(r"\s+\.(\w+):\s+(\S+)", line)
+                if m and m.group(1) in KEYS:
+                    cur[m.group(1)] = m.group(2)
+                elif m and m.group(1) == "name":
+                    cur["name"] = m.group(2)
+                elif m and m.group(1) == "wavefront_size":
+                    if "name" in cur:
+                        out[cur["name"]] = tuple(cur.get(k, "?") for k in KEYS)
+                    cur = None
+    return out
+
+
+def split_aim(name):
+    m = re.match(r"(.*8k_bounceI(?:L[ib]\d+E){8})Li(\d)E(E.*)$", name)
+    return (m.group(1) + m.group(3), int(m.group(2))) if m else (name, None)
+
+
+def main(parent, this):
+    p, t = metadata(parent), metadata(this)
+    changed, new, same = [], [], 0
+    for name, row in sorted(t.items()):
+        base, aim = split_aim(name)
+        if aim in (1, 2):
+            new.append((name, aim, row, p.get(base)))
+            continue
+        old = p.get(base if aim == 0 else name)
+        if old is None:
+            changed.append((name, None, row))
+        elif old != row:
+            changed.append((name, old, row))
+        else:
+            same += 1
+    gone = [n for n in p if n not in t and n not in {split_aim(x)[0] for x in t}]
+    print("columns: " + " ".join(KEYS))
+    print("kernels with the parent's numbers: %d; changed or without a parent: %d; in the parent only: %d" % (same, len(changed), len(gone)))
+    for name, old, row in changed:
+        print("CHANGED %s\n   parent %s\n   this   %s" % (name, old, row))
+    for n in gone:
+        print("GONE %s" % n)
+    print("\nthe AIM instantiations (1 writer, 2 reader) beside the parent's plain kernel:")
+    for name, aim, row, old in new:
+        print("AIM=%d %s\n   plain  %s\n   aimed  %s" % (aim, name, old, row))
+    return 1 if changed or gone else 0
+
+
+if __name__ == "__main__":
+    sys.exit(main(sys.argv[1], sys.argv[2]))
diff --git a/project3-cuda-path-tracer_amd/csrc/pt_h_api.hpp b/project3-cuda-path-tracer_amd/csrc/pt_h_api.hpp
--- a/project3-cuda-path-tracer_amd/csrc/pt_h_api.hpp
+++ b/project3-cuda-path-tracer_amd/csrc/pt_h_api.hpp
@@ -211,6 +211,8 @@
     if (const char *e = pt_experiment("PTMI355_FIRST_TWO")) R.first_two_enabled = atoi(e) != 0;
     R.first_state_enabled = true;
     if (const char *e = pt_experiment("PTMI355_FIRST_STATE")) R.first_state_enabled = atoi(e) != 0;
+    R.aimed_last_enabled = true;
+    if (const char *e = pt_experiment("PTMI355_AIMED_LAST")) R.aimed_last_enabled = atoi(e) != 0;
     R.host_sparse_enabled = (d->flags & (PT_HOST_SPARSE | PT_SHARED_IMAGE)) != 0;
     if (const char *e = pt_experiment("PTMI355_ASYNC_DIRECT")) R.async_direct_enabled = atoi(e) != 0;
     R.pin_enabled = true;
@@ -336,6 +338,7 @@
     R.mesh_mode = MESH_NONE;
     for (int i = 0; i < d->num_geoms; ++i)
         if (d->geoms[i].type == PT_TRIANGLE_MESH) R.mesh_mode = (d->flags & PT_MESH_BVH) ? MESH_BVH : MESH_TILES;
+    make_emitter_list(d);
     R.geoms_keep.assign(d->geoms, d->geoms + d->num_geoms);
     if (d->num_triangles > 0) R.tris_keep.assign(d->triangles, d->triangles + d->num_triangles);
     R.desc.geoms = R.geoms_keep.data();
@@ -447,6 +450,14 @@
                 HIPCHK(hipOccupancyMaxActiveBlocksPerMultiprocessor(&n, f, BLOCK, R.lds_bytes));
                 per_cu = std::min(per_cu, n);
             }
+            if constexpr (SH == 0) {
+                if (own && R.aim_valid)
+                    for (int k = 0; k < 4; ++k) {
+                        int n = 0;
+                        HIPCHK(hipOccupancyMaxActiveBlocksPerMultiprocessor(&n, (const void *)aimed_fn(R.scene_lds, (k & 1) != 0, (k & 2) ? AIM_READER : AIM_WRITER), BLOCK, R.lds_bytes));
+                        per_cu = std::min(per_cu, n);
+                    }
+            }
             return PT_OK;
         };
         int rc = size_for(std::integral_constant<int, 0>{});
diff --git a/project3-cuda-path-tracer_amd/csrc/pt_h_enqueue.hpp b/project3-cuda-path-tracer_amd/csrc/pt_h_enqueue.hpp
--- a/project3-cuda-path-tracer_amd/csrc/pt_h_enqueue.hpp
+++ b/project3-cuda-path-tracer_amd/csrc/pt_h_enqueue.hpp
@@ -33,6 +33,8 @@
     a.lights = R.d_lights; a.nlights = R.nlights;
     if (R.ntex + R.nbump > 0) { a.tex = R.d_tex; a.tex_tab = R.d_tex_tab; }
     if (R.nbump > 0) { a.bumps = R.d_bump; a.bump_tab = R.d_bump_tab; }
+    a.aim_n = R.aim_n;
+    for (int k = 0; k < AIM_MAX; ++k) a.aim_geom[k] = R.aim_geom[k];
     return a;
 }
 
@@ -142,6 +144,15 @@
     if (slds) return gen ? (const void *)k_bounce<MODE_FUSED, true, MESH, true, true, false, false, SH> : (const void *)k_bounce<MODE_FUSED, true, MESH, true, false, false, false, SH>;
     return gen ? (const void *)k_bounce<MODE_FUSED, true, MESH, false, true, false, false, SH> : (const void *)k_bounce<MODE_FUSED, true, MESH, false, false, false, false, SH>;
 }
+typedef void (*BounceKernel)(BounceArgs);
+BounceKernel aimed_fn(bool slds, bool own, int aim) {
+    if (aim == AIM_WRITER) {
+        if (own) return slds ? k_bounce<MODE_FUSED, true, MESH_NONE, true, false, false, true, 0, AIM_WRITER> : k_bounce<MODE_FUSED, true, MESH_NONE, false, false, false, true, 0, AIM_WRITER>;
+        return slds ? k_bounce<MODE_FUSED, true, MESH_NONE, true, false, false, false, 0, AIM_WRITER> : k_bounce<MODE_FUSED, true, MESH_NONE, false, false, false, false, 0, AIM_WRITER>;
+    }
+    if (own) return slds ? k_bounce<MODE_FUSED, true, MESH_NONE, true, false, false, true, 0, AIM_READER> : k_bounce<MODE_FUSED, true, MESH_NONE, false, false, false, true, 0, AIM_READER>;
+    return slds ? k_bounce<MODE_FUSED, true, MESH_NONE, true, false, false, false, 0, AIM_READER> : k_bounce<MODE_FUSED, true, MESH_NONE, false, false, false, false, 0, AIM_READER>;
+}
 #define PT_SHADE_DISPATCH_WITH(EXTRA, ...)                                                                  \
     do {                                                                                                    \
         switch ((a.env_n ? SH_ENV : 0) | ((R.flags & PT_GLOSSY) ? SH_GLOSSY : 0)) {                         \
@@ -180,6 +191,12 @@
             return;
         }
     }
+    if constexpr (MODE == MODE_FUSED && COMPACT && MESH == MESH_NONE && !GEN) {
+        if (R.aim_form != AIM_NONE) {
+            hipLaunchKernelGGL(aimed_fn(R.scene_lds, R.own_form, R.aim_form), dim3(R.grid), dim3(BLOCK), R.lds_bytes, R.stream, a);
+            return;
+        }
+    }
     if constexpr ((MODE == MODE_FUSED || MODE == MODE_CACHE0 || mode_first2(MODE)) && COMPACT && MESH == MESH_NONE) {
         if (R.own_form) {
             if (R.scene_lds) launch_k_bounce<MODE, COMPACT, MESH, true, GEN, false, true>(a);
@@ -210,6 +227,7 @@
 int enqueue_bounce(int depth, bool may_fuse = false) {
     BounceArgs a = bounce_args(depth);
     R.own_form = false;
+    R.aim_form = AIM_NONE;
     const bool compact = (R.flags & PT_COMPACT) != 0;
     const bool sort2 = (R.flags & PT_SORT_MATERIAL) && R.sort_keys == 0;
     const bool unfused = (R.flags & PT_UNFUSED) != 0 || sort2;
@@ -272,6 +290,11 @@
     }
     a.defer_dir = (compact && !unfused && R.mesh_mode == MESH_NONE && R.sort_keys == 0 && depth + 1 < R.trace_depth &&
                    R.defer_enabled) ? 1 : 0;
+    if (may_fuse && compact && !unfused && R.mesh_mode == MESH_NONE && R.sort_keys == 0 && !(R.flags & (PT_GLOSSY | PT_FAKE_SHADER)) &&
+        a.env_n == 0 && a.nlights == 0 && a.tex_tab == nullptr && R.trace_depth >= 4 && R.aim_valid && R.aimed_last_enabled && !cached0) {
+        if (depth == R.trace_depth - 2) { R.aim_form = AIM_WRITER; a.defer_dir = 0; R.aimed_last_launches++; }
+        else if (depth == R.trace_depth - 1) R.aim_form = AIM_READER;
+    }
     R.own_form = own_surface_plan((uint64_t)a.pool_n, R.scene.ngeoms,
                                   compact && !unfused && R.mesh_mode == MESH_NONE && R.sort_keys == 0 &&
                                   R.own_enabled);
diff --git a/project3-cuda-path-tracer_amd/csrc/pt_h_scene.hpp b/project3-cuda-path-tracer_amd/csrc/pt_h_scene.hpp
--- a/project3-cuda-path-tracer_amd/csrc/pt_h_scene.hpp
+++ b/project3-cuda-path-tracer_amd/csrc/pt_h_scene.hpp
@@ -43,6 +43,16 @@
     R.scene.cull = R.d_cull;
     R.cull_eye_reach = std::fabs(eye[0]) + std::fabs(eye[1]) + std::fabs(eye[2]);
     return upload_tri_bounds(d, (double)R.scene.rmax);
+}
+
+void make_emitter_list(const pt_scene_desc *d) {
+    R.aim_valid = true; R.aim_n = 0;
+    for (int k = 0; k < AIM_MAX; ++k) R.aim_geom[k] = 0;
+    for (int i = 0; i < d->num_geoms; ++i) {
+        if (!(d->materials[d->geoms[i].materialid].emittance > 0.0f)) continue;
+        if (d->geoms[i].type == PT_TRIANGLE_MESH || R.aim_n == AIM_MAX) { R.aim_valid = false; R.aim_n = 0; return; }
+        R.aim_geom[R.aim_n++] = i;
+    }
 }
 
 void make_tri_bounds(const pt_triangle *tris, int count, double Rorigin, float *out) {
diff --git a/project3-cuda-path-tracer_amd/csrc/pt_h_session.hpp b/project3-cuda-path-tracer_amd/csrc/pt_h_session.hpp
--- a/project3-cuda-path-tracer_amd/csrc/pt_h_session.hpp
+++ b/project3-cuda-path-tracer_amd/csrc/pt_h_session.hpp
@@ -51,6 +51,11 @@
     uint32_t *state_ended = nullptr;
     bool first_state_enabled = true;
     uint64_t first_state_launches = 0;
+    bool aim_valid = false;
+    int aim_n = 0, aim_geom[AIM_MAX] = {0, 0, 0, 0};
+    bool aimed_last_enabled = true;
+    int aim_form = AIM_NONE;
+    uint64_t aimed_last_launches = 0;
     uint64_t first_hit_fills = 0, first_hit_launches = 0;
     Isect isect{};
     float *final_mem = nullptr;
diff --git a/project3-cuda-path-tracer_amd/csrc/pt_k_bounce.hpp b/project3-cuda-path-tracer_amd/csrc/pt_k_bounce.hpp
--- a/project3-cuda-path-tracer_amd/csrc/pt_k_bounce.hpp
+++ b/project3-cuda-path-tracer_amd/csrc/pt_k_bounce.hpp
@@ -179,7 +179,7 @@
     return mesh_root_candidate(sc.bvh_meshes, sc.bvh_nmesh, sc.geoms, sc.bvh_nodes, ro, rd);
 }
 
-template <bool COMPACT, int MESH = MESH_NONE, bool SORT = false, bool DEFER = false, int SH = 0>
+template <bool COMPACT, int MESH = MESH_NONE, bool SORT = false, bool DEFER = false, int SH = 0, int AIM = AIM_NONE>
 __device__ __forceinline__ void tile_shade(const BounceArgs &a, const TileCtx &c, const Pool &in, const Pool &out, int depth,
                                            const TileRegs &tr, f3 ro, f3 rd, float t, f3 nrm, int mat, int outside,
                                            uint32_t n, uint32_t dst_base, uint32_t &packed, uint32_t &traced,
@@ -246,9 +246,26 @@
         }
         if (!ENV && !alive) end_path();
     }
+    if constexpr (AIM == AIM_WRITER) {
+        static_assert(COMPACT && MESH == MESH_NONE && !SORT && !DEFER && SH == 0, "the aimed writer is the plain fused compacting kernel");
+        const uint64_t survived = ballot64(alive);
+        if (alive) {
+            constexpr size_t SC = offsetof(BounceArgs, scene);
+            const CullRay cr = cull_ray(ps.o, ps.d, karg_field<float>(SC + offsetof(SceneDev, rmax)));
+            bool aimed = cr.wild;
+            const int ne = karg_field<int>(offsetof(BounceArgs, aim_n));
+            for (int k = 0; k < ne; ++k) {
+                cfloat *cb = as_const(karg_field<const float *>(SC + offsetof(SceneDev, cull))) +
+                             karg_field<int>(offsetof(BounceArgs, aim_geom) + 4 * (size_t)k) * CULL_WORDS;
+                aimed |= cull_box(cr, cb[0], cb[1], cb[2], cb[3], cb[4], cb[5]);
+            }
+            alive = aimed;
+        }
+        traced += (uint32_t)__popcll((unsigned long long)(survived & ~ballot64(alive)));
+    }
     const uint64_t bal = ballot64(alive);
     const uint64_t act = ballot64(tr.active);
-    traced += (uint32_t)__popcll((unsigned long long)act);
+    if constexpr (AIM != AIM_WRITER) traced += (uint32_t)__popcll((unsigned long long)act);
     uint32_t dst = tr.i;
     if (COMPACT && SORT) {
         for_each_key(alive, (uint32_t)mat, [&](uint32_t k, uint64_t m) {
@@ -281,7 +298,7 @@
     if (ENV && tr.active && !alive) end_path();
 }
 
-template <bool COMPACT, int MESH, bool SORT = false, bool DEFER = false, bool OWN = false, int SH = 0, bool FIRST = false>
+template <bool COMPACT, int MESH, bool SORT = false, bool DEFER = false, bool OWN = false, int SH = 0, bool FIRST = false, int AIM = AIM_NONE>
 __device__ __forceinline__ void tile_finish(const BounceArgs &a, const TileCtx &c, const WaveQ &q, int par, const Pool &in,
                                             const Pool &out, int depth, const TileRegs &tr, uint32_t n, uint32_t dst_base,
                                             uint32_t &packed, uint32_t &traced, uint32_t key_stride = 0) {
@@ -291,7 +308,7 @@
     float t = -1.0f; f3 nrm = ptd::mk(0, 0, 0); int mat = 0, outside = 1;
     int geom = -1;
     if (tr.active) tile_result(q, par, c.acc, a.scene.tris, tr.mb, t, nrm, mat, outside, geom);
-    tile_shade<COMPACT, MESH, SORT, DEFER, SH>(a, c, in, out, depth, tr, ro, rd, t, nrm, mat, outside, n, dst_base, packed, traced, key_stride,
+    tile_shade<COMPACT, MESH, SORT, DEFER, SH, AIM>(a, c, in, out, depth, tr, ro, rd, t, nrm, mat, outside, n, dst_base, packed, traced, key_stride,
                                            OWN ? (uint32_t)(geom + 1) << OWN_SHIFT : 0u, geom);
     if constexpr (FIRST && (SH & SH_ENV) != 0) {
         if (tr.miss0)
@@ -305,7 +322,7 @@
     uint32_t b0, b1, b2, b3;
 };
 
-template <int MODE, bool COMPACT, int MESH, bool GEN, bool SORT = false, bool DEFER = false, bool RESOLVE = false, bool OWN = false, int SH = 0>
+template <int MODE, bool COMPACT, int MESH, bool GEN, bool SORT = false, bool DEFER = false, bool RESOLVE = false, bool OWN = false, int SH = 0, int AIM = AIM_NONE>
 __device__ __forceinline__ void run_tiles(const BounceArgs &a, const TileCtx &c, WaveQ &q, const Pool &in, const Pool &out,
                                           int depth, uint32_t first_tile, uint32_t count, uint32_t tiles,
                                           uint32_t n, bool packed_in, uint32_t span_in, uint32_t &cur, uint32_t dst_base,
@@ -385,7 +402,7 @@
             const uint32_t ticket = q.total;
             if (pending) {
                 drain_to(q, c.acc, prev_ticket);
-                tile_finish<COMPACT, MESH, SORT, DEFER, OWN, SH, MODE == MODE_FIRST2>(a, c, q, par ^ 1, in, out, depth, prev, n, dst_base, packed, traced, key_stride);
+                tile_finish<COMPACT, MESH, SORT, DEFER, OWN, SH, MODE == MODE_FIRST2, AIM>(a, c, q, par ^ 1, in, out, depth, prev, n, dst_base, packed, traced, key_stride);
             }
             prev = tr; prev_ticket = ticket; pending = true; par ^= 1;
         } else if (MODE == MODE_CACHE0) {
@@ -413,7 +430,7 @@
     }
     if (pending) {
         drain_to(q, c.acc, prev_ticket);
-        tile_finish<COMPACT, MESH, SORT, DEFER, OWN, SH, MODE == MODE_FIRST2>(a, c, q, par ^ 1, in, out, depth, prev, n, dst_base, packed, traced, key_stride);
+        tile_finish<COMPACT, MESH, SORT, DEFER, OWN, SH, MODE == MODE_FIRST2, AIM>(a, c, q, par ^ 1, in, out, depth, prev, n, dst_base, packed, traced, key_stride);
     }
 }
 
@@ -422,12 +439,14 @@
 __device__ uint32_t g_wave_hw[8][8192];
 #endif
 
-template <int MODE, bool COMPACT, int MESH, bool SLDS, bool GEN = false, bool SORT = false, bool OWN = false, int SH = 0>
+template <int MODE, bool COMPACT, int MESH, bool SLDS, bool GEN = false, bool SORT = false, bool OWN = false, int SH = 0, int AIM = AIM_NONE>
 __global__ __launch_bounds__(BLOCK, MESH == MESH_TILES ? PT_LOOP_WAVES : (MESH == MESH_PRE && PT_PRE_WAVES > PT_MIN_WAVES) ? PT_PRE_WAVES : (SORT && MODE == MODE_FUSED && MESH == MESH_NONE) ? PT_SORT_WAVES : ((MODE == MODE_FUSED || MODE == MODE_CACHE0 || mode_first2(MODE)) && COMPACT && MESH == MESH_NONE && !SORT && PT_FUSED_WAVES > PT_MIN_WAVES) ? PT_FUSED_WAVES : PT_MIN_WAVES) void k_bounce(BounceArgs a) {
     static_assert(!OWN || ((MODE == MODE_FUSED || MODE == MODE_CACHE0 || mode_first2(MODE)) && COMPACT && MESH == MESH_NONE && !SORT),
                   "own-surface form: the plain fused compacting kernel, or the table form of its bounce 0");
     static_assert(!mode_first2(MODE) || (COMPACT && MESH == MESH_NONE && GEN && !SORT), "MODE_FIRST2 / MODE_STATE2: the plain compacting pipeline's first launch");
     static_assert(MODE != MODE_STATE2 || SH == 0, "MODE_STATE2: sessions without environment map or lobes");
+    static_assert(AIM == AIM_NONE || (MODE == MODE_FUSED && COMPACT && MESH == MESH_NONE && !GEN && !SORT && SH == 0),
+                  "the aimed forms: the plain fused compacting kernel of bounces >= 2");
 #ifdef PT_WAVE_TIMES
     const unsigned long long wt0 = __builtin_amdgcn_s_memrealtime();
 #endif
@@ -451,7 +470,7 @@
     const int lane = threadIdx.x & 63;
     c.lane = lane;
     const uint32_t Wp = gridDim.x * WAVES;
-    constexpr bool DEFER = COMPACT && MESH == MESH_NONE && !SORT && MODE != MODE_ISECT;
+    constexpr bool DEFER = COMPACT && MESH == MESH_NONE && !SORT && MODE != MODE_ISECT && AIM != AIM_WRITER;
     constexpr bool RESOLVE = MODE == MODE_FUSED && COMPACT && MESH == MESH_NONE && !SORT && !GEN;
     const uint32_t W = (SORT && COMPACT) ? a.dir_out.W : Wp;
     const uint32_t runs_per_wave = (SORT && COMPACT) ? W / Wp : 1u;
@@ -474,7 +493,7 @@
         if (packed_in && wid * R < tiles)
             cur = aligned ? find_range(a.dir_in.tbase(), a.dir_in.nr, wid * R) : find_range(a.dir_in.base(), a.dir_in.nr, wid * R * TILE);
         STAMP(2);
-        run_tiles<MODE, COMPACT, MESH, GEN, SORT, DEFER, RESOLVE, OWN, SH>(a, c, q, a.in, a.out, a.depth, wid * R, R, tiles, n, packed_in, span_in,
+        run_tiles<MODE, COMPACT, MESH, GEN, SORT, DEFER, RESOLVE, OWN, SH, AIM>(a, c, q, a.in, a.out, a.depth, wid * R, R, tiles, n, packed_in, span_in,
                                                   cur, wid * R * TILE, false, WgSpans{}, packed, traced, W * R * TILE, aligned);
         if (COMPACT) {
             if (SORT) {
@@ -503,6 +522,16 @@
             const uint32_t tb = sctl[8] + sctl[9] + sctl[10] + sctl[11];
             if (tb) { atomicAdd(&a.ctl->nlive[1], tb); atomicAdd(&a.ctl->alive[1], tb); }
         }
+    } else if (AIM == AIM_WRITER) {
+        if (blockIdx.x == 0 && threadIdx.x == 0) a.ctl->alive[a.depth] = n;
+        if (lane == 0) sctl[8 + (threadIdx.x >> 6)] = traced;
+        __syncthreads();
+        if (threadIdx.x == 0) {
+            const uint32_t tb = sctl[8] + sctl[9] + sctl[10] + sctl[11];
+            if (tb) atomicAdd(&a.ctl->aim_dropped, tb);
+        }
+    } else if (AIM == AIM_READER) {
+        if (blockIdx.x == 0 && threadIdx.x == 0) a.ctl->alive[a.depth] = n + a.ctl->aim_dropped;
     } else if (COMPACT) {
         if (blockIdx.x == 0 && threadIdx.x == 0) a.ctl->alive[a.depth] = n;
     } else {
diff --git a/project3-cuda-path-tracer_amd/csrc/pt_types.hpp b/project3-cuda-path-tracer_amd/csrc/pt_types.hpp
--- a/project3-cuda-path-tracer_amd/csrc/pt_types.hpp
+++ b/project3-cuda-path-tracer_amd/csrc/pt_types.hpp
@@ -41,6 +41,9 @@
     return plain_fused && ngeoms >= 1 && ngeoms <= OWN_MAX_GEOMS && paths <= OWN_MAX_PATHS;
 }
 
+constexpr int AIM_MAX = 4;
+enum { AIM_NONE = 0, AIM_WRITER = 1, AIM_READER = 2 };
+
 template <typename T>
 __device__ __forceinline__ T &at(T *plane, uint32_t i) {
     return *reinterpret_cast<T *>(reinterpret_cast<char *>(plane) + (i << 2));
@@ -118,13 +121,16 @@
     uint32_t done_sort[MAX_DEPTH];
     uint32_t error;
     uint32_t scan_ticks[MAX_DEPTH];
-    uint32_t pad[512 - 16 - 32 - 2 * (MAX_DEPTH + 1) - 3 * MAX_DEPTH - 1];
+    uint32_t aim_dropped;
+    uint32_t pad[512 - 16 - 32 - 2 * (MAX_DEPTH + 1) - 3 * MAX_DEPTH - 2];
     uint32_t bucket[MAX_DEPTH][2][32 * 16];
     uint32_t ticket[33 * 16];
 };
 constexpr int ELECT_BUCKETS = 32;
 static_assert(offsetof(Control, ticket) == 2048 + 2 * MAX_DEPTH * 32 * 16 * 4, "Control up to `ticket` is one memset block");
 static_assert(sizeof(Control) % 16 == 0, "memset block is a multiple of 16 B");
+static_assert(offsetof(Control, aim_dropped) > offsetof(Control, stamp) && offsetof(Control, pad) == offsetof(Control, aim_dropped) + 4 &&
+              offsetof(Control, bucket) == 2048, "aim_dropped is a word of the old pad: inside the per-batch memset, nothing else moved");
 
 __device__ __forceinline__ bool elect_last(uint32_t *buckets , uint32_t *top) {
     const uint32_t G = gridDim.x;
@@ -248,6 +254,8 @@
     float *first_state;
     const uint32_t *first_ended;
     uint32_t first_ended_tiles;
+    int aim_n;
+    int aim_geom[AIM_MAX];
 };
 
 enum : uint32_t { FS_ZERO = 0, FS_CONST = 1, FS_DIFFUSE = 2, FS_FIXED = 3, FS_KIND_MASK = 3 };
diff --git a/project3-cuda-path-tracer_amd/csrc/ptmi355.hip b/project3-cuda-path-tracer_amd/csrc/ptmi355.hip
--- a/project3-cuda-path-tracer_amd/csrc/ptmi355.hip
+++ b/project3-cuda-path-tracer_amd/csrc/ptmi355.hip
@@ -122,6 +122,22 @@
     return 0;
 }
 
+extern "C" int ptdbg_aimed_last(unsigned long long out[2]) {
+    out[0] = 0; out[1] = 0;
+    if (G.live) {
+        for (auto &wp : G.w) out[0] += wp->ctx.aimed_last_launches;
+        return 0;
+    }
+    if (!g_single.live) return -1;
+    out[0] = g_single.aimed_last_launches;
+    if (g_single.last_ctl) {
+        uint32_t dropped = 0;
+        if (hipMemcpy(&dropped, &g_single.last_ctl->aim_dropped, 4, hipMemcpyDeviceToHost) != hipSuccess) return -1;
+        out[1] = dropped;
+    }
+    return 0;
+}
+
 extern "C" int ptdbg_denoise(unsigned long long out[3]) {
     if (!g_single.live) return -1;
     for (int k = 0; k < 3; ++k) out[k] = g_single.dn_launches[k];
```

Result: no change. 65640 (-0.1%).
